# buctcurry/ICKA

Hardware: AMD Instinct MI355X
Metric: MNER samples/sec (fwd+bwd) at seq=128, 36 regions, bs=32 per GPU (higher is better)
Workload: dtype bf16; 1 GPU; c2: bert(H768,L12,h12,I3072)+36x2048 regions, seq_len 128, per-GPU batch 32, 1 cross layer(s), gated head, 13 labels, train mode p=0.1, token-CE loss; global_batch=32, seq_len=128, regions=36, parallelism=dp1, launch=hipgraph, precision=bf16, accumulate=1

## Files before the change

### icka_amd/_lib.py

```python
from __future__ import annotations

import ctypes as C
import os
from typing import Optional

_HERE = os.path.dirname(os.path.abspath(__file__))
LIB_PATH = os.path.join(_HERE, "libicka_hip.so")

c_vp, c_i32, c_i64, c_u64, c_f32 = C.c_void_p, C.c_int32, C.c_int64, C.c_uint64, C.c_float

ABI_VERSION = 6
GEMM_NT, GEMM_NN, GEMM_TN, GEMM_TT = 0, 1, 2, 3
ATTN_FP8, ATTN_TILED = 1, 2
LSTM_PER_STEP, LSTM_TICKETS, LSTM_NO_BATCH_SPLIT = 1, 2, 4
EPI_NONE, EPI_GELU, EPI_DGELU, EPI_ADD, EPI_GATE, EPI_TANH, EPI_RELU, EPI_ADD_RELU = 0, 1, 2, 3, 4, 5, 6, 7


class GemmDesc(C.Structure):
    _fields_ = [
        ("op", c_i32), ("M", c_i32), ("N", c_i32), ("K", c_i32), ("K1", c_i32),
        ("A", c_vp), ("lda", c_i64), ("B", c_vp), ("ldb", c_i64),
        ("A2", c_vp), ("lda2", c_i64), ("B2", c_vp), ("ldb2", c_i64),
        ("C", c_vp), ("ldc", c_i64), ("c_is_f32", c_i32),
        ("C2", c_vp), ("ldc2", c_i64),
        ("aux", c_vp), ("ldaux", c_i64),
        ("bias", c_vp), ("bias2", c_vp),
        ("alpha", c_f32), ("beta", c_f32),
        ("epilogue", c_i32),
        ("colsum_out", c_vp), ("colsum_accumulate", c_i32),
        ("ab_f16", c_i32), ("C3", c_vp), ("ldc3", c_i64), ("aux_f16", c_i32), ("c3_only", c_i32),
        ("tune", c_u64),
    ]


class SlabReduction(C.Structure):
    _fields_ = [("partials", c_vp), ("slab_stride", c_i64), ("nslab", c_i32), ("H", c_i32), ("nslots", c_i32),
                ("accumulate", c_i32), ("out", c_vp * 4)]


class XGemmDesc(C.Structure):
    _fields_ = [
        ("op", c_i32), ("M", c_i32), ("N", c_i32), ("K", c_i32),
        ("A", c_vp), ("lda", c_i64), ("a_bs0", c_i64), ("a_bs1", c_i64),
        ("B", c_vp), ("ldb", c_i64), ("b_bs0", c_i64), ("b_bs1", c_i64),
        ("C", c_vp), ("ldc", c_i64), ("c_bs0", c_i64), ("c_bs1", c_i64),
        ("nb0", c_i32), ("nb1", c_i32),
        ("bias", c_vp),
        ("alpha", c_f32), ("beta", c_f32),
    ]


PROTOTYPES = {
    "icka_abi_version": (c_i32, []),
    "icka_copy_many": (c_i32, [c_vp, c_vp, c_vp, c_i32, c_vp]),
    "icka_build_arch": (C.c_char_p, []),
    "icka_gemm": (c_i32, [C.POINTER(GemmDesc), c_vp]),
    "icka_gemm_grouped": (c_i32, [C.POINTER(GemmDesc), c_i32, c_vp]),
    "icka_gemm_grouped_ex": (c_i32, [C.POINTER(GemmDesc), c_i32, C.POINTER(SlabReduction), c_i32, c_vp]),
    "icka_gemm_ln": (c_i32, [C.POINTER(GemmDesc), c_vp, c_vp, c_i64, c_i32, c_vp, c_vp, c_vp, c_i64, c_vp, c_i32, c_vp, c_vp, c_f32,
                             c_f32, c_u64, c_vp, c_vp, c_vp]),
    "icka_gemm_qkv_attn": (c_i32, [C.POINTER(GemmDesc), c_vp, c_vp, c_vp, c_i64, c_vp, c_i32, c_i32, c_i32, c_f32, c_f32, c_u64, c_vp, c_vp]),
    "icka_gemm_ln_sync_words": (c_i64, []),
    "icka_gemm_ln_test_hooks": (c_i32, [c_i32, c_i32]),
    "icka_ln_fwd": (c_i32, [c_vp, c_i64, c_i32, c_vp, c_vp, c_i64, c_i32, c_vp, c_vp, c_vp, c_i64, c_vp, c_i64,
                            c_vp, c_vp, c_vp, c_i32, c_i32, c_f32, c_f32, c_u64, c_vp]),
    "icka_ln_fwd_h": (c_i32, [c_vp, c_i64, c_i32, c_vp, c_vp, c_i64, c_i32, c_vp, c_vp, c_vp, c_i64, c_vp, c_i64,
                            c_vp, c_vp, c_vp, c_i32, c_i32, c_f32, c_f32, c_u64, c_vp]),
    "icka_ln_bwd_workspace_floats": (c_i64, [c_i32]),
    "icka_ln_bwd": (c_i32, [c_vp, c_i64, c_vp, c_i64, c_vp, c_vp, c_vp, c_vp, c_i64, c_vp, c_i64, c_vp, c_vp, c_vp,
                            c_vp, c_i32, c_i32, c_f32, c_u64, c_i32, c_vp]),
    "icka_ln_bwd_slabs": (c_i32, [c_vp, c_i64, c_vp, c_i64, c_vp, c_vp, c_vp, c_vp, c_i64, c_vp, c_i64, c_vp, c_i32,
                                  c_i32, c_f32, c_u64, c_vp]),
    "icka_ln_bwd_nslab": (c_i32, [c_i32]),
    "icka_ln_slab_slots": (c_i32, []),
    "icka_embed_fwd": (c_i32, [c_vp, c_vp, c_vp, c_vp, c_vp, c_vp, c_vp, c_vp, c_vp, c_vp, c_vp, c_i32, c_i32,
                               c_i32, c_i32, c_i32, c_f32, c_f32, c_u64, c_vp]),
    "icka_embed_fwd_h": (c_i32, [c_vp, c_vp, c_vp, c_vp, c_vp, c_vp, c_vp, c_vp, c_vp, c_vp, c_vp, c_i32, c_i32,
                               c_i32, c_i32, c_i32, c_f32, c_f32, c_u64, c_vp]),
    "icka_embed_bwd": (c_i32, [c_vp, c_vp, c_vp, c_vp, c_vp, c_vp, c_vp, c_vp, c_vp, c_vp, c_vp, c_vp, c_i32, c_i32,
                               c_i32, c_i32, c_i32, c_i32, c_f32, c_u64, c_i32, c_vp]),
    "icka_embed_bwd_rows": (c_i32, [c_vp, c_vp, c_vp, c_vp, c_vp, c_vp, c_vp, c_vp, c_vp, c_vp, c_vp, c_vp, c_i32, c_i32,
                                    c_i32, c_i32, c_i32, c_i32, c_f32, c_u64, c_i32, c_vp]),
    "icka_embed_scatter_rows": (c_i32, [c_vp, c_i32, c_vp, c_vp, c_i64, c_i32, c_i32, c_i32, c_f32, c_vp]),
    "icka_attn_fwd": (c_i32, [c_vp, c_i64, c_vp, c_i64, c_vp, c_i64, c_vp, c_vp, c_i64, c_vp, c_i32, c_i32, c_i32,
                              c_i32, c_f32, c_f32, c_u64, c_vp]),
    "icka_attn_fwd_ex": (c_i32, [c_vp, c_i64, c_vp, c_i64, c_vp, c_i64, c_vp, c_vp, c_vp, c_i64, c_vp, c_i32, c_i32, c_i32,
                                 c_i32, c_f32, c_f32, c_u64, c_i32, c_vp, c_vp]),
    "icka_attn_keepbits_words": (c_i64, [c_i32, c_i32, c_i32, c_i32]),
    "icka_attn_fwd_fp8": (c_i32, [c_vp, c_i64, c_vp, c_i64, c_vp, c_i64, c_vp, c_vp, c_i64, c_vp, c_i32, c_i32, c_i32,
                              c_i32, c_f32, c_f32, c_u64, c_vp]),
    "icka_cls_head_fwd": (c_i32, [c_vp, c_vp, c_vp, c_vp, c_vp, c_i32, c_i32, c_i32, c_vp]),
    "icka_cls_head_fwd_h": (c_i32, [c_vp, c_vp, c_vp, c_vp, c_vp, c_i32, c_i32, c_i32, c_vp]),
    "icka_cls_head_bwd": (c_i32, [c_vp, c_i64, c_vp, c_vp, c_vp, c_vp, c_vp, c_vp, c_vp, c_vp, c_vp, c_i32, c_i32, c_i32,
                                  c_vp]),
    "icka_cls_head_bwd_slabs": (c_i32, [c_i32]),
    "icka_cls_head_slab_floats": (c_i64, [c_i32, c_i32]),
    "icka_conv_stem_patches": (c_i32, [c_vp, c_vp, c_i32, c_i32, c_i32, c_i64, c_vp]),
    "icka_conv_im2col3x3": (c_i32, [c_vp, c_vp, c_i32, c_i32, c_i32, c_i32, c_i32, c_i64, c_vp]),
    "icka_conv3x3_gemm": (c_i32, [c_vp, c_vp, c_vp, c_vp, c_i64, c_vp, c_i32, c_i32, c_i32, c_i32, c_i32, c_i32, c_i64, c_i32,
                                   c_vp, c_vp]),
    "icka_conv_subsample": (c_i32, [c_vp, c_vp, c_i32, c_i32, c_i32, c_i32, c_i32, c_i64, c_vp]),
    "icka_conv_maxpool3x3s2": (c_i32, [c_vp, c_vp, c_i32, c_i32, c_i32, c_i32, c_i64, c_vp]),
    "icka_conv_features_out": (c_i32, [c_vp, c_vp, c_vp, c_vp, c_i32, c_i32, c_i32, c_vp]),
    "icka_gemm_bn_stats": (c_i32, [c_vp, c_i64, c_vp, c_i64, c_vp, c_i64, c_i32, c_i32, c_i32, c_i64, c_vp, c_vp]),
    "icka_conv3x3_gemm_stats": (c_i32, [c_vp, c_vp, c_vp, c_i32, c_i32, c_i32, c_i32, c_i32, c_i32, c_i64, c_vp, c_vp, c_vp]),
    "icka_bn_finalize": (c_i32, [c_vp, c_i32, c_i32, c_vp, c_vp, c_vp, c_vp, c_vp, c_f32, c_f32, c_vp, c_vp, c_vp]),
    "icka_bn_apply": (c_i32, [c_vp, c_vp, c_vp, c_vp, c_vp, c_vp, c_vp, c_i32, c_i64, c_i64, c_i32, c_vp, c_vp, c_vp]),
    "icka_lstm_fwd": (c_i32, [c_vp, c_i64, c_vp, c_vp, c_vp, c_vp, c_vp, c_i32, c_i32, c_i32, c_i32, c_vp]),
    "icka_lstm_bwd": (c_i32, [c_vp, c_vp, c_vp, c_vp, c_vp, c_i64, c_vp, c_i32, c_i32, c_i32, c_i32, c_vp]),
    "icka_lstm_barrier_error": (c_i32, []),
    "icka_lstm_clear_error": (c_i32, []),
    "icka_lstm_set_reserved_cus": (c_i32, [c_i32]),
    "icka_lstm_test_hooks": (c_i32, [c_i32, c_i32]),
    "icka_linear_small_m": (c_i32, [c_vp, c_i64, c_vp, c_vp, c_vp, c_i64, c_i32, c_i32, c_i32, c_i32, c_vp]),
    "icka_transpose_bf16": (c_i32, [c_vp, c_vp, c_i32, c_i32, c_i32, c_vp]),
    "icka_crf_llh": (c_i32, [c_vp, c_i64, c_vp, c_vp, c_vp, c_vp, c_vp, c_vp, c_i32, c_i32, c_i32, c_vp]),
    "icka_crf_grad": (c_i32, [c_vp, c_i64, c_vp, c_vp, c_vp, c_vp, c_vp, c_vp, c_vp, c_i64, c_vp, c_vp, c_vp, c_i32,
                              c_i32, c_i32, c_vp]),
    "icka_crf_decode": (c_i32, [c_vp, c_i64, c_vp, c_vp, c_vp, c_vp, c_vp, c_vp, c_i32, c_i32, c_i32, c_vp]),
    "icka_crf_score_decode": (c_i32, [c_vp, c_i64, c_vp, c_vp, c_vp, c_vp, c_vp, c_vp, c_vp, c_vp, c_i64, c_i32, c_i32, c_i32,
                                      c_vp]),
    "icka_chunk_eval": (c_i32, [c_vp, c_vp, c_i64, c_vp, c_i64, c_vp, c_vp, c_vp, c_vp, c_i32, c_i32, c_i32, c_i32, c_vp]),
    "icka_loss_accumulate": (c_i32, [c_vp, c_vp, c_vp]),
    "icka_attn_bwd":(c_i32, [c_vp, c_i64, c_vp, c_i64, c_vp, c_i64, c_vp, c_vp, c_i64, c_vp, c_i64, c_vp, c_vp,
                              c_vp, c_i64, c_vp, c_i64, c_vp, c_i64, c_i32, c_i32, c_i32, c_i32, c_f32, c_f32, c_u64,
                              c_vp, c_i32, c_vp]),
    "icka_cast_f32_to_bf16": (c_i32, [c_vp, c_vp, c_i64, c_vp]),
    "icka_cast_to_f16": (c_i32, [c_vp, c_i32, c_vp, c_i64, c_vp]),
    "icka_cast_f32_to_bf16_f16": (c_i32, [c_vp, c_vp, c_vp, c_i64, c_vp]),
    "icka_cast_bf16_to_f32": (c_i32, [c_vp, c_vp, c_i64, c_vp]),
    "icka_cast_pad_f32_to_bf16": (c_i32, [c_vp, c_i64, c_vp, c_i64, c_i32, c_i32, c_vp]),
    "icka_additive_mask": (c_i32, [c_vp, c_i64, c_vp, c_i32, c_i32, c_vp]),
    "icka_dropout": (c_i32, [c_vp, c_i64, c_vp, c_i64, c_vp, c_i64, c_i32, c_i32, c_f32, c_u64, c_vp]),
    "icka_regions_to_tokens": (c_i32, [c_vp, c_vp, c_i32, c_i32, c_i32, c_i32, c_vp]),
    "icka_regions_to_tokens_h": (c_i32, [c_vp, c_vp, c_vp, c_i32, c_i32, c_i32, c_i32, c_vp]),
    "icka_sample_gate_fwd_h": (c_i32, [c_vp, c_i64, c_vp, c_i32, c_vp, c_vp, c_i64, c_i32, c_i32, c_i32, c_vp]),
    "icka_colsum": (c_i32, [c_vp, c_i64, c_vp, c_vp, c_i32, c_i32, c_i32, c_vp]),
    "icka_colsum_workspace_floats": (c_i64, [c_i32]),
    "icka_gate_bwd": (c_i32, [c_vp, c_i64, c_vp, c_vp, c_i64, c_vp, c_i64, c_vp, c_vp, c_i64, c_i32, c_i32, c_vp]),
    "icka_sample_gate_fwd": (c_i32, [c_vp, c_i64, c_vp, c_i64, c_vp, c_i32, c_vp, c_i64, c_i32, c_i32, c_i32, c_vp]),
    "icka_sample_gate_bwd": (c_i32, [c_vp, c_i64, c_vp, c_i64, c_vp, c_i64, c_vp, c_i32, c_vp, c_i64, c_vp, c_i64, c_vp,
                                     c_i32, c_i32, c_i32, c_vp]),
    "icka_crs_fwd": (c_i32, [c_vp, c_i64, c_vp, c_i64, c_vp, c_vp, c_vp, c_i32, c_i32, c_i32, c_vp]),
    "icka_crs_bwd": (c_i32, [c_vp, c_vp, c_i64, c_vp, c_i64, c_vp, c_vp, c_vp, c_vp, c_vp, c_i32, c_i32, c_i32, c_i32,
                             c_vp]),
    "icka_add_bf16": (c_i32, [c_vp, c_vp, c_vp, c_i64, c_vp]),
    "icka_tanh_bwd": (c_i32, [c_vp, c_vp, c_vp, c_i64, c_vp]),
    "icka_contrastive_workspace_floats": (c_i64, [c_i32]),
    "icka_contrastive_fwd": (c_i32, [c_vp, c_i64, c_vp, c_i64, c_i32, c_i32, c_i32, c_f32, c_f32, c_vp, c_i32, c_vp, c_vp, c_vp]),
    "icka_contrastive_bwd": (c_i32, [c_vp, c_i64, c_vp, c_i64, c_i32, c_i32, c_i32, c_f32, c_f32, c_vp, c_vp, c_vp, c_vp, c_vp,
                                     c_vp, c_i32, c_vp, c_vp]),
    "icka_relu_bwd": (c_i32, [c_vp, c_vp, c_vp, c_i64, c_i32, c_vp]),
    "icka_sample_swap": (c_i32, [c_vp, c_vp, c_i32, c_i64, c_i32, c_vp]),
    "icka_dgelu_bf16": (c_i32, [c_vp, c_vp, c_vp, c_i64, c_vp]),
    "icka_embed_prompt_fwd": (c_i32, [c_vp, c_vp, c_vp, c_vp, c_vp, c_vp, c_vp, c_vp, c_vp, c_vp, c_vp, c_vp, c_i32, c_i32,
# ... 101 lines not shown
```

### icka_amd/csrc/gemm.hip

```cpp
#include "common.h"
#include "ln_row.h"
#include "attn_core.h"
#include <cstdio>
#include <cstdlib>

namespace {

constexpr int BM = 128, BN = 128, BK = 64;
constexpr int TILE_BYTES = 128 * 64 * 2;

struct GemmArgs {
    int M, N, K, K1;
    const bf16_t* A;  int64_t lda;
    const bf16_t* B;  int64_t ldb;
    const bf16_t* A2; int64_t lda2;
    const bf16_t* B2; int64_t ldb2;
    void* C;  int64_t ldc;
    bf16_t* C2; int64_t ldc2;
    const bf16_t* aux; int64_t ldaux;
    const float* bias; const float* bias2;
    float alpha, beta;
    int epi, c_f32;
    int a_vec, b_vec;
    int abl;
// ... 274 lines not shown
__device__ __forceinline__ void wait_vmcnt() { asm volatile("s_waitcnt vmcnt(%0)" ::"n"(N) : "memory"); }

template <bool KM, int NCOL = 128>
__device__ __forceinline__ void dma_init(const bf16_t* (&ptr)[4], const bf16_t* __restrict__ P, int64_t ld, int row0,
                                         int wave, int lane) {
#pragma unroll
    for (int j = 0; j < 4; ++j) {
        const int p = wave + 4 * j;
        if (!KM) {
            const int row = (8 * p + (lane >> 3)) % NCOL;
            const int lc = (lane & 7) ^ ((row >> 1) & 7);
            ptr[j] = P + (int64_t)(row0 + row) * ld + 8 * lc;
        } else {
            const int kr = 4 * p + (lane >> 4);
            int lc = (lane & 15) ^ (((kr & 3) << 2) | ((kr >> 2) & 3));
            if (lc >= NCOL / 8) lc &= 7;
            ptr[j] = P + (int64_t)kr * ld + row0 + 8 * lc;
        }
    }
}
#ifndef ICKA_DMA_POL
#define ICKA_DMA_POL ""
#endif
template <int NJ = 4>
__device__ __forceinline__ void dma_issue(const bf16_t* (&ptr)[4], int64_t stride, uint32_t lds_base) {
    uint32_t keep;
    if constexpr (NJ == 2) {
        asm volatile(
            "s_mov_b32 %0, m0\n\t"
            "s_mov_b32 m0, %3\n\t"
            "s_nop 0\n\t"
            "global_load_lds_dwordx4 %1, off" ICKA_DMA_POL "\n\t"
            "s_add_u32 m0, m0, 0x1000\n\t"
            "s_nop 0\n\t"
            "global_load_lds_dwordx4 %2, off" ICKA_DMA_POL "\n\t"
            "s_mov_b32 m0, %0"
            : "=&s"(keep)
            : "v"(ptr[0]), "v"(ptr[1]), "s"(lds_base)
            : "memory", "scc");
#pragma unroll
        for (int j = 0; j < 2; ++j) ptr[j] += stride;
        return;
    }
    if constexpr (NJ == 3) {
        asm volatile(
            "s_mov_b32 %0, m0\n\t"
            "s_mov_b32 m0, %4\n\t"
            "s_nop 0\n\t"
            "global_load_lds_dwordx4 %1, off" ICKA_DMA_POL "\n\t"
            "s_add_u32 m0, m0, 0x1000\n\t"
            "s_nop 0\n\t"
            "global_load_lds_dwordx4 %2, off" ICKA_DMA_POL "\n\t"
            "s_add_u32 m0, m0, 0x1000\n\t"
            "s_nop 0\n\t"
            "global_load_lds_dwordx4 %3, off" ICKA_DMA_POL "\n\t"
            "s_mov_b32 m0, %0"
            : "=&s"(keep)
            : "v"(ptr[0]), "v"(ptr[1]), "v"(ptr[2]), "s"(lds_base)
            : "memory", "scc");
#pragma unroll
        for (int j = 0; j < 3; ++j) ptr[j] += stride;
        return;
    }
    asm volatile(
        "s_mov_b32 %0, m0\n\t"
        "s_mov_b32 m0, %5\n\t"
        "s_nop 0\n\t"
        "global_load_lds_dwordx4 %1, off" ICKA_DMA_POL "\n\t"
        "s_add_u32 m0, m0, 0x1000\n\t"
        "s_nop 0\n\t"
        "global_load_lds_dwordx4 %2, off" ICKA_DMA_POL "\n\t"
        "s_add_u32 m0, m0, 0x1000\n\t"
        "s_nop 0\n\t"
        "global_load_lds_dwordx4 %3, off" ICKA_DMA_POL "\n\t"
        "s_add_u32 m0, m0, 0x1000\n\t"
        "s_nop 0\n\t"
        "global_load_lds_dwordx4 %4, off" ICKA_DMA_POL "\n\t"
        "s_mov_b32 m0, %0"
        : "=&s"(keep)
        : "v"(ptr[0]), "v"(ptr[1]), "v"(ptr[2]), "v"(ptr[3]), "s"(lds_base)
        : "memory", "scc");
#pragma unroll
    for (int j = 0; j < 4; ++j) ptr[j] += stride;
}

__device__ __forceinline__ uint32_t off_c(int row, int ch) { return row * 512 + ((ch ^ (row & 31)) << 4); }
__device__ __forceinline__ uint32_t off_cw(int row, int ch) { return row * 768 + ((ch ^ (row & 15)) << 4); }

template <typename T>
__device__ __forceinline__ void st_out(T* p, const T v) {
#ifdef ICKA_ST_TEMPORAL
    *p = v;
#else
    __builtin_nontemporal_store(v, p);
#endif
}
template <typename T>
__device__ __forceinline__ T ld_once(const T* p) {
#ifdef ICKA_NT_AUX
    return __builtin_nontemporal_load(p);
#else
    return *p;
#endif
}
__device__ __forceinline__ void load8_bf16(const bf16_t* p, float (&o)[8]) {
    const bf16x8 v = as_bf16x8(ld_once(reinterpret_cast<const u32x4*>(p)));
#pragma unroll
    for (int e = 0; e < 8; ++e) o[e] = bf2f(v[e]);
}
__device__ __forceinline__ void load8_aux(const bf16_t* p, int f16, float (&o)[8]) {
    if (f16) {
        const f16x8 v = __builtin_bit_cast(f16x8, ld_once(reinterpret_cast<const u32x4*>(p)));
#pragma unroll
        for (int e = 0; e < 8; ++e) o[e] = (float)v[e];
    } else {
        load8_bf16(p, o);
    }
}
__device__ __forceinline__ void cvt8_aux(const u32x4 raw, int f16, float (&o)[8]) {
    if (f16) {
        const f16x8 v = __builtin_bit_cast(f16x8, raw);
#pragma unroll
        for (int e = 0; e < 8; ++e) o[e] = (float)v[e];
    } else {
        const bf16x8 v = as_bf16x8(raw);
#pragma unroll
        for (int e = 0; e < 8; ++e) o[e] = bf2f(v[e]);
    }
}
__device__ __forceinline__ void store8_bf16(bf16_t* p, const float (&v)[8]) {
    bf16x8 o;
#pragma unroll
    for (int e = 0; e < 8; ++e) o[e] = f2bf(v[e]);
    st_out(reinterpret_cast<u32x4*>(p), as_u32x4(o));
}
template <typename T>
__device__ __forceinline__ void st_main(T* p, const T v, int plain) {
    if (plain) *p = v;
    else st_out(p, v);
}
__device__ __forceinline__ void store8_bf16_main(bf16_t* p, const float (&v)[8], int plain) {
    bf16x8 o;
#pragma unroll
    for (int e = 0; e < 8; ++e) o[e] = f2bf(v[e]);
    st_main(reinterpret_cast<u32x4*>(p), as_u32x4(o), plain);
}

__device__ __forceinline__ _Float16 f2h(float v) { return (_Float16)fminf(fmaxf(v, -65504.f), 65504.f); }
__device__ __forceinline__ void store8_f16(void* p, const float (&v)[8], int plain = 0) {
    f16x8 o;
#pragma unroll
    for (int e = 0; e < 8; ++e) o[e] = f2h(v[e]);
    st_main(reinterpret_cast<u32x4*>(p), __builtin_bit_cast(u32x4, o), plain);
}

__device__ __forceinline__ void tile_origin(int bid, int nb, int nbm, int nbn, int& m0, int& n0, int bn = BN) {
    const int xcd = bid & 7, li = bid >> 3;
    if (nbn >= 12 && (nb & 7) == 0 && (nbm & 3) == 0 && (nbn & 1) == 0) {
        const int sm = nbm >> 2, sn = nbn >> 1;
        const int xi = xcd >> 1, xj = xcd & 1;
        m0 = (xi * sm + li / sn) * BM;
        n0 = (xj * sn + li % sn) * bn;
        return;
    }
    const int qn = nb >> 3, rn = nb & 7;
    const int sw = (xcd < rn ? xcd * (qn + 1) : rn * (qn + 1) + (xcd - rn) * qn) + li;
// ... 1071 lines not shown
    return best;
}

template <bool A_KM, bool B_KM, bool F16 = false>
int launch(GemmArgs g, bool aligned, hipStream_t st, const Tune& t) {
    const int nb = ((g.M + BM - 1) / BM) * ((g.N + BN - 1) / BN);
    if constexpr (!A_KM && !B_KM) {
        if (!aligned && g.n64ok && t.ws) {
            hipLaunchKernelGGL((gemm_ws_kernel<false, false, 3, 0, 64, F16>), dim3((g.M / BM) * (g.N / 64)), dim3(512), 0, st, g);
            ICKA_CHECK_LAUNCH();
            return 0;
        }
    }
    if (aligned) {
#ifdef ICKA_GEMM_ABLATE
        if (t.abl == 1 && !t.ws) hipLaunchKernelGGL((gemm_dma_kernel<A_KM, B_KM, 3, 1>), dim3(nb), dim3(256), 0, st, g);
        else if (t.abl == 2 && !t.ws) hipLaunchKernelGGL((gemm_dma_kernel<A_KM, B_KM, 3, 2>), dim3(nb), dim3(256), 0, st, g);
        else
#endif
        {
            if (t.ws || F16) {
#ifdef ICKA_GEMM_ABLATE
                if (t.bn == 96 && g.n96ok) {
                    const int nb96 = (g.M / BM) * (g.N / 96);
                    if (t.abl == 1) { hipLaunchKernelGGL((gemm_ws_kernel<A_KM, B_KM, 3, 1, 96>), dim3(nb96), dim3(512), 0, st, g); ICKA_CHECK_LAUNCH(); return 0; }
                    if (t.abl == 2) { hipLaunchKernelGGL((gemm_ws_kernel<A_KM, B_KM, 3, 2, 96>), dim3(nb96), dim3(512), 0, st, g); ICKA_CHECK_LAUNCH(); return 0; }
                    if (t.abl == 3) { hipLaunchKernelGGL((gemm_ws_kernel<A_KM, B_KM, 3, 3, 96>), dim3(nb96), dim3(512), 0, st, g); ICKA_CHECK_LAUNCH(); return 0; }
                }
                if (t.abl == 1) { hipLaunchKernelGGL((gemm_ws_kernel<A_KM, B_KM, 3, 1>), dim3(nb), dim3(512), 0, st, g); ICKA_CHECK_LAUNCH(); return 0; }
                if (t.abl == 2) { hipLaunchKernelGGL((gemm_ws_kernel<A_KM, B_KM, 3, 2>), dim3(nb), dim3(512), 0, st, g); ICKA_CHECK_LAUNCH(); return 0; }
#endif
                if constexpr (!A_KM) {
                    const int nb3 = (g.M / 256) * (g.N / 192);
                    const int rounds3 = (nb3 + 255) / 256;
                    if (t.w3 && g.M % 256 == 0 && g.N % 192 == 0 && g.K <= 1024 && g.K1 == 0 && nb3 % 8 == 0 &&
                        nb3 >= 128 && 4 * nb3 >= 3 * 256 * rounds3 && g.ksplit == 1) {
                        { const int pm = gemm_w3_grid(g.M, g.N, 192, t.w3grid), pn = 8 / pm;
                          g.w3_sn = (g.N / 192) / pn; g.w3_pnlog = pn == 1 ? 0 : (pn == 2 ? 1 : (pn == 4 ? 2 : 3)); }
                        hipLaunchKernelGGL((gemm_w3_kernel<B_KM, F16>), dim3(nb3), dim3(768), 0, st, g);
                        ICKA_CHECK_LAUNCH();
                        return 0;
                    }
                    const int nb2 = (g.M / 256) * (g.N / 128);
                    if (t.w3 && g.M % 256 == 0 && g.K1 == 0 && g.ksplit == 1 && nb2 % 8 == 0 && nb2 >= 192 && nb2 <= 256 &&
                        !(g.n96ok && t.bn == 96) && !(g.K <= 1024 && g.direct && g.c_f32 && g.epi == ICKA_EPI_NONE && g.beta == 0.f)) {
                        { const int pm = gemm_w3_grid(g.M, g.N, 128, t.w3grid), pn = 8 / pm;
                          g.w3_sn = (g.N / 128) / pn; g.w3_pnlog = pn == 1 ? 0 : (pn == 2 ? 1 : (pn == 4 ? 2 : 3)); }
                        hipLaunchKernelGGL((gemm_w3_kernel<B_KM, F16, 128>), dim3(nb2), dim3(768), 0, st, g);
                        ICKA_CHECK_LAUNCH();
                        return 0;
                    }
                }
                if (g.n96ok && t.bn != 128) {
                    const int nb96 = (g.M / BM) * (g.N / 96);
                    if (t.bn == 96 || (nb < 256 && nb96 <= 256 && nb96 > nb)) {
                        if ((t.ws == 2 || (t.ws == 1 && nb96 >= 448 && g.K <= 1024)) && !A_KM)
                            hipLaunchKernelGGL((gemm_ws2_kernel<A_KM, B_KM, 96, F16>), dim3(nb96), dim3(512), 0, st, g);
                        else if (t.nbuf == 4 && !F16)
                            hipLaunchKernelGGL((gemm_ws_kernel<A_KM, B_KM, 4, 0, 96>), dim3(nb96), dim3(512), 0, st, g);
                        else if (t.nbuf == 5 && !F16)
                            hipLaunchKernelGGL((gemm_ws_kernel<A_KM, B_KM, 5, 0, 96>), dim3(nb96), dim3(512), 0, st, g);
                        else
                            hipLaunchKernelGGL((gemm_ws_kernel<A_KM, B_KM, 3, 0, 96, F16>), dim3(nb96), dim3(512), 0, st, g);
                        ICKA_CHECK_LAUNCH();
                        return 0;
                    }
                }
                if ((t.ws == 2 || (t.ws == 1 && nb >= 448 && g.K <= 1024)) && !A_KM)
                    hipLaunchKernelGGL((gemm_ws2_kernel<A_KM, B_KM, 128, F16>), dim3(nb), dim3(512), 0, st, g);
                else if (t.nbuf == 4 && !F16) hipLaunchKernelGGL((gemm_ws_kernel<A_KM, B_KM, 4>), dim3(nb), dim3(512), 0, st, g);
                else if (t.nbuf == 5 && !F16) hipLaunchKernelGGL((gemm_ws_kernel<A_KM, B_KM, 5>), dim3(nb), dim3(512), 0, st, g);
                else hipLaunchKernelGGL((gemm_ws_kernel<A_KM, B_KM, 3, 0, 128, F16>), dim3(nb), dim3(512), 0, st, g);
                ICKA_CHECK_LAUNCH();
                return 0;
            }
            const int nbuf = t.nbuf > 0 ? t.nbuf : (nb >= 448 ? 2 : 4);
            if (nbuf == 2) hipLaunchKernelGGL((gemm_dma_kernel<A_KM, B_KM, 2, 0>), dim3(nb), dim3(256), 0, st, g);
            else if (nbuf == 3) hipLaunchKernelGGL((gemm_dma_kernel<A_KM, B_KM, 3, 0>), dim3(nb), dim3(256), 0, st, g);
            else hipLaunchKernelGGL((gemm_dma_kernel<A_KM, B_KM, 4, 0>), dim3(nb), dim3(256), 0, st, g);
        }
    } else {
        const int nk = (g.K + BK - 1) / BK;
        int ks = 1;
        if (g.c_f32 && g.epi == ICKA_EPI_NONE && nb < 64 && nk >= 16 && g.M <= 256 && !g.C3) {
            ks = 256 / nb;
            if (ks > nk / 4) ks = nk / 4;
            if (ks < 1) ks = 1;
        }
        if (ks > 1) {
            const int64_t n = (int64_t)g.M * g.N;
            hipLaunchKernelGGL(scale_c_kernel, dim3((unsigned)((n + 255) / 256)), dim3(256), 0, st,
                               reinterpret_cast<float*>(g.C), g.ldc, g.M, g.N, g.beta);
            ICKA_CHECK_LAUNCH();
            g.beta = 0.f;
            g.ksplit = ks;
        }
        hipLaunchKernelGGL((gemm_kernel<A_KM, B_KM, false, F16>), dim3(nb, ks), dim3(256), 0, st, g);
    }
    ICKA_CHECK_LAUNCH();
    return 0;
}

inline bool vec_ok(const void* p, int64_t ld) { return (ld % 8 == 0) && ((reinterpret_cast<uintptr_t>(p) & 15) == 0); }

}

#ifdef ICKA_GEMM_STAMP
extern "C" int icka_diag_gemm_stamp_buffer(void* p) {
    g_stamp = (unsigned long long*)p;
    return 0;
}
#endif

static int site_bit(const icka_gemm_desc* d) {
    const int64_t N = d->N, K = d->K;
    if (d->c_is_f32 == 1 || d->M < 1024) return -1;
    if (d->op == ICKA_GEMM_NT) {
        if (N == 3 * K) return 0;
        if (N == K) return 1;
        if (N == 4 * K) return 2;
        if (K == 4 * N) return 3;
    } else if (d->op == ICKA_GEMM_NN) {
        if (N == 4 * K) return 4;
        if (K == 4 * N) return 5;
        if (N == K) return 6;
        if (K == 3 * N) return 7;
    }
    return -1;
}
static int plain_mask() {
    static int m = -1;
    if (m < 0) {
        const char* e = getenv("ICKA_GEMM_PLAIN_MASK");
        m = e ? (int)strtol(e, nullptr, 0) : 0;
    }
    return m;
}

static int convert(const icka_gemm_desc* d, GemmArgs& g, bool& aligned, Tune& t) {
    if (!d || !d->A || !d->B || !d->C) return ICKA_E_ARG;
    if (!tune_of(d->tune, t)) return ICKA_E_ARG;
    if (d->M <= 0 || d->N <= 0 || d->K <= 0) return ICKA_E_SHAPE;
    if (d->op < ICKA_GEMM_NT || d->op > ICKA_GEMM_TN) return ICKA_E_ARG;
    if (d->K1 != 0 && (d->K1 < 0 || d->K1 >= d->K || d->K1 % BK != 0 || !d->A2 || !d->B2)) return ICKA_E_ARG;
    if ((d->epilogue == ICKA_EPI_GELU) && !d->C2) return ICKA_E_ARG;
    if ((d->epilogue == ICKA_EPI_DGELU || d->epilogue == ICKA_EPI_ADD || d->epilogue == ICKA_EPI_GATE ||
         d->epilogue == ICKA_EPI_ADD_RELU) && !d->aux)
        return ICKA_E_ARG;
    g.M = d->M; g.N = d->N; g.K = d->K; g.K1 = d->K1;
    g.A = (const bf16_t*)d->A; g.lda = d->lda; g.B = (const bf16_t*)d->B; g.ldb = d->ldb;
    g.A2 = (const bf16_t*)d->A2; g.lda2 = d->lda2; g.B2 = (const bf16_t*)d->B2; g.ldb2 = d->ldb2;
    g.C = d->C; g.ldc = d->ldc; g.C2 = (bf16_t*)d->C2; g.ldc2 = d->ldc2;
    g.aux = (const bf16_t*)d->aux; g.ldaux = d->ldaux; g.bias = d->bias; g.bias2 = d->bias2;
    g.alpha = d->alpha; g.beta = d->beta; g.epi = d->epilogue;
    if (d->c_is_f32 < 0 || d->c_is_f32 > 2) return ICKA_E_ARG;
    g.c_f32 = d->c_is_f32 == 1; g.c_f16 = d->c_is_f32 == 2;
    g.f16 = d->ab_f16 != 0; g.C3 = (bf16_t*)d->C3; g.ldc3 = d->ldc3; g.aux_f16 = d->aux_f16 != 0;
    if (g.f16 && d->op != ICKA_GEMM_NT) return ICKA_E_ARG;
    if (g.c_f16 && d->beta != 0.f) return ICKA_E_ARG;
    if (g.C3 && !g.c_f16 && !g.c_f32) return ICKA_E_ARG;
    if (g.C3 && g.c_f32 && d->op != ICKA_GEMM_TN) return ICKA_E_ARG;
    g.c3_only = d->c3_only != 0;
    {
        const int sb = site_bit(d);
        g.plain = (sb >= 0 && ((plain_mask() >> sb) & 1)) ? 1 : 0;
    }
    if (g.c3_only && !(g.C3 && g.c_f32 && d->beta == 0.f && d->epilogue == ICKA_EPI_NONE)) return ICKA_E_ARG;
// ... 180 lines not shown
        hipLaunchKernelGGL((gemm_ws_kernel<false, false, 3, 0, 64, false, true>), dim3((g.M / BM) * (Cout / 64)), dim3(512), 0, st, g);
    ICKA_CHECK_LAUNCH();
    return 0;
}

static int launch_bn_stats(BnStatsArgs& p, hipStream_t st) {
    GemmArgs& g = p.g;
    g.K1 = 0; g.alpha = 1.f; g.beta = 0.f; g.epi = ICKA_EPI_NONE; g.c_f32 = 0; g.a_vec = g.b_vec = 1; g.ksplit = 1; g.direct = 0;
    if (g.N % 128 == 0)
        hipLaunchKernelGGL((gemm_ws_bn_stats_kernel<128, false>), dim3((g.M / BM) * (g.N / 128)), dim3(512), 0, st, p);
    else
        hipLaunchKernelGGL((gemm_ws_bn_stats_kernel<64, false>), dim3((g.M / BM) * (g.N / 64)), dim3(512), 0, st, p);
    ICKA_CHECK_LAUNCH();
    return 0;
}

extern "C" int icka_gemm_bn_stats(const void* a, int64_t lda, const void* w, int64_t ldw, void* y, int64_t ldy, int32_t M, int32_t N,
                                  int32_t K, int64_t rows_valid, float* partials, void* stream) {
    if (!a || !w || !y || !partials) return ICKA_E_ARG;
    if (M <= 0 || M % BM || N <= 0 || N % 64 || K <= 0 || K % BK || rows_valid < 1 || rows_valid > M) return ICKA_E_SHAPE;
    auto al = [](const void* p) { return (reinterpret_cast<uintptr_t>(p) & 15) == 0; };
    if (!al(a) || !al(w) || !al(y) || !al(partials) || lda % 8 || ldw % 8 || ldy % 8 || lda < K || ldw < K || ldy < N)
        return ICKA_E_ALIGN;
    BnStatsArgs p{};
    p.g.M = M; p.g.N = N; p.g.K = K;
    p.g.A = (const bf16_t*)a; p.g.lda = lda; p.g.B = (const bf16_t*)w; p.g.ldb = ldw; p.g.C = y; p.g.ldc = ldy;
    p.part = partials; p.rows_valid = (int)rows_valid;
    return launch_bn_stats(p, (hipStream_t)stream);
}

extern "C" int icka_conv3x3_gemm_stats(const void* x, const void* w, void* y, int32_t B, int32_t H, int32_t W, int32_t C, int32_t Cout,
                                       int32_t stride, int64_t rows_padded, const void* zeros, float* partials, void* stream) {
    if (!x || !w || !y || !zeros || !partials) return ICKA_E_ARG;
    if (B <= 0 || H <= 0 || W <= 0 || C <= 0 || C % 64 || Cout <= 0 || Cout % 64 || (stride != 1 && stride != 2))
        return ICKA_E_SHAPE;
    const int Ho = (H + 2 - 3) / stride + 1, Wo = (W + 2 - 3) / stride + 1;
    const int64_t rows = (int64_t)B * Ho * Wo;
    if (rows_padded < rows || rows_padded % BM || rows_padded > 0x7fffffff) return ICKA_E_SHAPE;
    auto al = [](const void* p) { return (reinterpret_cast<uintptr_t>(p) & 15) == 0; };
    if (!al(x) || !al(w) || !al(y) || !al(zeros) || !al(partials)) return ICKA_E_ALIGN;
    BnStatsArgs p{};
    p.g.M = (int)rows_padded; p.g.N = Cout; p.g.K = 9 * C;
    p.g.A = (const bf16_t*)x; p.g.lda = C; p.g.B = (const bf16_t*)w; p.g.ldb = 9 * (int64_t)C; p.g.C = y; p.g.ldc = Cout;
    p.g.cvH = H; p.g.cvW = W; p.g.cvC = C; p.g.cvS = stride; p.g.cvHo = Ho; p.g.cvWo = Wo; p.g.cvRows = (int)rows;
    p.g.cvZero = (const bf16_t*)zeros;
    p.part = partials; p.rows_valid = (int)rows;
    GemmArgs& g = p.g;
    g.K1 = 0; g.alpha = 1.f; g.beta = 0.f; g.epi = ICKA_EPI_NONE; g.c_f32 = 0; g.a_vec = g.b_vec = 1; g.ksplit = 1; g.direct = 0;
    hipStream_t st = (hipStream_t)stream;
    if (Cout % 128 == 0)
        hipLaunchKernelGGL((gemm_ws_bn_stats_kernel<128, true>), dim3((g.M / BM) * (Cout / 128)), dim3(512), 0, st, p);
    else
        hipLaunchKernelGGL((gemm_ws_bn_stats_kernel<64, true>), dim3((g.M / BM) * (Cout / 64)), dim3(512), 0, st, p);
    ICKA_CHECK_LAUNCH();
    return 0;
}

template <bool A_KM, bool B_KM, int NBUF>
__global__ __launch_bounds__(512) void gemm_ws_group_kernel(const GroupArgs ga) {
    __shared__ __attribute__((aligned(16))) char smem[NBUF * 2 * TILE_BYTES];
    const int bid = blockIdx.x;
    int pi = 0;
#pragma unroll
    for (int i = 1; i < MAX_GROUP; ++i) pi += bid >= ga.start[i] ? 1 : 0;
    const GemmArgs g = ga.p[pi];
    gemm_ws_body<A_KM, B_KM, NBUF>(g, smem, bid - ga.start[pi], ga.start[pi + 1] - ga.start[pi]);
}

constexpr int BIG_STAGE = 3 * TILE_BYTES;
constexpr int BIG_NBUF = 3;
constexpr int CS_COLS = 64;

constexpr int MAX_RED = 4;
struct SlabRed {
    const float* partials; float* out[4];
    int nslab, H, nslots, slab_stride, accumulate, blocks;
};
struct BigGroupArgs {
    GemmArgs p[MAX_GROUP];
    int start[MAX_GROUP + 1];
    int cs_start[MAX_GROUP + 1];
    SlabRed red[MAX_RED];
    int red_start[MAX_RED + 1];
};

__device__ __forceinline__ void slab_reduce_block(const SlabRed& r, char* smem, int rb) {
    float* red = reinterpret_cast<float*>(smem);
    const int tid = threadIdx.x, cx = tid & 63, sy = tid >> 6;
    const int idx = rb * 64 + cx;
    const bool ok = idx < r.nslots * r.H;
    float s = 0.f;
    if (ok) {
        const int slot = idx / r.H, c = idx - slot * r.H;
        const float* p = r.partials + (int64_t)slot * r.H + c;
        for (int b = sy; b < r.nslab; b += 8) s += p[(int64_t)b * r.slab_stride];
    }
    red[sy * 64 + cx] = s;
    __syncthreads();
    if (sy == 0 && ok) {
        const int slot = idx / r.H, c = idx - slot * r.H;
        float* out = r.out[slot];
        if (out) {
            float t = 0.f;
#pragma unroll
            for (int k = 0; k < 8; ++k) t += red[k * 64 + cx];
            out[c] = r.accumulate ? out[c] + t : t;
        }
    }
}
__global__ __launch_bounds__(512) void slab_reduce_kernel(const SlabRed r) {
    __shared__ __attribute__((aligned(16))) char smem[8 * 64 * 4];
    slab_reduce_block(r, smem, blockIdx.x);
}
struct GroupArgsRed { GroupArgs ga; SlabRed red[MAX_RED]; int red_start[MAX_RED + 1]; };
template <bool A_KM, bool B_KM, int NBUF>
__global__ __launch_bounds__(512) void gemm_ws_group_red_kernel(const GroupArgsRed gr) {
    __shared__ __attribute__((aligned(16))) char smem[NBUF * 2 * TILE_BYTES];
    const int bid = blockIdx.x;
    const int tiles = gr.ga.start[MAX_GROUP];
    if (bid >= tiles) {
        const int rb = bid - tiles;
        int ri = 0;
#pragma unroll
        for (int i = 1; i < MAX_RED; ++i) ri += rb >= gr.red_start[i] ? 1 : 0;
        slab_reduce_block(gr.red[ri], smem, rb - gr.red_start[ri]);
        return;
    }
    int pi = 0;
#pragma unroll
    for (int i = 1; i < MAX_GROUP; ++i) pi += bid >= gr.ga.start[i] ? 1 : 0;
    const GemmArgs g = gr.ga.p[pi];
    gemm_ws_body<A_KM, B_KM, NBUF>(g, smem, bid - gr.ga.start[pi], gr.ga.start[pi + 1] - gr.ga.start[pi]);
}
struct SlabRedMulti { SlabRed red[MAX_RED]; int red_start[MAX_RED + 1]; };
__global__ __launch_bounds__(512) void slab_reduce_multi_kernel(const SlabRedMulti m) {
    __shared__ __attribute__((aligned(16))) char smem[8 * 64 * 4];
    const int rb = blockIdx.x;
    int ri = 0;
#pragma unroll
    for (int i = 1; i < MAX_RED; ++i) ri += rb >= m.red_start[i] ? 1 : 0;
    slab_reduce_block(m.red[ri], smem, rb - m.red_start[ri]);
}

template <bool WIRE>
__device__ __forceinline__ void gemm_big_tn_body(const GemmArgs& g, char* smem, const int m0, const int n0) {
    const int tid = threadIdx.x, lane = tid & 63;
    const int wave = __builtin_amdgcn_readfirstlane(tid >> 6);
    const uint32_t lds0 = __builtin_amdgcn_readfirstlane((uint32_t)reinterpret_cast<uintptr_t>(LDS_PTR(char, smem)));
    const int nk = g.K / BK;

    if (wave >= 4) {
        const int lw = wave - 4;
        const bf16_t* pa0[4];
        const bf16_t* pa1[4];
        const bf16_t* pb[4];
        dma_init<true>(pa0, g.A, g.lda, m0, lw, lane);
        dma_init<true>(pa1, g.A, g.lda, m0 + 128, lw, lane);
        dma_init<true>(pb, g.B, g.ldb, n0, lw, lane);
        const int64_t sa = (int64_t)BK * g.lda, sb = (int64_t)BK * g.ldb;
#define ICKA_BIG_STAGE(BUF)                                              \
    do {                                                                 \
        dma_issue(pa0, sa, lds0 + (BUF) + lw * 1024);                    \
        dma_issue(pa1, sa, lds0 + (BUF) + TILE_BYTES + lw * 1024);       \
        dma_issue(pb, sb, lds0 + (BUF) + 2 * TILE_BYTES + lw * 1024);    \
    } while (0)
#pragma unroll
// ... 54 lines not shown
    __builtin_amdgcn_sched_barrier(0);
    int cur = 0;
    for (int kt = 0; kt + 1 < nk; ++kt) {
        ICKA_BIG_READ(fa1, fb1, cur, 1);
        ICKA_BIG_MMA(fa0, fb0);
        ICKA_BIG_INTERLEAVE();
        const int nxt = cur + 1 == BIG_NBUF ? 0 : cur + 1;
        asm volatile("s_waitcnt lgkmcnt(0)" ::: "memory");
        __builtin_amdgcn_s_barrier();
        asm volatile("" ::: "memory");
        ICKA_BIG_READ(fa0, fb0, nxt, 0);
        ICKA_BIG_MMA(fa1, fb1);
        ICKA_BIG_INTERLEAVE();
        cur = nxt;
    }
    ICKA_BIG_READ(fa1, fb1, cur, 1);
    ICKA_BIG_MMA(fa0, fb0);
    ICKA_BIG_INTERLEAVE();
    ICKA_BIG_MMA(fa1, fb1);
    __builtin_amdgcn_sched_barrier(0);
#undef ICKA_BIG_INTERLEAVE
#undef ICKA_BIG_READ
#undef ICKA_BIG_MMA
    asm volatile("s_nop 7\n\ts_nop 7" ::: "memory");
#pragma unroll
    for (int ni = 0; ni < 4; ++ni) {
        const int n = n0 + wc + 16 * ni + 4 * (lane >> 4);
#pragma unroll
        for (int mi = 0; mi < 8; ++mi) {
            const int m = m0 + wsub * 128 + 16 * mi + (lane & 15);
            f32x4* dst = reinterpret_cast<f32x4*>(reinterpret_cast<float*>(g.C) + (int64_t)m * g.ldc + n);
            f32x4 v = acc[mi][ni] * g.alpha;
            if (g.beta != 0.f) v += g.beta * ld_once(dst);
            if (!WIRE || !g.c3_only) st_out(dst, v);
            if constexpr (WIRE) {
                if (g.C3) st_out(reinterpret_cast<u32x2*>(g.C3 + (int64_t)m * g.ldc3 + n), pack4(v[0], v[1], v[2], v[3]));
            }
        }
    }
}

__device__ __forceinline__ void big_colsum_block(const GemmArgs& g, char* smem, int cb) {
    float* red = reinterpret_cast<float*>(smem);
    const int tid = threadIdx.x, cx = tid & 7, ry = tid >> 3;
    const int col = cb * CS_COLS + cx * 8;
    float s[8];
#pragma unroll
    for (int e = 0; e < 8; ++e) s[e] = 0.f;
    if (col < g.M) {
        const bf16_t* base = g.A + col;
        int k = ry;
        for (; k + 7 * 64 < g.K; k += 8 * 64) {
            u32x4 v[8];
#pragma unroll
            for (int u = 0; u < 8; ++u) v[u] = *reinterpret_cast<const u32x4*>(base + (int64_t)(k + 64 * u) * g.lda);
#pragma unroll
            for (int u = 0; u < 8; ++u) {
                const bf16x8 h = as_bf16x8(v[u]);
#pragma unroll
                for (int e = 0; e < 8; ++e) s[e] += bf2f(h[e]);
            }
        }
        for (; k < g.K; k += 64) {
            const bf16x8 h = as_bf16x8(*reinterpret_cast<const u32x4*>(base + (int64_t)k * g.lda));
#pragma unroll
            for (int e = 0; e < 8; ++e) s[e] += bf2f(h[e]);
        }
    }
#pragma unroll
    for (int e = 0; e < 8; ++e) red[ry * CS_COLS + cx * 8 + e] = s[e];
    __syncthreads();
    if (tid < CS_COLS) {
        const int c = cb * CS_COLS + tid;
        if (c < g.M) {
            float t = 0.f;
#pragma unroll 8
            for (int r = 0; r < 64; ++r) t += red[r * CS_COLS + tid];
            g.colsum[c] = g.colsum_acc ? g.colsum[c] + t : t;
        }
    }
}


template <bool WIRE>
__device__ __forceinline__ void gemm_big12_tn_body(const GemmArgs& g, char* smem, const int m0, const int n0) {
    const int tid = threadIdx.x, lane = tid & 63;
    const int wave = __builtin_amdgcn_readfirstlane(tid >> 6);
    const uint32_t lds0 = __builtin_amdgcn_readfirstlane((uint32_t)reinterpret_cast<uintptr_t>(LDS_PTR(char, smem)));
    const int nk = g.K / BK;
    if (wave >= 8) {
        const int lw = wave - 8;
        const bf16_t* pa0[4];
        const bf16_t* pa1[4];
        const bf16_t* pb[4];
        dma_init<true>(pa0, g.A, g.lda, m0, lw, lane);
        dma_init<true>(pa1, g.A, g.lda, m0 + 128, lw, lane);
        dma_init<true>(pb, g.B, g.ldb, n0, lw, lane);
        const int64_t sa = (int64_t)BK * g.lda, sb = (int64_t)BK * g.ldb;
#define ICKA_BIG_STAGE(BUF)                                              \
    do {                                                                 \
        dma_issue(pa0, sa, lds0 + (BUF) + lw * 1024);                    \
        dma_issue(pa1, sa, lds0 + (BUF) + TILE_BYTES + lw * 1024);       \
        dma_issue(pb, sb, lds0 + (BUF) + 2 * TILE_BYTES + lw * 1024);    \
    } while (0)
#pragma unroll
        for (int t = 0; t < BIG_NBUF - 1; ++t)
            if (t < nk) ICKA_BIG_STAGE(t * BIG_STAGE);
        int cur = 0;
        for (int kt = 0; kt < nk; ++kt) {
            int ahead = nk - 1 - kt;
            ahead = ahead > BIG_NBUF - 2 ? BIG_NBUF - 2 : ahead;
            if (ahead >= 1) wait_vmcnt<12>();
            else wait_vmcnt<0>();
            __builtin_amdgcn_s_barrier();
            if (kt + BIG_NBUF - 1 < nk) {
                int nx = cur + BIG_NBUF - 1;
                nx = nx >= BIG_NBUF ? nx - BIG_NBUF : nx;
                ICKA_BIG_STAGE(nx * BIG_STAGE);
            }
            cur = cur + 1 == BIG_NBUF ? 0 : cur + 1;
        }
#undef ICKA_BIG_STAGE
        return;
    }
    const int wr = (wave >> 1) * 64, wc = (wave & 1) * 64;
    f32x4 acc[4][4];
#pragma unroll
    for (int i = 0; i < 4; ++i)
#pragma unroll
        for (int j = 0; j < 4; ++j) acc[i][j] = f32x4{0.f, 0.f, 0.f, 0.f};
    int cur = 0;
    for (int kt = 0; kt < nk; ++kt) {
        __builtin_amdgcn_s_barrier();
        asm volatile("" ::: "memory");
        const char* st = smem + cur * BIG_STAGE;
        const char* sA = st + (wr >> 7) * TILE_BYTES;
        const char* sB = st + 2 * TILE_BYTES;
#pragma unroll
        for (int ks = 0; ks < 2; ++ks) {
            bf16x8 fa[4], fb[4];
#pragma unroll
            for (int t = 0; t < 4; ++t) fa[t] = read_frag<true>(sA, (wr & 127) + 16 * t, ks, lane);
#pragma unroll
            for (int t = 0; t < 4; ++t) fb[t] = read_frag<true>(sB, wc + 16 * t, ks, lane);
#pragma unroll
            for (int mi = 0; mi < 4; ++mi)
#pragma unroll
                for (int ni = 0; ni < 4; ++ni) acc[mi][ni] = mfma16(fb[ni], fa[mi], acc[mi][ni]);
        }
        cur = cur + 1 == BIG_NBUF ? 0 : cur + 1;
    }
    asm volatile("s_nop 7\n\ts_nop 7" ::: "memory");
#pragma unroll
    for (int ni = 0; ni < 4; ++ni) {
        const int n = n0 + wc + 16 * ni + 4 * (lane >> 4);
#pragma unroll
        for (int mi = 0; mi < 4; ++mi) {
            const int m = m0 + wr + 16 * mi + (lane & 15);
            f32x4* dst = reinterpret_cast<f32x4*>(reinterpret_cast<float*>(g.C) + (int64_t)m * g.ldc + n);
            f32x4 v = acc[mi][ni] * g.alpha;
            if (g.beta != 0.f) v += g.beta * ld_once(dst);
            if (!WIRE || !g.c3_only) st_out(dst, v);
            if constexpr (WIRE) {
                if (g.C3) st_out(reinterpret_cast<u32x2*>(g.C3 + (int64_t)m * g.ldc3 + n), pack4(v[0], v[1], v[2], v[3]));
            }
        }
    }
}

template <bool W12, bool WIRE = false>
__global__ __launch_bounds__(W12 ? 768 : 512) void gemm_big_group_kernel(const BigGroupArgs ga) {
    __shared__ __attribute__((aligned(16))) char smem[BIG_NBUF * BIG_STAGE];
    const int bid = blockIdx.x;
    const int tiles = ga.start[MAX_GROUP];
    if (bid >= tiles + ga.cs_start[MAX_GROUP]) {
        const int rb = bid - tiles - ga.cs_start[MAX_GROUP];
        int ri = 0;
#pragma unroll
        for (int i = 1; i < MAX_RED; ++i) ri += rb >= ga.red_start[i] ? 1 : 0;
        if (W12 && threadIdx.x >= 512) return;
        slab_reduce_block(ga.red[ri], smem, rb - ga.red_start[ri]);
        return;
    }
    if (bid >= tiles) {
        const int cb = bid - tiles;
        int pi = 0;
#pragma unroll
        for (int i = 1; i < MAX_GROUP; ++i) pi += cb >= ga.cs_start[i] ? 1 : 0;
        const GemmArgs g = ga.p[pi];
        if (W12 && threadIdx.x >= 512) return;
        big_colsum_block(g, smem, cb - ga.cs_start[pi]);
        return;
    }
    const int xcd = bid & 7, slot = bid >> 3;
    const int qn = tiles >> 3, rn = tiles & 7;
    const int gt = (xcd < rn ? xcd * (qn + 1) : rn * (qn + 1) + (xcd - rn) * qn) + slot;
    int pi = 0;
#pragma unroll
    for (int i = 1; i < MAX_GROUP; ++i) pi += gt >= ga.start[i] ? 1 : 0;
    const GemmArgs g = ga.p[pi];
    const int local = gt - ga.start[pi];
    const int nbm = g.M / 256, nbn = g.N / BN;
    int tm, tn;
    if (nbn > nbm) { tm = local % nbm; tn = local / nbm; }
    else { tm = local / nbn; tn = local % nbn; }
    if constexpr (W12) gemm_big12_tn_body<WIRE>(g, smem, tm * 256, tn * BN);
    else gemm_big_tn_body<WIRE>(g, smem, tm * 256, tn * BN);
}

static bool big_ok(const GemmArgs& g, bool aligned) {
    return aligned && g.M % 256 == 0 && g.c_f32 && g.epi == ICKA_EPI_NONE && g.K1 == 0 && !g.bias && !g.bias2 && g.direct;
}

template <bool A_KM, bool B_KM>
static int launch_group(const GroupArgs& ga, int total, hipStream_t st, const Tune& t) {
    if (t.ws) {
        hipLaunchKernelGGL((gemm_ws_group_kernel<A_KM, B_KM, 3>), dim3(total), dim3(512), 0, st, ga);
        ICKA_CHECK_LAUNCH();
        return 0;
    }
    const int nbuf = t.nbuf > 0 ? t.nbuf : (total >= 448 ? 2 : 4);
    if (nbuf == 2) hipLaunchKernelGGL((gemm_dma_group_kernel<A_KM, B_KM, 2>), dim3(total), dim3(256), 0, st, ga);
    else if (nbuf == 3) hipLaunchKernelGGL((gemm_dma_group_kernel<A_KM, B_KM, 3>), dim3(total), dim3(256), 0, st, ga);
    else hipLaunchKernelGGL((gemm_dma_group_kernel<A_KM, B_KM, 4>), dim3(total), dim3(256), 0, st, ga);
    ICKA_CHECK_LAUNCH();
    return 0;
}

static int grouped_impl(const icka_gemm_desc* descs, int32_t n, const icka_slab_reduction* reds, int32_t n_red,
                        hipStream_t st);

extern "C" int icka_gemm_grouped(const icka_gemm_desc* descs, int32_t n, void* stream) {
    if (!descs || n <= 0) return ICKA_E_ARG;
    return grouped_impl(descs, n, nullptr, 0, (hipStream_t)stream);
}

extern "C" int icka_gemm_grouped_ex(const icka_gemm_desc* descs, int32_t n, const icka_slab_reduction* reds,
                                    int32_t n_red, void* stream) {
    if (n < 0 || n_red < 0 || (n > 0 && !descs) || (n_red > 0 && !reds) || n_red > MAX_RED) return ICKA_E_ARG;
    for (int r = 0; r < n_red; ++r)
        if (!reds[r].partials || reds[r].nslab <= 0 || reds[r].H <= 0 || reds[r].nslots <= 0 || reds[r].nslots > 4 ||
            reds[r].slab_stride < (int64_t)reds[r].nslots * reds[r].H)
            return ICKA_E_ARG;
    return grouped_impl(descs, n, reds, n_red, (hipStream_t)stream);
}

static SlabRed to_red(const icka_slab_reduction& r) {
    SlabRed o{};
    o.partials = r.partials;
    for (int k = 0; k < 4; ++k) o.out[k] = k < r.nslots ? r.out[k] : nullptr;
    o.nslab = r.nslab; o.H = r.H; o.nslots = r.nslots; o.slab_stride = (int)r.slab_stride; o.accumulate = r.accumulate;
    o.blocks = (r.nslots * r.H + 63) / 64;
    return o;
}

static int grouped_impl(const icka_gemm_desc* descs, int32_t n, const icka_slab_reduction* reds, int32_t n_red,
                        hipStream_t st) {
    bool reds_done = n_red == 0;
    int i = 0;
    Tune t = kTuneEnv;
    if (n > 0 && !tune_of(descs[0].tune, t)) return ICKA_E_ARG;
    Tune tk;
    while (i < n) {
        if (t.big && t.ws && descs[i].op == ICKA_GEMM_TN) {
            BigGroupArgs ba;
            int cnt = 0, total = 0, cs_total = 0;
            while (i + cnt < n && cnt < MAX_GROUP && descs[i + cnt].op == ICKA_GEMM_TN) {
                bool aligned = false;
                GemmArgs g;
                const int rc = convert(&descs[i + cnt], g, aligned, tk);
                if (rc) return rc;
                if (!big_ok(g, aligned)) break;
                ba.p[cnt] = g;
                ba.start[cnt] = total;
                ba.cs_start[cnt] = cs_total;
                total += (g.M / 256) * (g.N / BN);
                if (g.colsum) cs_total += (g.M + CS_COLS - 1) / CS_COLS;
                ++cnt;
            }
            if (cnt >= 1 && total >= 64) {
                for (int k = cnt; k <= MAX_GROUP; ++k) { ba.start[k] = total; ba.cs_start[k] = cs_total; }
                for (int k = cnt; k < MAX_GROUP; ++k) ba.p[k] = ba.p[0];
                int red_total = 0;
                for (int r = 0; r < MAX_RED; ++r) {
                    ba.red_start[r] = red_total;
                    if (!reds_done && r < n_red) { ba.red[r] = to_red(reds[r]); red_total += ba.red[r].blocks; }
                    else ba.red[r] = SlabRed{};
                }
                ba.red_start[MAX_RED] = red_total;
                reds_done = true;
                bool wire = false;
                for (int k = 0; k < cnt; ++k) wire = wire || ba.p[k].C3 != nullptr;
                const dim3 grid(total + cs_total + red_total);
                if (t.big == 2) {
                    if (wire) hipLaunchKernelGGL((gemm_big_group_kernel<true, true>), grid, dim3(768), 0, st, ba);
                    else hipLaunchKernelGGL((gemm_big_group_kernel<true, false>), grid, dim3(768), 0, st, ba);
                } else {
                    if (wire) hipLaunchKernelGGL((gemm_big_group_kernel<false, true>), grid, dim3(512), 0, st, ba);
                    else hipLaunchKernelGGL((gemm_big_group_kernel<false, false>), grid, dim3(512), 0, st, ba);
                }
                ICKA_CHECK_LAUNCH();
                i += cnt;
                continue;
            }
        }
        GroupArgs ga;
        int cnt = 0, total = 0;
        const int op = descs[i].op;
        while (i + cnt < n && cnt < MAX_GROUP && descs[i + cnt].op == op && !descs[i + cnt].ab_f16) {
            bool aligned = false;
            const int rc = convert(&descs[i + cnt], ga.p[cnt], aligned, tk);
            if (rc) return rc;
            if (ga.p[cnt].colsum && !(aligned && t.ws)) return ICKA_E_ARG;
            if (!aligned) break;
            ga.start[cnt] = total;
            total += (ga.p[cnt].M / BM) * (ga.p[cnt].N / BN);
            ++cnt;
        }
        if (cnt >= 2) {
            for (int k = cnt; k <= MAX_GROUP; ++k) ga.start[k] = total;
            for (int k = cnt; k < MAX_GROUP; ++k) ga.p[k] = ga.p[0];
            int rc;
            if (op == ICKA_GEMM_TN && !reds_done && t.ws) {
                GroupArgsRed gr;
                gr.ga = ga;
                int red_total = 0;
                for (int r = 0; r < MAX_RED; ++r) {
                    gr.red_start[r] = red_total;
                    if (r < n_red) { gr.red[r] = to_red(reds[r]); red_total += gr.red[r].blocks; }
                    else gr.red[r] = SlabRed{};
                }
                gr.red_start[MAX_RED] = red_total;
                hipLaunchKernelGGL((gemm_ws_group_red_kernel<true, true, 3>), dim3(total + red_total), dim3(512), 0, st, gr);
                ICKA_CHECK_LAUNCH();
                reds_done = true;
                rc = 0;
            } else if (op == ICKA_GEMM_NT) rc = launch_group<false, false>(ga, total, st, t);
            else if (op == ICKA_GEMM_NN) rc = launch_group<false, true>(ga, total, st, t);
            else rc = launch_group<true, true>(ga, total, st, t);
            if (rc) return rc;
            i += cnt;
        } else {
            const int rc = icka_gemm(&descs[i], (void*)st);
            if (rc) return rc;
            ++i;
        }
    }
    if (!reds_done) {
        if (n_red == 1) {
            const SlabRed sr = to_red(reds[0]);
            hipLaunchKernelGGL(slab_reduce_kernel, dim3(sr.blocks), dim3(512), 0, st, sr);
        } else {
            SlabRedMulti m;
            int total = 0;
            for (int r = 0; r < MAX_RED; ++r) {
                m.red_start[r] = total;
                if (r < n_red) { m.red[r] = to_red(reds[r]); total += m.red[r].blocks; }
                else m.red[r] = SlabRed{};
            }
            m.red_start[MAX_RED] = total;
            for (int r = n_red; r < MAX_RED; ++r) m.red_start[r] = total;
            hipLaunchKernelGGL(slab_reduce_multi_kernel, dim3(total), dim3(512), 0, st, m);
        }
        ICKA_CHECK_LAUNCH();
    }
    return 0;
}
```

### icka_amd/csrc/layernorm.hip

```cpp
#include "common.h"
#include "ln_row.h"
#include <cstdlib>

namespace {

constexpr int BWD_BLOCKS = 1024;
constexpr int SLOTS = 4;

template <int NCH>
__global__ __launch_bounds__(256) void ln_fwd_kernel(const LnFwdArgs a_) {
    LnFwdArgs a = a_;
    a.drop = drop_resolve(a.drop);
    const int lane = threadIdx.x & 63;
    const int wid = blockIdx.x * 4 + (threadIdx.x >> 6), nw = gridDim.x * 4;
    ln_fwd_rows<NCH>(a, wid, nw, a.M, lane);
}

struct LnBwdArgs {
    const bf16_t* dy; int64_t lddy; const bf16_t* dy2; int64_t lddy2; const bf16_t* xhat; const float* rstd;
    const float* gamma; bf16_t* dres; int64_t lddres; bf16_t* dx; int64_t lddx; float* partials;
    int M, H; DropCfg drop;
};

template <int NCH, int NS>
__device__ __forceinline__ void flush_columns(float (&acc)[NS][NCH][8], float* lds, float* partials, int H) {
    const int lane = threadIdx.x & 63, nchunk = H >> 3;
    for (int i = threadIdx.x; i < NS * H; i += 256) lds[i] = 0.f;
    __syncthreads();
#pragma unroll
    for (int s = 0; s < NS; ++s)
#pragma unroll
        for (int i = 0; i < NCH; ++i) {
            const int c = lane + 64 * i;
            if (c < nchunk) {
#pragma unroll
                for (int e = 0; e < 8; ++e) atomicAdd(&lds[s * H + c * 8 + e], acc[s][i][e]);
            }
        }
    __syncthreads();
    float* slab = partials + (int64_t)blockIdx.x * SLOTS * H;
    for (int i = threadIdx.x; i < NS * H; i += 256) slab[i] = lds[i];
}

template <int NCH>
__device__ __forceinline__ void ln_bwd_load_raw(const LnBwdArgs& a, int row, int lane, int nchunk, u32x4 (&dy)[NCH], u32x4 (&dy2)[NCH],
                                                u32x4 (&xh)[NCH]) {
#pragma unroll
    for (int i = 0; i < NCH; ++i) {
        const int c = lane + 64 * i;
        if (c < nchunk) {
            dy[i] = *reinterpret_cast<const u32x4*>(a.dy + (int64_t)row * a.lddy + c * 8);
            if (a.dy2) dy2[i] = *reinterpret_cast<const u32x4*>(a.dy2 + (int64_t)row * a.lddy2 + c * 8);
            xh[i] = *reinterpret_cast<const u32x4*>(a.xhat + (int64_t)row * a.H + c * 8);
        }
    }
}
__device__ __forceinline__ void unpack8(const u32x4 raw, float (&o)[8]) {
    const bf16x8 v = as_bf16x8(raw);
#pragma unroll
    for (int e = 0; e < 8; ++e) o[e] = bf2f(v[e]);
}

template <int NCH>
__device__ __forceinline__ void ln_rows_body(const LnBwdArgs& a_, int blk, int nblk) {
    LnBwdArgs a = a_;
    a.drop = drop_resolve(a.drop);
    const int lane = threadIdx.x & 63;
    const int wid = blk * 4 + (threadIdx.x >> 6), nw = nblk * 4;
    const int nchunk = a.H >> 3;
    const float inv_h = 1.f / (float)a.H;
    u32x4 rdy[NCH], rdy2[NCH], rxh[NCH];
    if (wid < a.M) ln_bwd_load_raw<NCH>(a, wid, lane, nchunk, rdy, rdy2, rxh);
    for (int row = wid; row < a.M; row += nw) {
        float xh[NCH][8], gd[NCH][8];
        float s1 = 0.f, s2 = 0.f;
        uint32_t kb[NCH];
#pragma unroll
        for (int i = 0; i < NCH; ++i) {
            kb[i] = 0xffu;
            const int c = lane + 64 * i;
            if (a.drop.thr && c < nchunk) {
                const uint32_t base = (uint32_t)row * (uint32_t)a.H + c * 8;
                uint32_t bits = 0u;
#pragma unroll
                for (int e = 0; e < 8; ++e) bits |= (icka_hash(a.drop.s0, a.drop.s1, base + e) >= a.drop.thr ? 1u : 0u) << e;
                kb[i] = bits;
            }
        }
#pragma unroll
        for (int i = 0; i < NCH; ++i) asm volatile("" : "+v"(kb[i]));
#pragma unroll
        for (int i = 0; i < NCH; ++i) {
            const int c = lane + 64 * i;
            if (c < nchunk) {
                float dy[8];
                unpack8(rdy[i], dy);
                if (a.dy2) {
                    float t[8];
                    unpack8(rdy2[i], t);
#pragma unroll
                    for (int e = 0; e < 8; ++e) dy[e] += t[e];
                }
                unpack8(rxh[i], xh[i]);
                float g[8];
                load8f(a.gamma + c * 8, g);
#pragma unroll
                for (int e = 0; e < 8; ++e) {
                    gd[i][e] = g[e] * dy[e];
                    s1 += gd[i][e];
                    s2 += gd[i][e] * xh[i][e];
                }
            }
        }
        const int nrow = row + nw;
        if (nrow < a.M) ln_bwd_load_raw<NCH>(a, nrow, lane, nchunk, rdy, rdy2, rxh);
        const float c1 = wave_sum(s1) * inv_h, c2 = wave_sum(s2) * inv_h;
        const float rstd = a.rstd[row];
#pragma unroll
        for (int i = 0; i < NCH; ++i) {
            const int c = lane + 64 * i;
            if (c < nchunk) {
                float ds[8];
#pragma unroll
                for (int e = 0; e < 8; ++e) ds[e] = rstd * (gd[i][e] - c1 - xh[i][e] * c2);
                if (a.dres) store8(a.dres + (int64_t)row * a.lddres + c * 8, ds);
                if (a.drop.thr) {
#pragma unroll
                    for (int e = 0; e < 8; ++e) ds[e] *= ((kb[i] >> e) & 1u) ? a.drop.scale : 0.f;
                }
                if (a.dx) store8(a.dx + (int64_t)row * a.lddx + c * 8, ds);
            }
        }
    }
}

template <int NCH>
__global__ __launch_bounds__(256) void ln_bwd_kernel(const LnBwdArgs a) {
    ln_rows_body<NCH>(a, blockIdx.x, gridDim.x);
}

constexpr int COL_GROUPS = 128;
__device__ __forceinline__ void ln_cols_body(const bf16_t* __restrict__ dy, int64_t lddy,
                                             const bf16_t* __restrict__ dy2, int64_t lddy2,
                                             const bf16_t* __restrict__ xhat, const bf16_t* __restrict__ dx,
                                             int64_t lddx, float* __restrict__ partials, int M, int H,
                                             int rows_per_group, int bx, int by) {
    __shared__ float red[3][8][32][8];
    const int cx = threadIdx.x & 31, ry = threadIdx.x >> 5;
    const int col = (bx * 32 + cx) * 8;
    const int r0 = by * rows_per_group;
    int r1 = r0 + rows_per_group; r1 = r1 > M ? M : r1;
    float ag[8], ab[8], ax[8];
#pragma unroll
    for (int e = 0; e < 8; ++e) { ag[e] = 0.f; ab[e] = 0.f; ax[e] = 0.f; }
    if (col < H) {
#pragma unroll 4
        for (int r = r0 + ry; r < r1; r += 8) {
            float d[8], x[8];
            load8(dy + (int64_t)r * lddy + col, d);
            if (dy2) {
                float t[8];
                load8(dy2 + (int64_t)r * lddy2 + col, t);
#pragma unroll
                for (int e = 0; e < 8; ++e) d[e] += t[e];
            }
            load8(xhat + (int64_t)r * H + col, x);
#pragma unroll
            for (int e = 0; e < 8; ++e) { ag[e] += d[e] * x[e]; ab[e] += d[e]; }
            if (dx) {
                load8(dx + (int64_t)r * lddx + col, x);
#pragma unroll
                for (int e = 0; e < 8; ++e) ax[e] += x[e];
            }
        }
    }
#pragma unroll
    for (int e = 0; e < 8; ++e) { red[0][ry][cx][e] = ag[e]; red[1][ry][cx][e] = ab[e]; red[2][ry][cx][e] = ax[e]; }
    __syncthreads();
    for (int i = threadIdx.x; i < 3 * 256; i += 256) {
        const int slot = i >> 8, cc = i & 255, c = bx * 256 + cc;
        if (c < H) {
            float t = 0.f;
#pragma unroll
            for (int k = 0; k < 8; ++k) t += red[slot][k][cc >> 3][cc & 7];
            partials[((int64_t)by * SLOTS + slot) * H + c] = t;
        }
    }
}
__global__ __launch_bounds__(256) void ln_cols_kernel(const bf16_t* __restrict__ dy, int64_t lddy,
                                                      const bf16_t* __restrict__ dy2, int64_t lddy2,
                                                      const bf16_t* __restrict__ xhat, const bf16_t* __restrict__ dx,
                                                      int64_t lddx, float* __restrict__ partials, int M, int H,
                                                      int rows_per_group) {
    ln_cols_body(dy, lddy, dy2, lddy2, xhat, dx, lddx, partials, M, H, rows_per_group, blockIdx.x, blockIdx.y);
}

struct LnColsArgs {
    int nx, groups, rows_per_group;
};
template <int NCH>
__global__ __launch_bounds__(256) void ln_bwd_fused_kernel(const LnBwdArgs a, const LnColsArgs c) {
    const int ncol = c.nx * c.groups;
    if ((int)blockIdx.x >= ncol) {
        ln_rows_body<NCH>(a, blockIdx.x - ncol, gridDim.x - ncol);
        return;
    }
    ln_cols_body(a.dy, a.lddy, a.dy2, a.lddy2, a.xhat, nullptr, 0, a.partials, a.M, a.H, c.rows_per_group,
                 blockIdx.x % c.nx, blockIdx.x / c.nx);
}

__global__ __launch_bounds__(1024) void finalize_kernel(const float* __restrict__ partials, int nslab, int H, float* o0,
                                                        float* o1, float* o2, float* o3, int accumulate) {
    __shared__ float red[16][64];
    const int cx = threadIdx.x & 63, sy = threadIdx.x >> 6;
    const int idx = blockIdx.x * 64 + cx;
    float s = 0.f;
    if (idx < SLOTS * H) {
        const int slot = idx / H, c = idx - slot * H;
        for (int b = sy; b < nslab; b += 16) s += partials[((int64_t)b * SLOTS + slot) * H + c];
    }
    red[sy][cx] = s;
    __syncthreads();
    if (sy == 0 && idx < SLOTS * H) {
        const int slot = idx / H, c = idx - slot * H;
        float* out = slot == 0 ? o0 : slot == 1 ? o1 : slot == 2 ? o2 : o3;
        if (out) {
            float t = 0.f;
#pragma unroll
            for (int k = 0; k < 16; ++k) t += red[k][cx];
            out[c] = accumulate ? out[c] + t : t;
        }
    }
}

struct EmbFwdArgs {
    const int64_t* ids; const int64_t* tt; const float* word; const float* pos; const float* type;
    const float* gamma; const float* beta; bf16_t* y; void* yf; bf16_t* xhat; float* rstd;
    int M, S, H, vocab, n_type; float eps; DropCfg drop;
    const int32_t* src; const bf16_t* prompt; int S_in, P, pos_offset;
    int yf_f16;
};

template <int NCH>
__global__ __launch_bounds__(256) void embed_fwd_kernel(const EmbFwdArgs a_) {
    EmbFwdArgs a = a_;
    a.drop = drop_resolve(a.drop);
    const int lane = threadIdx.x & 63;
    const int wid = blockIdx.x * 4 + (threadIdx.x >> 6), nw = gridDim.x * 4;
    const int nchunk = a.H >> 3;
    const float inv_h = 1.f / (float)a.H;
    for (int row = wid; row < a.M; row += nw) {
        const int sp = row % a.S;
        const int sidx = a.src ? a.src[sp] : sp;
        const bf16_t* prow = sidx < 0 ? a.prompt + ((int64_t)(row / a.S) * a.P + (-1 - sidx)) * a.H : nullptr;
        int64_t id = sidx < 0 ? 0 : a.ids[a.src ? (int64_t)(row / a.S) * a.S_in + sidx : row];
        id = id < 0 ? 0 : (id >= a.vocab ? a.vocab - 1 : id);
        int64_t t = a.tt ? a.tt[row] : 0;
        t = t < 0 ? 0 : (t >= a.n_type ? a.n_type - 1 : t);
        float s[NCH][8];
        float sum = 0.f;
#pragma unroll
        for (int i = 0; i < NCH; ++i) {
            const int c = lane + 64 * i;
            if (c < nchunk) {
                float w[8], p[8], ty[8];
                if (prow) load8(prow + c * 8, w);
                else load8f(a.word + id * a.H + c * 8, w);
                load8f(a.pos + (int64_t)(sp + a.pos_offset) * a.H + c * 8, p);
                load8f(a.type + t * a.H + c * 8, ty);
#pragma unroll
                for (int e = 0; e < 8; ++e) { s[i][e] = (w[e] + p[e]) + ty[e]; sum += s[i][e]; }
            } else {
#pragma unroll
                for (int e = 0; e < 8; ++e) s[i][e] = 0.f;
            }
        }
        const float mean = wave_sum(sum) * inv_h;
        float sq = 0.f;
#pragma unroll
        for (int i = 0; i < NCH; ++i)
            if (lane + 64 * i < nchunk) {
#pragma unroll
                for (int e = 0; e < 8; ++e) { const float d = s[i][e] - mean; sq += d * d; }
            }
        const float rstd = 1.f / sqrtf(wave_sum(sq) * inv_h + a.eps);
        if (lane == 0 && a.rstd) a.rstd[row] = rstd;
#pragma unroll
// ... 244 lines not shown
                           int64_t ldy, void* y2, int64_t ldy2, void* y_twin, void* xhat, float* rstd, int32_t M,
                           int32_t H, float eps, float p_drop, uint64_t seed, void* stream) {
    if (!x || !gamma || !beta || !y) return ICKA_E_ARG;
    if (x_is_f32 < 0 || x_is_f32 > 2 || res_is_f32 < 0 || res_is_f32 > 2) return ICKA_E_ARG;
    if (M <= 0 || H <= 0 || H % 8 != 0 || H > 8 * 64 * MAX_CH) return ICKA_E_SHAPE;
    if (ldx % 8 || ldy % 8 || (residual && ldr % 8) || (y2 && ldy2 % 8)) return ICKA_E_ALIGN;
    if (!al16(x) || !al16(y) || (residual && !al16(residual)) || (y2 && !al16(y2)) || (xhat && !al16(xhat)) ||
        (bias && !al16(bias)) || !al16(gamma) || !al16(beta) || (y_twin && !al16(y_twin)))
        return ICKA_E_ALIGN;
    LnFwdArgs a{x, ldx, x_is_f32, bias, residual, ldr, res_is_f32, gamma, beta, (bf16_t*)y, ldy,
                (bf16_t*)y2, ldy2, y_twin, (bf16_t*)xhat, rstd, M, H, eps, make_drop(p_drop, seed), twin_f16};
    hipStream_t st = (hipStream_t)stream;
    DISPATCH_NCH(pick_nch(H), ln_fwd_kernel, fwd_grid(M), 0, st, a);
    ICKA_CHECK_LAUNCH();
    return 0;
}

extern "C" int icka_ln_fwd(const void* x, int64_t ldx, int32_t x_is_f32, const float* bias, const void* residual,
                           int64_t ldr, int32_t res_is_f32, const float* gamma, const float* beta, void* y,
                           int64_t ldy, void* y2, int64_t ldy2, float* y_f32, void* xhat, float* rstd, int32_t M,
                           int32_t H, float eps, float p_drop, uint64_t seed, void* stream) {
    return ln_fwd_impl(0, x, ldx, x_is_f32, bias, residual, ldr, res_is_f32, gamma, beta, y, ldy, y2, ldy2, y_f32, xhat, rstd,
                       M, H, eps, p_drop, seed, stream);
}
extern "C" int icka_ln_fwd_h(const void* x, int64_t ldx, int32_t x_kind, const float* bias, const void* residual,
                             int64_t ldr, int32_t res_kind, const float* gamma, const float* beta, void* y,
                             int64_t ldy, void* y2, int64_t ldy2, void* y_f16, void* xhat, float* rstd, int32_t M,
                             int32_t H, float eps, float p_drop, uint64_t seed, void* stream) {
    return ln_fwd_impl(1, x, ldx, x_kind, bias, residual, ldr, res_kind, gamma, beta, y, ldy, y2, ldy2, y_f16, xhat, rstd,
                       M, H, eps, p_drop, seed, stream);
}

extern "C" int icka_ln_bwd(const void* dy, int64_t lddy, const void* dy2, int64_t lddy2, const void* xhat,
                           const float* rstd, const float* gamma, void* dres, int64_t lddres, void* dx, int64_t lddx,
                           float* dgamma, float* dbeta, float* dbias, float* partials, int32_t M, int32_t H,
                           float p_drop, uint64_t seed, int32_t accumulate, void* stream) {
    if (!dy || !xhat || !rstd || !gamma || !partials) return ICKA_E_ARG;
    if (dbias && !dx) return ICKA_E_ARG;
    if (M <= 0 || H <= 0 || H % 8 != 0 || H > 8 * 64 * MAX_CH) return ICKA_E_SHAPE;
    if (lddy % 8 || (dy2 && lddy2 % 8) || (dres && lddres % 8) || (dx && lddx % 8)) return ICKA_E_ALIGN;
    if (!al16(dy) || (dy2 && !al16(dy2)) || !al16(xhat) || (dres && !al16(dres)) || (dx && !al16(dx)) || !al16(gamma))
        return ICKA_E_ALIGN;
    LnBwdArgs a{(const bf16_t*)dy, lddy, (const bf16_t*)dy2, lddy2, (const bf16_t*)xhat, rstd, gamma,
                (bf16_t*)dres, lddres, (bf16_t*)dx, lddx, partials, M, H, make_drop(p_drop, seed)};
    hipStream_t st = (hipStream_t)stream;
    int groups = (M + 31) / 32; groups = groups > COL_GROUPS ? COL_GROUPS : groups;
    const int rpg = (M + groups - 1) / groups;
    const int nx = (H + 255) / 256;
    if ((dgamma || dbeta) && !dbias) {
        const LnColsArgs c{nx, groups, rpg};
        const int grid = nx * groups + bwd_row_grid(M);
        switch (pick_nch(H)) {
            case 1: hipLaunchKernelGGL((ln_bwd_fused_kernel<1>), dim3(grid), dim3(256), 0, st, a, c); break;
            case 2: hipLaunchKernelGGL((ln_bwd_fused_kernel<2>), dim3(grid), dim3(256), 0, st, a, c); break;
            case 3: hipLaunchKernelGGL((ln_bwd_fused_kernel<3>), dim3(grid), dim3(256), 0, st, a, c); break;
            default: hipLaunchKernelGGL((ln_bwd_fused_kernel<4>), dim3(grid), dim3(256), 0, st, a, c); break;
        }
        ICKA_CHECK_LAUNCH();
        hipLaunchKernelGGL(finalize_kernel, dim3((2 * H + 63) / 64), dim3(1024), 0, st, partials, groups, H, dgamma,
                           dbeta, (float*)nullptr, (float*)nullptr, accumulate);
        ICKA_CHECK_LAUNCH();
        return 0;
    }
    DISPATCH_NCH(pick_nch(H), ln_bwd_kernel, bwd_row_grid(M), 0, st, a);
    ICKA_CHECK_LAUNCH();
    if (dgamma || dbeta || dbias) {
        hipLaunchKernelGGL(ln_cols_kernel, dim3((H + 255) / 256, groups), dim3(256), 0, st, (const bf16_t*)dy, lddy,
                           (const bf16_t*)dy2, lddy2, (const bf16_t*)xhat, dbias ? (const bf16_t*)dx : nullptr, lddx,
                           partials, M, H, rpg);
        ICKA_CHECK_LAUNCH();
        hipLaunchKernelGGL(finalize_kernel, dim3((SLOTS * H + 63) / 64), dim3(1024), 0, st, partials, groups, H, dgamma,
                           dbeta, dbias, (float*)nullptr, accumulate);
        ICKA_CHECK_LAUNCH();
    }
    return 0;
}

extern "C" int32_t icka_ln_bwd_nslab(int32_t M) {
    int groups = (M + 31) / 32;
    return groups > COL_GROUPS ? COL_GROUPS : groups;
}
extern "C" int32_t icka_ln_slab_slots(void) { return SLOTS; }

extern "C" int icka_ln_bwd_slabs(const void* dy, int64_t lddy, const void* dy2, int64_t lddy2, const void* xhat,
                                 const float* rstd, const float* gamma, void* dres, int64_t lddres, void* dx,
                                 int64_t lddx, float* partials, int32_t M, int32_t H, float p_drop, uint64_t seed,
                                 void* stream) {
    if (!dy || !xhat || !rstd || !gamma || !partials) return ICKA_E_ARG;
    if (M <= 0 || H <= 0 || H % 8 != 0 || H > 8 * 64 * MAX_CH) return ICKA_E_SHAPE;
    if (lddy % 8 || (dy2 && lddy2 % 8) || (dres && lddres % 8) || (dx && lddx % 8)) return ICKA_E_ALIGN;
    if (!al16(dy) || (dy2 && !al16(dy2)) || !al16(xhat) || (dres && !al16(dres)) || (dx && !al16(dx)) || !al16(gamma))
        return ICKA_E_ALIGN;
    LnBwdArgs a{(const bf16_t*)dy, lddy, (const bf16_t*)dy2, lddy2, (const bf16_t*)xhat, rstd, gamma,
                (bf16_t*)dres, lddres, (bf16_t*)dx, lddx, partials, M, H, make_drop(p_drop, seed)};
    const int groups = icka_ln_bwd_nslab(M);
    const int nx = (H + 255) / 256;
    const LnColsArgs c{nx, groups, (M + groups - 1) / groups};
    const int grid = nx * groups + bwd_row_grid(M);
    hipStream_t st = (hipStream_t)stream;
    switch (pick_nch(H)) {
        case 1: hipLaunchKernelGGL((ln_bwd_fused_kernel<1>), dim3(grid), dim3(256), 0, st, a, c); break;
        case 2: hipLaunchKernelGGL((ln_bwd_fused_kernel<2>), dim3(grid), dim3(256), 0, st, a, c); break;
        case 3: hipLaunchKernelGGL((ln_bwd_fused_kernel<3>), dim3(grid), dim3(256), 0, st, a, c); break;
        default: hipLaunchKernelGGL((ln_bwd_fused_kernel<4>), dim3(grid), dim3(256), 0, st, a, c); break;
    }
    ICKA_CHECK_LAUNCH();
    return 0;
}

static int embed_fwd_impl(int32_t twin_f16, const int64_t* ids, const int64_t* token_type, const float* word, const float* pos,
                              const float* type, const float* gamma, const float* beta, void* y, void* y_twin,
                              void* xhat, float* rstd, int32_t B, int32_t S, int32_t H, int32_t vocab,
                              int32_t n_type, float eps, float p_drop, uint64_t seed, void* stream) {
    if (!ids || !word || !pos || !type || !gamma || !beta || !y) return ICKA_E_ARG;
    if (B <= 0 || S <= 0 || H <= 0 || H % 8 != 0 || H > 8 * 64 * MAX_CH || vocab <= 0 || n_type <= 0)
        return ICKA_E_SHAPE;
    if (!al16(word) || !al16(pos) || !al16(type) || !al16(gamma) || !al16(beta) || !al16(y) || (xhat && !al16(xhat)) ||
        (y_twin && !al16(y_twin)))
        return ICKA_E_ALIGN;
    EmbFwdArgs a{ids, token_type, word, pos, type, gamma, beta, (bf16_t*)y, y_twin, (bf16_t*)xhat, rstd,
                 B * S, S, H, vocab, n_type, eps, make_drop(p_drop, seed), nullptr, nullptr, S, 0, 0, twin_f16};
    hipStream_t st = (hipStream_t)stream;
    DISPATCH_NCH(pick_nch(H), embed_fwd_kernel, row_grid(B * S), 0, st, a);
    ICKA_CHECK_LAUNCH();
    return 0;
}

extern "C" int icka_embed_fwd(const int64_t* ids, const int64_t* token_type, const float* word, const float* pos,
                              const float* type, const float* gamma, const float* beta, void* y, float* y_f32,
                              void* xhat, float* rstd, int32_t B, int32_t S, int32_t H, int32_t vocab,
                              int32_t n_type, float eps, float p_drop, uint64_t seed, void* stream) {
    return embed_fwd_impl(0, ids, token_type, word, pos, type, gamma, beta, y, y_f32, xhat, rstd, B, S, H, vocab, n_type, eps,
                          p_drop, seed, stream);
}
extern "C" int icka_embed_fwd_h(const int64_t* ids, const int64_t* token_type, const float* word, const float* pos,
                                const float* type, const float* gamma, const float* beta, void* y, void* y_f16,
                                void* xhat, float* rstd, int32_t B, int32_t S, int32_t H, int32_t vocab,
                                int32_t n_type, float eps, float p_drop, uint64_t seed, void* stream) {
    return embed_fwd_impl(1, ids, token_type, word, pos, type, gamma, beta, y, y_f16, xhat, rstd, B, S, H, vocab, n_type, eps,
                          p_drop, seed, stream);
}

extern "C" int icka_embed_prompt_fwd(const int64_t* ids, const int32_t* src, const void* prompt, const float* word,
                                     const float* pos, const float* type, const float* gamma, const float* beta, void* y,
                                     float* y_f32, void* xhat, float* rstd, int32_t B, int32_t S_in, int32_t S,
                                     int32_t P, int32_t H, int32_t vocab, int32_t pos_offset, float eps, float p_drop,
                                     uint64_t seed, void* stream) {
    if (!ids || !src || !prompt || !word || !pos || !type || !gamma || !beta || !y) return ICKA_E_ARG;
    if (B <= 0 || S <= 0 || S_in <= 0 || P <= 0 || H <= 0 || H % 8 != 0 || H > 8 * 64 * MAX_CH || vocab <= 0 || pos_offset < 0)
        return ICKA_E_SHAPE;
    if (!al16(word) || !al16(pos) || !al16(type) || !al16(gamma) || !al16(beta) || !al16(y) || (xhat && !al16(xhat)) ||
        !al16(prompt))
        return ICKA_E_ALIGN;
    EmbFwdArgs a{ids, nullptr, word, pos, type, gamma, beta, (bf16_t*)y, y_f32, (bf16_t*)xhat, rstd,
                 B * S, S, H, vocab, 1, eps, make_drop(p_drop, seed), src, (const bf16_t*)prompt, S_in, P, pos_offset, 0};
    hipStream_t st = (hipStream_t)stream;
    DISPATCH_NCH(pick_nch(H), embed_fwd_kernel, row_grid(B * S), 0, st, a);
    ICKA_CHECK_LAUNCH();
    return 0;
}

static int embed_bwd_impl(const void* dy, const int64_t* ids, const int64_t* token_type, const void* xhat,
                          const float* rstd, const float* gamma, float* dword, float* dtok, float* dpos, float* dtype,
                          float* dgamma, float* dbeta, float* partials, int32_t B, int32_t S, int32_t H,
                          int32_t vocab, int32_t n_type, int32_t padding_idx, float p_drop, uint64_t seed,
                          int32_t accumulate, void* stream) {
    if (!dy || !ids || !xhat || !rstd || !gamma || (!dword && !dtok) || !dpos || !dtype || !dgamma || !dbeta || !partials)
        return ICKA_E_ARG;
    if (B <= 0 || S <= 0 || H <= 0 || H % 8 != 0 || H > 8 * 64 * MAX_CH || vocab <= 0 || n_type <= 0)
        return ICKA_E_SHAPE;
    if (!al16(dy) || !al16(xhat) || !al16(gamma)) return ICKA_E_ALIGN;
    EmbBwdArgs a{(const bf16_t*)dy, ids, token_type, (const bf16_t*)xhat, rstd, gamma, dword, dpos, dtype, partials,
                 B * S, S, H, vocab, n_type, padding_idx, make_drop(p_drop, seed), nullptr, nullptr, S, 0, 0, dtok};
    hipStream_t st = (hipStream_t)stream;
    int grid = bwd_grid(B * S);
    if (S <= BWD_BLOCKS) {
        grid = S;
        switch (pick_nch(H)) {
            case 1: hipLaunchKernelGGL((embed_bwd_pos_kernel<1>), dim3(S), dim3(512), 8 * H * sizeof(float), st, a); break;
            case 2: hipLaunchKernelGGL((embed_bwd_pos_kernel<2>), dim3(S), dim3(512), 8 * H * sizeof(float), st, a); break;
            case 3: hipLaunchKernelGGL((embed_bwd_pos_kernel<3>), dim3(S), dim3(512), 8 * H * sizeof(float), st, a); break;
            default: hipLaunchKernelGGL((embed_bwd_pos_kernel<4>), dim3(S), dim3(512), 8 * H * sizeof(float), st, a); break;
        }
    } else {
        DISPATCH_NCH(pick_nch(H), embed_bwd_kernel, grid, 8 * H * sizeof(float), st, a);
    }
    ICKA_CHECK_LAUNCH();
    float* t0 = n_type <= 2 ? dtype : nullptr;
    float* t1 = n_type == 2 ? dtype + H : nullptr;
    hipLaunchKernelGGL(finalize_kernel, dim3((SLOTS * H + 63) / 64), dim3(1024), 0, st, partials, grid, H, dgamma,
// ... 86 lines not shown
```

### icka_amd/kernels.py

```python
from __future__ import annotations

import ctypes as C
import math
from typing import Optional

import torch

from . import _lib
from ._lib import (EPI_ADD, EPI_ADD_RELU, EPI_DGELU, EPI_GATE, EPI_GELU, EPI_NONE, EPI_RELU, EPI_TANH, GEMM_NN, GEMM_NT, GEMM_TN,
                   GemmDesc, check)

BF16 = torch.bfloat16
F32 = torch.float32
F16 = torch.float16


_RAW_STREAM = getattr(torch._C, "_cuda_getCurrentRawStream", None)
_CUR_DEVICE = getattr(torch._C, "_cuda_getDevice", None)


def _stream() -> int:
    if _RAW_STREAM is not None and _CUR_DEVICE is not None:
        return _RAW_STREAM(_CUR_DEVICE())
    return torch.cuda.current_stream().cuda_stream
# ... 180 lines not shown
        if tile_n not in (96, 128):
            raise ValueError("tile_n: 96 or 128")
        t |= (1 if tile_n == 96 else 2) << 4
    if wide_tiles is not None:
        t |= (2 if wide_tiles else 1) << 8
    if direct_epilogue is not None:
        t |= (2 if direct_epilogue else 1) << 12
    if warp_specialized is not None:
        if warp_specialized not in (0, 1, 2, 3):
            raise ValueError("warp_specialized: 0 .. 3")
        t |= (warp_specialized + 1) << 16
    if w3_grid is not None:
        if w3_grid not in (1, 2, 4, 8):
            raise ValueError("w3_grid: 1, 2, 4 or 8")
        t |= w3_grid << 20
    if big_tiles is not None:
        if big_tiles not in (0, 1, 2):
            raise ValueError("big_tiles: 0 .. 2")
        t |= (big_tiles + 1) << 24
    if ablation is not None:
        if ablation not in (1, 2, 3):
            raise ValueError("ablation: 1 .. 3 (diagnostic builds)")
        t |= ablation << 28
    return t


def gemm(op: int, A: torch.Tensor, B: torch.Tensor, out: torch.Tensor, **kw) -> torch.Tensor:
    lib = _lib.load()
    d = gemm_desc(op, A, B, out, **kw)
    if _PROF is not None:
        _PROF.append((0, d, 1, [d]))
    check(lib.icka_gemm(C.byref(d), _stream()), "icka_gemm")
    return out


def slab_reduction(partials: torch.Tensor, nslab: int, H: int, outs, accumulate: bool, slab_stride: int = 0,
                   offset: int = 0):
    r = _lib.SlabReduction()
    if slab_stride == 0:
        slab_stride = _lib.load().icka_ln_slab_slots() * H
    r.partials, r.slab_stride, r.nslab, r.H = partials.data_ptr() + 4 * offset, slab_stride, nslab, H
    r.nslots, r.accumulate = len(outs), int(bool(accumulate))
    for i, o in enumerate(outs):
        _dev(o, "reduction output")
        if o.dtype != F32 or o.numel() != H or not o.is_contiguous():
            raise ValueError("reduction outputs must be contiguous f32 with %d elements" % H)
        r.out[i] = o.data_ptr()
    r._keep = (partials,) + tuple(outs)
    return r


def cls_head_fwd(seq, gated, W, bias, logits):
    dt = seq.dtype if seq.dtype == F16 else BF16
    _mat(seq, "seq", dt); _mat(gated, "gated", dt)
    M, H = seq.shape
    Cn = W.shape[0]
    if not (seq.is_contiguous() and gated.is_contiguous() and W.is_contiguous() and logits.is_contiguous()):
        raise ValueError("cls_head_fwd: contiguous operands")
    if W.dtype != dt or tuple(W.shape) != (Cn, 2 * H) or logits.dtype != F32 or tuple(logits.shape) != (M, Cn):
        raise ValueError("cls_head_fwd: W %s [C,2H], logits f32 [M,C]" % dt)
    lib = _lib.load()
    fn = lib.icka_cls_head_fwd_h if dt == F16 else lib.icka_cls_head_fwd
    check(fn(seq.data_ptr(), gated.data_ptr(), W.data_ptr(), _ptr(bias), logits.data_ptr(), M, H, Cn, _stream()),
          "icka_cls_head_fwd")
    return logits


def cls_head_bwd(dl, seq, gated, gate, cross, W, dseq, du, dcross, partials):
    M, H = seq.shape
    Cn = W.shape[0]
    for n, t in (("seq", seq), ("gated", gated), ("gate", gate), ("cross", cross), ("dseq", dseq), ("du", du),
                 ("dcross", dcross)):
        _mat(t, n)
        if not t.is_contiguous() or tuple(t.shape) != (M, H):
            raise ValueError("%s must be contiguous bf16 [M,H]" % n)
    _mat(dl, "dl")
    lib = _lib.load()
    check(lib.icka_cls_head_bwd(dl.data_ptr(), dl.stride(0), seq.data_ptr(), gated.data_ptr(), gate.data_ptr(),
                                cross.data_ptr(), W.data_ptr(), dseq.data_ptr(), du.data_ptr(), dcross.data_ptr(),
                                partials.data_ptr(), M, H, Cn, _stream()), "icka_cls_head_bwd")
    return lib.icka_cls_head_bwd_slabs(M)


def gemm_grouped(descs, reductions=None) -> None:
    reductions = reductions or []
    if not descs and not reductions:
        return
    lib = _lib.load()
    arr = (GemmDesc * max(len(descs), 1))(*descs)
    if _PROF is not None and descs:
        _PROF.append((1, arr, len(descs), list(descs)))
    if not reductions:
        check(lib.icka_gemm_grouped(arr, len(descs), _stream()), "icka_gemm_grouped")
        return
    for i in range(0, len(reductions), 4):
        chunk = reductions[i:i + 4]
        rarr = (_lib.SlabReduction * len(chunk))(*chunk)
        check(lib.icka_gemm_grouped_ex(arr if i == 0 else None, len(descs) if i == 0 else 0, rarr, len(chunk),
                                       _stream()), "icka_gemm_grouped_ex")


def _kind(t: torch.Tensor) -> int:
    return {BF16: 0, F32: 1, F16: 2}[t.dtype]


def ln_fwd(x, bias, residual, gamma, beta, y, *, y2=None, y_f32=None, y_f16=None, xhat=None, rstd=None, eps=1e-12,
           p_drop=0.0, seed=0):
    lib = _lib.load()
    _mat(x, "x", x.dtype if x.dtype in (BF16, F32, F16) else BF16); _mat(y, "y")
    if residual is not None:
        _mat(residual, "residual", residual.dtype if residual.dtype in (BF16, F32, F16) else BF16)
    if y_f32 is not None and y_f16 is not None:
        raise ValueError("one twin copy: y_f32 or y_f16")
    M, H = x.shape
    twin = y_f16 if y_f16 is not None else y_f32
    if twin is not None and (twin.dtype != (F16 if y_f16 is not None else F32) or not twin.is_contiguous()
                             or tuple(twin.shape) != (M, H)):
        raise ValueError("twin output must be contiguous [M,H] f32 (y_f32) / fp16 (y_f16)")
    fn = lib.icka_ln_fwd_h if y_f16 is not None else lib.icka_ln_fwd
    check(fn(x.data_ptr(), x.stride(0), _kind(x), _ptr(bias), _ptr(residual), _ld(residual),
             0 if residual is None else _kind(residual), gamma.data_ptr(), beta.data_ptr(),
             y.data_ptr(), y.stride(0), _ptr(y2), _ld(y2), _ptr(twin), _ptr(xhat), _ptr(rstd),
             M, H, eps, p_drop, seed, _stream()), "icka_ln_fwd")
    return y


class GemmLnHandoffError(RuntimeError):
    """A stripe wait of a fused dense + LayerNorm launch gave up: the rows it finished are NaN."""


_GEMM_LN_ERR = None
_GEMM_LN_ERR_NP = None
_GEMM_LN_ERR_PTR = 0


def _gemm_ln_err_word() -> int:
    global _GEMM_LN_ERR, _GEMM_LN_ERR_NP, _GEMM_LN_ERR_PTR
    if _GEMM_LN_ERR is None:
        _GEMM_LN_ERR = torch.zeros(16, dtype=torch.int32).pin_memory()
        _GEMM_LN_ERR_NP = _GEMM_LN_ERR.numpy()
        _GEMM_LN_ERR_PTR = _GEMM_LN_ERR.data_ptr()
    return _GEMM_LN_ERR_PTR


def gemm_ln_sync(device) -> torch.Tensor:
    return torch.zeros(_lib.load().icka_gemm_ln_sync_words(), dtype=torch.int32, device=device)


def gemm_ln(h, w, o, bias, residual, gamma, beta, y, sync, *, y_f32=None, y_f16=None, xhat=None, rstd=None, eps=1e-12,
            p_drop=0.0, seed=0) -> bool:
    gemm_ln_check_error("detected before the next fused launch")
    lib = _lib.load()
    d = gemm_desc(GEMM_NT, h, w, o)
    _mat(y, "y")
    if residual is not None:
        _mat(residual, "residual", residual.dtype if residual.dtype in (BF16, F32, F16) else BF16)
    twin = y_f16 if y_f16 is not None else y_f32
    M, N = o.shape
    if twin is not None and (twin.dtype != (F16 if y_f16 is not None else F32) or not twin.is_contiguous() or tuple(twin.shape) != (M, N)):
        raise ValueError("twin output must be contiguous [M,N] f32 (y_f32) / fp16 (y_f16)")
    args = (d, _ptr(bias), _ptr(residual), _ld(residual), 0 if residual is None else _kind(residual), gamma.data_ptr(),
            beta.data_ptr(), y.data_ptr(), y.stride(0), _ptr(twin), int(y_f16 is not None), _ptr(xhat), _ptr(rstd), eps,
            p_drop, seed, sync.data_ptr(), _gemm_ln_err_word(), _stream())
    rc = lib.icka_gemm_ln(*args)
    if rc == -1:
        return False
    check(rc, "icka_gemm_ln")
    if _PROF is not None:
        d._keep = (h, w, o, bias, residual, gamma, beta, y, twin, xhat, rstd, sync)
        _PROF.append((2, args, 1, [d]))
    return True


def gemm_qkv_attn(x, w, bias, qkv, add_mask, ctx, lse, B, heads, S, *, p_drop=0.0, seed=0, scale=None, out16=None,
                  keepbits=None) -> bool:
    lib = _lib.load()
    d = gemm_desc(GEMM_NT, x, w, qkv, bias=bias)
    _mat(ctx, "ctx")
    H = heads * 64
    if tuple(qkv.shape) != (B * S, 3 * H) or tuple(ctx.shape) != (B * S, H):
        return False
    if add_mask.dtype != F32 or not add_mask.is_contiguous() or add_mask.numel() != B * S:
        raise ValueError("add_mask must be contiguous f32 [B, S]")
    if lse is not None and (lse.dtype != F32 or not lse.is_contiguous() or lse.numel() != B * heads * S):
        raise ValueError("lse must be contiguous f32 [B, heads, S]")
    if out16 is not None:
        _mat(out16, "out16", F16)
        if tuple(out16.shape) != tuple(ctx.shape) or out16.stride(0) != ctx.stride(0):
            raise ValueError("out16 must have the shape and row stride of ctx")
    if keepbits is not None and (not keepbits.is_cuda or keepbits.element_size() != 4 or not keepbits.is_contiguous()
                                 or keepbits.numel() < lib.icka_attn_keepbits_words(B, heads, S, S)):
        raise ValueError("keepbits: contiguous 32-bit device buffer of icka_attn_keepbits_words words (attn_keepbits)")
    args = (d, add_mask.data_ptr(), ctx.data_ptr(), _ptr(out16), ctx.stride(0), _ptr(lse), B, heads, S,
            (1.0 / 8.0) if scale is None else scale, p_drop, seed, _ptr(keepbits), _stream())
    rc = lib.icka_gemm_qkv_attn(*args)
    if rc == -1:
        return False
    check(rc, "icka_gemm_qkv_attn")
    if _PROF is not None:
        d._keep = (x, w, bias, qkv, add_mask, ctx, lse, out16, keepbits)
        _PROF.append((3, args, 1, [d]))
    return True


def gemm_ln_check_error(where: str = "") -> None:
    if _GEMM_LN_ERR_NP is not None and _GEMM_LN_ERR_NP[0] != 0:
        _GEMM_LN_ERR_NP[0] = 0
        raise GemmLnHandoffError(
            "icka_amd fused dense + LayerNorm%s: a block gave up waiting for the other blocks of its 128-row stripe -- the grid "
            "was not co-resident (another kernel held CUs: a collective on another stream, a second model, a partitioned GPU).  "
            "The rows it finished are NaN.  Reserve CUs (icka_lstm_set_reserved_cus) or set ICKA_FUSE_DENSE_LN=0."
            % ((" (" + where + ")") if where else ""))


def ln_bwd_slabs(dy, xhat, rstd, gamma, partials, *, dy2=None, dres=None, dx=None, p_drop=0.0, seed=0) -> int:
    lib = _lib.load()
    _mat(dy, "dy"); _mat(xhat, "xhat")
    M, H = dy.shape
    check(lib.icka_ln_bwd_slabs(dy.data_ptr(), dy.stride(0), _ptr(dy2), _ld(dy2), xhat.data_ptr(), rstd.data_ptr(),
                                gamma.data_ptr(), _ptr(dres), _ld(dres), _ptr(dx), _ld(dx), partials.data_ptr(), M, H,
                                p_drop, seed, _stream()), "icka_ln_bwd_slabs")
    return lib.icka_ln_bwd_nslab(M)


def ln_bwd_workspace(H: int, device) -> torch.Tensor:
    return torch.empty(_lib.load().icka_ln_bwd_workspace_floats(H), dtype=F32, device=device)


def ln_bwd(dy, xhat, rstd, gamma, *, dy2=None, dres=None, dx=None, dgamma=None, dbeta=None, dbias=None,
           partials=None, p_drop=0.0, seed=0, accumulate=True):
    lib = _lib.load()
    _mat(dy, "dy"); _mat(xhat, "xhat")
    M, H = dy.shape
    check(lib.icka_ln_bwd(dy.data_ptr(), dy.stride(0), _ptr(dy2), _ld(dy2), xhat.data_ptr(), rstd.data_ptr(),
                          gamma.data_ptr(), _ptr(dres), _ld(dres), _ptr(dx), _ld(dx), _ptr(dgamma), _ptr(dbeta),
                          _ptr(dbias), partials.data_ptr(), M, H, p_drop, seed, int(accumulate), _stream()),
          "icka_ln_bwd")


def embed_fwd(ids, token_type, word, pos, typ, gamma, beta, y, *, y_f32=None, y_f16=None, xhat=None, rstd=None, eps=1e-12,
              p_drop=0.0, seed=0):
    lib = _lib.load()
    _dev(ids, "ids")
    B, S = ids.shape
    H = word.shape[1]
    if y_f32 is not None and y_f16 is not None:
        raise ValueError("one twin copy: y_f32 or y_f16")
    twin = y_f16 if y_f16 is not None else y_f32
    if twin is not None and (twin.dtype != (F16 if y_f16 is not None else F32) or not twin.is_contiguous()):
        raise ValueError("twin output must be contiguous f32 (y_f32) / fp16 (y_f16)")
    fn = lib.icka_embed_fwd_h if y_f16 is not None else lib.icka_embed_fwd
    check(fn(ids.data_ptr(), _ptr(token_type), word.data_ptr(), pos.data_ptr(), typ.data_ptr(),
             gamma.data_ptr(), beta.data_ptr(), y.data_ptr(), _ptr(twin), _ptr(xhat), _ptr(rstd),
             B, S, H, word.shape[0], typ.shape[0], eps, p_drop, seed, _stream()), "icka_embed_fwd")
    return y


def embed_bwd(dy, ids, token_type, xhat, rstd, gamma, dword, dpos, dtype_, dgamma, dbeta, partials, *,
              padding_idx=0, p_drop=0.0, seed=0, accumulate=True):
    lib = _lib.load()
    B, S = ids.shape
    H = dword.shape[1]
    check(lib.icka_embed_bwd(dy.data_ptr(), ids.data_ptr(), _ptr(token_type), xhat.data_ptr(), rstd.data_ptr(),
                             gamma.data_ptr(), dword.data_ptr(), dpos.data_ptr(), dtype_.data_ptr(),
                             dgamma.data_ptr(), dbeta.data_ptr(), partials.data_ptr(), B, S, H, dword.shape[0],
                             dtype_.shape[0], padding_idx, p_drop, seed, int(accumulate), _stream()),
          "icka_embed_bwd")


def embed_bwd_rows(dy, ids, token_type, xhat, rstd, gamma, dtok, dpos, dtype_, dgamma, dbeta, partials, *, vocab,
                   padding_idx=0, p_drop=0.0, seed=0, accumulate=True):
    lib = _lib.load()
    B, S = ids.shape
    H = dtok.shape[1]
    if dtok.dtype != F32 or tuple(dtok.shape) != (B * S, H) or not dtok.is_contiguous():
        raise ValueError("dtok must be contiguous f32 [B*S, H]")
    check(lib.icka_embed_bwd_rows(dy.data_ptr(), ids.data_ptr(), _ptr(token_type), xhat.data_ptr(), rstd.data_ptr(),
                                  gamma.data_ptr(), dtok.data_ptr(), dpos.data_ptr(), dtype_.data_ptr(), dgamma.data_ptr(),
                                  dbeta.data_ptr(), partials.data_ptr(), B, S, H, int(vocab), dtype_.shape[0], padding_idx, p_drop,
                                  seed, int(accumulate), _stream()), "icka_embed_bwd_rows")


def embed_scatter_rows(rows, ids, dword, *, padding_idx=0, scale=1.0):
    _dev(rows, "rows"); _dev(ids, "ids"); _dev(dword, "dword")
    if rows.dtype not in (F32, BF16) or rows.dim() != 2 or not rows.is_contiguous():
        raise ValueError("rows must be contiguous f32 / bf16 [T, H]")
    if ids.dtype != torch.int64 or ids.numel() != rows.shape[0] or not ids.is_contiguous():
        raise ValueError("ids must be contiguous int64 with one entry per row")
    if dword.dtype != F32 or dword.dim() != 2 or dword.shape[1] != rows.shape[1] or not dword.is_contiguous():
        raise ValueError("dword must be contiguous f32 [vocab, H]")
    check(_lib.load().icka_embed_scatter_rows(rows.data_ptr(), int(rows.dtype == BF16), ids.data_ptr(), dword.data_ptr(),
                                              rows.shape[0], rows.shape[1], dword.shape[0], padding_idx, float(scale), _stream()),
          "icka_embed_scatter_rows")


def embed_prompt_fwd(ids, src, prompt, word, pos, typ, gamma, beta, y, *, y_f32=None, xhat=None, rstd=None,
                     pos_offset=0, eps=1e-5, p_drop=0.0, seed=0):
    lib = _lib.load()
    _dev(ids, "ids"); _dev(src, "src"); _dev(prompt, "prompt")
    if ids.dtype != torch.int64 or not ids.is_contiguous() or ids.dim() != 2:
        raise ValueError("ids must be contiguous int64 [B,S_in]")
    if src.dtype != torch.int32 or src.dim() != 1 or not src.is_contiguous():
        raise ValueError("src must be contiguous int32 [S]")
    B, S_in = ids.shape
# ... 806 lines not shown
```

### icka_amd/ops.py

```python
from __future__ import annotations

from typing import Optional

import torch

from . import kernels as K
from .arena import ParamArena

BF16, F32, F16 = torch.bfloat16, torch.float32, torch.float16
import os as _os
ATTN_KEEPBITS = _os.environ.get("ICKA_ATTN_KEEPBITS", "auto")
FUSE_DENSE_LN = _os.environ.get("ICKA_FUSE_DENSE_LN", "1") != "0"
FUSE_DENSE_LN_MIN_ROWS = 3072
FUSE_QKV_ATTN = _os.environ.get("ICKA_FUSE_QKV_ATTN", "1") != "0"
FUSE_QKV_ATTN_MIN_ROWS = 3072


def _keepbits_on(Sq: int, Skv: int) -> bool:
    if ATTN_KEEPBITS == "auto":
        return Sq > 128 and Skv > 128 and Sq <= 256 and Skv <= 256
    return ATTN_KEEPBITS == "1"


def _empty(ref: torch.Tensor, *shape, dtype=BF16) -> torch.Tensor:
    return torch.empty(*shape, dtype=dtype, device=ref.device)


def _c(t: torch.Tensor) -> torch.Tensor:
    if t.dtype != BF16:
        raise TypeError("expected a bf16 gradient, got %s" % t.dtype)
    return t if t.is_contiguous() else t.contiguous()


class Dims(object):
    __slots__ = ("B", "S", "R", "H", "I", "heads", "eps", "p_hidden", "p_attn", "train", "h16", "pack")

    def __init__(self, B, S, R, H, I, heads, eps, p_hidden, p_attn, train, h16=False, pack=None):
        self.B, self.S, self.R, self.H, self.I, self.heads, self.eps = B, S, R, H, I, heads, eps
        self.p_hidden = p_hidden if train else 0.0
        self.p_attn = p_attn if train else 0.0
        self.train = train
        self.h16 = bool(h16)
        self.pack = pack


def _fwd_twin(A: ParamArena, x, xf, d: Dims):
    if not d.h16:
        return xf
    if A.shadow16 is None:
        A.enable_fp16_shadow()
        A.sync(force=True)
    if xf is not None and xf.dtype == F16:
        return xf
    return K.cast_to_f16(x if xf is None else xf, _empty(x, x.shape[0], x.shape[1], dtype=F16))


def _wgrad(A: ParamArena, dy, x, gout, beta: float, bias=None) -> None:
    bout, bacc = None, False
    if bias is not None:
        bacc = A.grad_beta(bias) > 0
        bout = A.g_cat(bias) if isinstance(bias, tuple) else A.g(bias)
        M, N, Kt = dy.shape[1], x.shape[1], dy.shape[0]
        if M % 128 or N % 128 or Kt % 64:
            csw = A.workspace("colsum", K._lib.load().icka_colsum_workspace_floats(M))
            K.colsum(dy, bout, csw, accumulate=bacc)
            bout = None
    wire = A.wire_of(gout, beta)
    A.pending_wgrad.append((K.gemm_desc(K.GEMM_TN, dy, x, gout, beta=beta, colsum_out=bout, colsum_accumulate=bacc,
                                        **wire), dy, x, gout, bout, wire))


def _flush_wgrad(A: ParamArena) -> None:
    if A.pending_wgrad or A.pending_reductions:
        K.gemm_grouped([t[0] for t in A.pending_wgrad], reductions=A.pending_reductions)
        A.pending_wgrad = []
        A.pending_reductions = []


def _ln_bwd_deferred(A: ParamArena, tag: str, norm, dy, xhat, rstd, *, dy2, dres, dx, p_drop, seed) -> None:
    H = dy.shape[1]
    ws = A.workspace(tag, K._lib.load().icka_ln_bwd_workspace_floats(H))
    acc = A.grad_beta((norm.weight, norm.bias)) > 0
    nslab = K.ln_bwd_slabs(dy, xhat, rstd, norm.weight, ws, dy2=dy2, dres=dres, dx=dx, p_drop=p_drop, seed=seed)
    A.pending_reductions.append(K.slab_reduction(ws, nslab, H, (A.g(norm.weight), A.g(norm.bias)), acc))


def _attn_generic_fwd(qkv, kvbuf, self_attn: bool, add_mask, d: Dims, Skv: int, seed_a: int, ctx, ctx16, save: bool):
    import math
    from . import exact as X
    B, h, S, H = d.B, d.heads, d.S, d.H
    dh = H // h
    q32b = K.cast_bf16_to_f32(qkv, torch.empty(qkv.shape, dtype=F32, device=qkv.device))
    if self_attn:
        q, k, v = q32b[:, :H], q32b[:, H:2 * H], q32b[:, 2 * H:]
        kv32b = None
    else:
        kv32b = K.cast_bf16_to_f32(kvbuf, torch.empty(kvbuf.shape, dtype=F32, device=kvbuf.device))
        q, k, v = q32b, kv32b[:, :H], kv32b[:, H:]
    P = torch.empty(B, h, S, Skv, dtype=F32, device=qkv.device)
    X.gemm_raw(X.GEMM_NT, S, Skv, dh, q, q.stride(0), (S * q.stride(0), dh), k, k.stride(0), (Skv * k.stride(0), dh),
               P, Skv, (h * S * Skv, S * Skv), B, h)
    Pd = torch.empty_like(P) if d.p_attn > 0 else None
    X.softmax_fwd(P, Pd, add_mask, B, h, S, Skv, 1.0 / math.sqrt(dh), d.p_attn, seed_a)
    Pu = P if Pd is None else Pd
    ctx32 = torch.empty(B * S, H, dtype=F32, device=qkv.device)
    X.gemm_raw(X.GEMM_NN, S, dh, Skv, Pu, Skv, (h * S * Skv, S * Skv), v, v.stride(0), (Skv * v.stride(0), dh),
               ctx32, H, (S * H, dh), B, h)
    K.cast_f32_to_bf16(ctx32, ctx)
    if ctx16 is not None:
        K.cast_to_f16(ctx32, ctx16)
    return ("generic", q32b, kv32b, P, Pd) if save else None


def _attn_generic_bwd(gen, self_attn: bool, dctx, d: Dims, Skv: int, seed_a: int, dq_out, dkv_out) -> None:
    import math
    from . import exact as X
    _tag, q32b, kv32b, P, Pd = gen
    B, h, S, H = d.B, d.heads, d.S, d.H
    dh = H // h
    scale = 1.0 / math.sqrt(dh)
    dev = q32b.device
    d32 = K.cast_bf16_to_f32(dctx if dctx.is_contiguous() else dctx.contiguous(), torch.empty(B * S, H, dtype=F32, device=dev))
    if self_attn:
        q, k, v = q32b[:, :H], q32b[:, H:2 * H], q32b[:, 2 * H:]
        g32 = torch.empty(B * S, 3 * H, dtype=F32, device=dev)
        dq, dk, dv = g32[:, :H], g32[:, H:2 * H], g32[:, 2 * H:]
        gkv = None
    else:
        q, k, v = q32b, kv32b[:, :H], kv32b[:, H:]
        g32 = torch.empty(B * S, H, dtype=F32, device=dev)
        gkv = torch.empty(kv32b.shape, dtype=F32, device=dev)
        K.zero_(gkv.view(-1))
        dq, dk, dv = g32, gkv[:, :H], gkv[:, H:]
    pb = (h * S * Skv, S * Skv)
    Pu = P if Pd is None else Pd
    dS = torch.empty_like(P)
    X.gemm_raw(X.GEMM_NT, S, Skv, dh, d32, H, (S * H, dh), v, v.stride(0), (Skv * v.stride(0), dh), dS, Skv, pb, B, h)
    X.gemm_raw(X.GEMM_TN, Skv, dh, S, Pu, Skv, pb, d32, H, (S * H, dh), dv, dv.stride(0), (Skv * dv.stride(0), dh), B, h)
    X.softmax_bwd(P, dS, B, h, S, Skv, scale, d.p_attn, seed_a)
    X.gemm_raw(X.GEMM_NN, S, dh, Skv, dS, Skv, pb, k, k.stride(0), (Skv * k.stride(0), dh), dq, dq.stride(0),
               (S * dq.stride(0), dh), B, h)
    X.gemm_raw(X.GEMM_TN, Skv, dh, S, dS, Skv, pb, q, q.stride(0), (S * q.stride(0), dh), dk, dk.stride(0),
               (Skv * dk.stride(0), dh), B, h)
    K.cast_f32_to_bf16(g32, dq_out)
    if gkv is not None:
        K.cast_f32_to_bf16(gkv, dkv_out)


def _attn_core_fwd(A: ParamArena, sa, x, kv_src, add_mask, d: Dims, Skv: int, save: bool, x16=None, kv16=None):
    M, H = x.shape
    h16 = x16 is not None
    xa = x16 if h16 else x
    if kv_src is None:
        qkv = _empty(x, M, 3 * H)
        wq = (sa.query.weight, sa.key.weight, sa.value.weight)
        bq = A.f_cat((sa.query.bias, sa.key.bias, sa.value.bias))
        pre = None
        want_kb = save and d.p_attn > 0 and _keepbits_on(d.S, Skv)
        if (FUSE_QKV_ATTN and d.pack is None and d.S in (128, 256) and Skv == d.S and H == 64 * d.heads and M >= FUSE_QKV_ATTN_MIN_ROWS
                and not (want_kb and d.S != 256)):
            ctx = _empty(x, M, H)
            ctx16 = _empty(x, M, H, dtype=F16) if h16 else None
            seed_a = A.next_seed() if d.p_attn > 0 else 0
            lse = _empty(x, d.B, d.heads, d.S, dtype=F32) if save else None
            kb = K.attn_keepbits(d.B, d.heads, d.S, Skv, x.device) if want_kb else None
            if K.gemm_qkv_attn(xa, A.w16_cat(wq) if h16 else A.w_cat(wq), bq, qkv, add_mask, ctx, lse, d.B, d.heads, d.S,
                               p_drop=d.p_attn, seed=seed_a, out16=ctx16, keepbits=kb):
                return ctx, ctx16, ((qkv, None, lse, seed_a, kb) if save else None)
            pre = (ctx, seed_a, lse, ctx16, kb)
        K.gemm(K.GEMM_NT, xa, A.w16_cat(wq) if h16 else A.w_cat(wq), qkv, bias=bq)
        q, k, v = qkv[:, :H], qkv[:, H:2 * H], qkv[:, 2 * H:]
        kvbuf = None
    else:
        pre = None
        qkv = _empty(x, M, H)
        K.gemm(K.GEMM_NT, xa, A.w16(sa.query.weight) if h16 else A.w(sa.query.weight), qkv, bias=sa.query.bias)
        kvbuf = _empty(x, kv_src.shape[0], 2 * H)
        wkv = (sa.key.weight, sa.value.weight)
        if h16 and kv16 is not None:
            K.gemm(K.GEMM_NT, kv16, A.w16_cat(wkv), kvbuf, bias=A.f_cat((sa.key.bias, sa.value.bias)))
        else:
            K.gemm(K.GEMM_NT, kv_src, A.w_cat(wkv), kvbuf, bias=A.f_cat((sa.key.bias, sa.value.bias)))
        q, k, v = qkv, kvbuf[:, :H], kvbuf[:, H:]
    ctx = pre[0] if pre else _empty(x, M, H)
    ctx16 = pre[3] if pre else (_empty(x, M, H, dtype=F16) if h16 else None)
    seed_a = pre[1] if pre else (A.next_seed() if d.p_attn > 0 else 0)
    if H // d.heads != 64:
        if (kv_src is not None) and bool(getattr(sa, "fp8_scores", False)):
            raise ValueError("the fp8 cross-attention kernels are built for head size 64, got %d" % (H // d.heads))
        gen = _attn_generic_fwd(qkv, kvbuf, kv_src is None, add_mask, d, Skv, seed_a, ctx, ctx16, save)
        return ctx, ctx16, ((qkv, kvbuf, gen, seed_a, None) if save else None)
    lse = pre[2] if pre else (_empty(x, d.B, d.heads, d.S, dtype=F32) if save else None)
    fp8 = (kv_src is not None) and bool(getattr(sa, "fp8_scores", False))
    kb = pre[4] if pre else (K.attn_keepbits(d.B, d.heads, d.S, Skv, x.device) if (save and d.p_attn > 0 and _keepbits_on(d.S, Skv)) else None)
    if d.pack is not None:
        K.attn_fwd_packed(q, k, v, add_mask, ctx, lse, d.pack.cu, kv_src is None, d.B, d.heads, d.S, Skv, p_drop=d.p_attn,
                          seed=seed_a, keepbits=kb)
        return ctx, ctx16, ((qkv, kvbuf, lse, seed_a, kb) if save else None)
    K.attn_fwd(q, k, v, add_mask, ctx, lse, d.B, d.heads, d.S, Skv, p_drop=d.p_attn, seed=seed_a, fp8=fp8, out16=ctx16,
               keepbits=kb)
    return ctx, ctx16, ((qkv, kvbuf, lse, seed_a, kb) if save else None)


def _attn_core_bwd(A: ParamArena, sa, x, kv_src, add_mask, d: Dims, Skv: int, saved, ctx, dctx, dres, need_dkv_src: bool):
    qkv, kvbuf, lse, seed_a, kb = saved
    M, H = x.shape
    generic = isinstance(lse, tuple)
    delta = None if generic else _empty(x, d.B, d.heads, d.S, dtype=F32)
    epi = dict(epilogue=K.EPI_ADD, aux=dres) if dres is not None else {}
    if kv_src is None:
        dqkv = _empty(x, M, 3 * H)
        q, k, v = qkv[:, :H], qkv[:, H:2 * H], qkv[:, 2 * H:]
        if generic:
            _attn_generic_bwd(lse, True, dctx, d, Skv, seed_a, dqkv, None)
        elif d.pack is not None:
            K.attn_bwd_packed(q, k, v, add_mask, dctx, lse, delta, dqkv[:, :H], dqkv[:, H:2 * H], dqkv[:, 2 * H:], d.pack.cu,
                              True, d.B, d.heads, d.S, Skv, p_drop=d.p_attn, seed=seed_a, keepbits=kb)
        else:
            K.attn_bwd(q, k, v, add_mask, ctx, dctx, lse, delta, dqkv[:, :H], dqkv[:, H:2 * H], dqkv[:, 2 * H:], d.B,
                       d.heads, d.S, Skv, p_drop=d.p_attn, seed=seed_a, keepbits=kb)
        wg = (sa.query.weight, sa.key.weight, sa.value.weight)
        bg = (sa.query.bias, sa.key.bias, sa.value.bias)
        _wgrad(A, dqkv, x, A.g_cat(wg), A.grad_beta(wg), bias=bg)
        dx = _empty(x, M, H)
        K.gemm(K.GEMM_NN, dqkv, A.w_cat(wg), dx, **epi)
        return dx, None
    dq = _empty(x, M, H)
    dkv = _empty(x, kv_src.shape[0], 2 * H)
    if kv_src.shape[0] > d.B * Skv:
        K.zero_rows_(dkv, d.B * Skv)
    if generic:
        _attn_generic_bwd(lse, False, dctx, d, Skv, seed_a, dq, dkv)
    elif d.pack is not None:
        K.attn_bwd_packed(qkv, kvbuf[:, :H], kvbuf[:, H:], add_mask, dctx, lse, delta, dq, dkv[:, :H], dkv[:, H:], d.pack.cu,
                          False, d.B, d.heads, d.S, Skv, p_drop=d.p_attn, seed=seed_a, keepbits=kb)
    else:
        K.attn_bwd(qkv, kvbuf[:, :H], kvbuf[:, H:], add_mask, ctx, dctx, lse, delta, dq, dkv[:, :H], dkv[:, H:], d.B,
                   d.heads, d.S, Skv, p_drop=d.p_attn, seed=seed_a, keepbits=kb)
    _wgrad(A, dq, x, A.g(sa.query.weight), A.grad_beta(sa.query.weight), bias=sa.query.bias)
    wg = (sa.key.weight, sa.value.weight)
    bg = (sa.key.bias, sa.value.bias)
    _wgrad(A, dkv, kv_src, A.g_cat(wg), A.grad_beta(wg), bias=bg)
    dx = _empty(x, M, H)
    K.gemm(K.GEMM_NN, dq, A.w(sa.query.weight), dx, **epi)
    dsrc = None
    if need_dkv_src:
        dsrc = _empty(x, kv_src.shape[0], H)
        K.gemm(K.GEMM_NN, dkv, A.w_cat(wg), dsrc)
    return dx, dsrc


def _dense_norm_fwd(A: ParamArena, mod, h, res, d: Dims, save: bool, h16=None):
    M = h.shape[0]
    H = mod.dense.weight.shape[0]
    o = _empty(h, M, H, dtype=F32)
    y = _empty(h, M, H)
    yf = _empty(h, M, H, dtype=F16 if d.h16 else F32)
    xhat = _empty(h, M, H) if save else None
    rstd = _empty(h, M, dtype=F32) if save else None
    seed_h = A.next_seed() if d.p_hidden > 0 else 0
    twin = {"y_f16": yf} if d.h16 else {"y_f32": yf}
    if FUSE_DENSE_LN and h16 is None and M >= FUSE_DENSE_LN_MIN_ROWS:
        sync = A._ws.get("gemm_ln_sync")
        if sync is None:
            sync = A._ws["gemm_ln_sync"] = K.gemm_ln_sync(h.device)
        if K.gemm_ln(h, A.w(mod.dense.weight), o, mod.dense.bias, res, mod.LayerNorm.weight, mod.LayerNorm.bias, y, sync,
                     xhat=xhat, rstd=rstd, eps=d.eps, p_drop=d.p_hidden, seed=seed_h, **twin):
            return y, yf, ((xhat, rstd, seed_h) if save else None)
    if h16 is not None:
        K.gemm(K.GEMM_NT, h16, A.w16(mod.dense.weight), o)
    else:
        K.gemm(K.GEMM_NT, h, A.w(mod.dense.weight), o)
    K.ln_fwd(o, mod.dense.bias, res, mod.LayerNorm.weight, mod.LayerNorm.bias, y, xhat=xhat, rstd=rstd,
             eps=d.eps, p_drop=d.p_hidden, seed=seed_h, **twin)
    return y, yf, ((xhat, rstd, seed_h) if save else None)


def _dense_norm_bwd(A: ParamArena, tag: str, mod, h, d: Dims, saved, dy, dy2):
    xhat, rstd, seed_h = saved
    M, H = xhat.shape
    dres = _empty(h, M, H)
    do = _empty(h, M, H)
    _ln_bwd_deferred(A, tag, mod.LayerNorm, dy, xhat, rstd, dy2=dy2, dres=dres, dx=do, p_drop=d.p_hidden, seed=seed_h)
    _wgrad(A, do, h, A.g(mod.dense.weight), A.grad_beta(mod.dense.weight), bias=mod.dense.bias)
    return do, dres


def _inter_fwd(A: ParamArena, inter, x, x16=None):
    M = x.shape[0]
    I = inter.dense.weight.shape[0]
    z = _empty(x, M, I)
    g = _empty(x, M, I)
    if x16 is not None:
        g16 = _empty(x, M, I, dtype=F16)
        K.gemm(K.GEMM_NT, x16, A.w16(inter.dense.weight), g16, bias=inter.dense.bias, epilogue=K.EPI_GELU, out2=z, out3=g)
        return g, z, g16
    K.gemm(K.GEMM_NT, x, A.w(inter.dense.weight), g, bias=inter.dense.bias, epilogue=K.EPI_GELU, out2=z)
    return g, z, None


def _inter_bwd(A: ParamArena, inter, x, dz, dres):
    _wgrad(A, dz, x, A.g(inter.dense.weight), A.grad_beta(inter.dense.weight), bias=inter.dense.bias)
    dx = _empty(x, x.shape[0], x.shape[1])
    if dres is not None:
        K.gemm(K.GEMM_NN, dz, A.w(inter.dense.weight), dx, epilogue=K.EPI_ADD, aux=dres)
    else:
        K.gemm(K.GEMM_NN, dz, A.w(inter.dense.weight), dx)
    return dx


def _attn_block_fwd(A: ParamArena, att, x, xres, kv_src, add_mask, d: Dims, Skv: int, save: bool, kv16=None):
    xres = _fwd_twin(A, x, xres, d)
    ctx, ctx16, s_core = _attn_core_fwd(A, att.self, x, kv_src, add_mask, d, Skv, save, x16=xres if d.h16 else None,
                                        kv16=kv16 if d.h16 else None)
    y, yf, s_out = _dense_norm_fwd(A, att.output, ctx, x if xres is None else xres, d, save, h16=ctx16)
    return y, yf, ((ctx, s_core, s_out) if save else None)


def _attn_block_bwd(A: ParamArena, att, x, kv_src, add_mask, d: Dims, Skv: int, saved, dy, dy2, need_dkv_src: bool):
    ctx, s_core, s_out = saved
    dao, dres = _dense_norm_bwd(A, "ln_attn", att.output, ctx, d, s_out, dy, dy2)
    dctx = _empty(x, x.shape[0], x.shape[1])
    K.gemm(K.GEMM_NN, dao, A.w(att.output.dense.weight), dctx)
    return _attn_core_bwd(A, att.self, x, kv_src, add_mask, d, Skv, s_core, ctx, dctx, dres, need_dkv_src)


def _ffn_block_fwd(A: ParamArena, layer, x, xres, d: Dims, save: bool):
    xres = _fwd_twin(A, x, xres, d)
    g, z, g16 = _inter_fwd(A, layer.intermediate, x, xres if d.h16 else None)
    y, yf, s_out = _dense_norm_fwd(A, layer.output, g, x if xres is None else xres, d, save, h16=g16)
    return y, yf, ((z, g, s_out) if save else None)


def _ffn_block_bwd(A: ParamArena, layer, x, d: Dims, saved, dy, dy2=None):
    z, g, s_out = saved
    dfo, dres = _dense_norm_bwd(A, "ln_ffn", layer.output, g, d, s_out, dy, dy2)
    dz = _empty(x, z.shape[0], z.shape[1])
    K.gemm(K.GEMM_NN, dfo, A.w(layer.output.dense.weight), dz, epilogue=K.EPI_DGELU, aux=z)
    return _inter_bwd(A, layer.intermediate, x, dz, dres)


class EmbeddingsFn(torch.autograd.Function):

    @staticmethod
    def forward(ctx, anchor, mod, A: ParamArena, ids, tt, d: Dims):
        B, S = ids.shape
        H = d.H
        save = any(ctx.needs_input_grad)
        y = torch.empty(B * S, H, dtype=BF16, device=ids.device)
        yf = torch.empty(B * S, H, dtype=F16 if d.h16 else F32, device=ids.device)
        xhat = torch.empty_like(y) if save else None
        rstd = torch.empty(B * S, dtype=F32, device=ids.device) if save else None
        seed = A.next_seed() if d.p_hidden > 0 else 0
        K.embed_fwd(ids, tt, mod.word_embeddings.weight, mod.position_embeddings.weight,
                    mod.token_type_embeddings.weight, mod.LayerNorm.weight, mod.LayerNorm.bias, y,
                    xhat=xhat, rstd=rstd, eps=d.eps, p_drop=d.p_hidden, seed=seed,
                    **({"y_f16": yf} if d.h16 else {"y_f32": yf}))
        ctx.mod, ctx.A, ctx.d, ctx.seed = mod, A, d, seed
        ctx.save_for_backward(ids, tt, xhat, rstd)
        ctx.mark_non_differentiable(yf)
        ctx.set_materialize_grads(False)
        return y, yf

    @staticmethod
    def backward(ctx, dy, _dyf=None):
        mod, A, d = ctx.mod, ctx.A, ctx.d
        ids, tt, xhat, rstd = ctx.saved_tensors
        dy = _c(dy)
        ws = A.workspace("ln", K._lib.load().icka_ln_bwd_workspace_floats(d.H))
        tables = (mod.word_embeddings.weight, mod.position_embeddings.weight)
        small = (mod.token_type_embeddings.weight, mod.LayerNorm.weight, mod.LayerNorm.bias)
        red = A.reducer
        if red is not None and getattr(red, "sparse_word", None) is A.slot(tables[0]):
            beta_w = A.grad_beta(tables[0])
            if A.grad_beta(tables[1]) == 0.0:
                K.zero_(A.g(tables[1]).view(-1))
            acc = A.grad_beta(small) > 0
            dtok = A.workspace("dtok", ids.numel() * d.H).view(ids.numel(), d.H)
            K.embed_bwd_rows(dy, ids, tt, xhat, rstd, mod.LayerNorm.weight, dtok, A.g(tables[1]), A.g(small[0]), A.g(small[1]),
                             A.g(small[2]), ws, vocab=tables[0].shape[0], padding_idx=0, p_drop=d.p_hidden, seed=ctx.seed,
                             accumulate=acc)
            red.set_sparse_rows(dtok, ids.reshape(-1), accumulate=beta_w > 0)
            A.flush_final()
            return None, None, None, None, None, None
        if A.grad_beta(tables) == 0.0:
            K.zero_(A.g_cat(tables).view(-1))
        acc = A.grad_beta(small) > 0
        K.embed_bwd(dy, ids, tt, xhat, rstd, mod.LayerNorm.weight, A.g(tables[0]), A.g(tables[1]), A.g(small[0]),
                    A.g(small[1]), A.g(small[2]), ws, padding_idx=0, p_drop=d.p_hidden, seed=ctx.seed, accumulate=acc)
        A.flush_final()
        return None, None, None, None, None, None


class BertLayerFn(torch.autograd.Function):

    @staticmethod
    def forward(ctx, anchor, x, xf, layer, A: ParamArena, add_mask, d: Dims):
        save = any(ctx.needs_input_grad)
        x1, x1f, s_att = _attn_block_fwd(A, layer.attention, x, xf, None, add_mask, d, d.S, save)
        x2, x2f, s_ffn = _ffn_block_fwd(A, layer, x1, x1f, d, save)
        ctx.layer, ctx.A, ctx.d, ctx.s_att, ctx.s_ffn = layer, A, d, s_att, s_ffn
        ctx.save_for_backward(x, x1, add_mask)
        ctx.mark_non_differentiable(x2f)
        ctx.set_materialize_grads(False)
        return x2, x2f

    @staticmethod
    def backward(ctx, dy, _dyf=None):
        x, x1, add_mask = ctx.saved_tensors
        layer, A, d = ctx.layer, ctx.A, ctx.d
        dx1 = _ffn_block_bwd(A, layer, x1, d, ctx.s_ffn, _c(dy))
        dx, _ = _attn_block_bwd(A, layer.attention, x, None, add_mask, d, d.S, ctx.s_att, dx1, None, False)
        if not A.keep_saved:
            ctx.s_att = ctx.s_ffn = None
        _flush_wgrad(A)
        A.flush_final()
        return None, dx, None, None, None, None, None


class CrossLayerFn(torch.autograd.Function):

    @staticmethod
    def forward(ctx, anchor, s1, s1f, s2, layer, A: ParamArena, add_mask, d: Dims, s2_16=None):
        save = any(ctx.needs_input_grad)
        x1, x1f, s_att = _attn_block_fwd(A, layer.attention, s1, s1f, s2, add_mask, d, d.R, save, kv16=s2_16)
        x2, x2f, s_ffn = _ffn_block_fwd(A, layer, x1, x1f, d, save)
        ctx.layer, ctx.A, ctx.d, ctx.s_att, ctx.s_ffn = layer, A, d, s_att, s_ffn
        ctx.need_s2 = s2.requires_grad
        ctx.save_for_backward(s1, s2, x1, add_mask)
        ctx.mark_non_differentiable(x2f)
        ctx.set_materialize_grads(False)
        return x2, x2f

    @staticmethod
    def backward(ctx, dy, _dyf=None):
        s1, s2, x1, add_mask = ctx.saved_tensors
        layer, A, d = ctx.layer, ctx.A, ctx.d
        dx1 = _ffn_block_bwd(A, layer, x1, d, ctx.s_ffn, _c(dy))
        ds1, ds2 = _attn_block_bwd(A, layer.attention, s1, s2, add_mask, d, d.R, ctx.s_att, dx1, None, ctx.need_s2)
        if not A.keep_saved:
            ctx.s_att = ctx.s_ffn = None
        _flush_wgrad(A)
        A.flush_final()
        return None, ds1, None, ds2, None, None, None, None, None


class AttnCoreFn(torch.autograd.Function):

    @staticmethod
    def forward(ctx, anchor, x, kv_src, sa, A: ParamArena, add_mask, d: Dims, Skv: int):
        save = any(ctx.needs_input_grad)
        c, _c16, saved = _attn_core_fwd(A, sa, x, kv_src, add_mask, d, Skv, save)
        ctx.sa, ctx.A, ctx.d, ctx.Skv, ctx.saved = sa, A, d, Skv, saved
        ctx.need_kv = kv_src is not None and kv_src.requires_grad
        ctx.save_for_backward(x, kv_src, add_mask, c)
        return c

    @staticmethod
    def backward(ctx, dc):
        x, kv_src, add_mask, c = ctx.saved_tensors
        A = ctx.A
        dx, dsrc = _attn_core_bwd(A, ctx.sa, x, kv_src, add_mask, ctx.d, ctx.Skv, ctx.saved, c, _c(dc), None, ctx.need_kv)
        if not A.keep_saved:
            ctx.saved = None
        _flush_wgrad(A)
        A.flush_final()
        return None, dx, dsrc, None, None, None, None, None


class DenseResidualNormFn(torch.autograd.Function):

    @staticmethod
    def forward(ctx, anchor, h, res, resf, mod, A: ParamArena, d: Dims):
        save = any(ctx.needs_input_grad)
        y, yf, saved = _dense_norm_fwd(A, mod, h, res if resf is None else resf, d, save)
        ctx.mod, ctx.A, ctx.d, ctx.saved = mod, A, d, saved
        ctx.save_for_backward(h)
        ctx.mark_non_differentiable(yf)
        ctx.set_materialize_grads(False)
        return y, yf

    @staticmethod
    def backward(ctx, dy, _dyf=None):
        (h,) = ctx.saved_tensors
        mod, A = ctx.mod, ctx.A
        do, dres = _dense_norm_bwd(A, "ln_sub", mod, h, ctx.d, ctx.saved, _c(dy), None)
        dh = torch.empty_like(h)
        K.gemm(K.GEMM_NN, do, A.w(mod.dense.weight), dh)
        if not A.keep_saved:
            ctx.saved = None
        _flush_wgrad(A)
        A.flush_final()
        return None, dh, dres, None, None, None, None


class IntermediateFn(torch.autograd.Function):

    @staticmethod
    def forward(ctx, anchor, x, inter, A: ParamArena):
        g, z, _g16 = _inter_fwd(A, inter, x)
        ctx.inter, ctx.A = inter, A
        ctx.save_for_backward(x, z)
        return g

    @staticmethod
    def backward(ctx, dg):
        x, z = ctx.saved_tensors
        A = ctx.A
        dz = K.dgelu(_c(dg), z, torch.empty_like(z))
        dx = _inter_bwd(A, ctx.inter, x, dz, None)
        _flush_wgrad(A)
        A.flush_final()
        return None, dx, None, None


class LinearFn(torch.autograd.Function):

    @staticmethod
    def forward(ctx, anchor, x, lin, A: ParamArena, out_f32: bool, epilogue: int, x16=None):
        M = x.shape[0]
        N = lin.weight.shape[0]
        if x16 is not None:
            if out_f32 or epilogue != K.EPI_NONE:
                raise ValueError("LinearFn: the fp16-operand form is a plain bf16-output projection")
            if A.shadow16 is None:
                A.enable_fp16_shadow()
                A.sync(force=True)
            y = torch.empty(M, N, dtype=BF16, device=x.device)
            y16 = torch.empty(M, N, dtype=F16, device=x.device)
            K.gemm(K.GEMM_NT, x16, A.w16(lin.weight), y16, bias=lin.bias, out3=y)
            ctx.lin, ctx.A, ctx.epi = lin, A, epilogue
            ctx.need_dx = x.requires_grad
            ctx.save_for_backward(x, None)
            ctx.mark_non_differentiable(y16)
            ctx.set_materialize_grads(False)
            return y, y16
        y = torch.empty(M, N, dtype=F32 if out_f32 else BF16, device=x.device)
        if M <= 64 and not out_f32 and x.shape[1] % 128 == 0 and x.stride(0) % 8 == 0 and \
                epilogue in (K.EPI_NONE, K.EPI_TANH):
            K.linear_small_m(x, A.w(lin.weight), lin.bias, y, act=1 if epilogue == K.EPI_TANH else 0)
        else:
            K.gemm(K.GEMM_NT, x, A.w(lin.weight), y, bias=lin.bias, epilogue=epilogue)
        ctx.lin, ctx.A, ctx.epi = lin, A, epilogue
        ctx.need_dx = x.requires_grad
        ctx.save_for_backward(x, y if epilogue == K.EPI_TANH else None)
        return y

    @staticmethod
    def backward(ctx, dy, _dy16=None):
        x, y = ctx.saved_tensors
        lin, A = ctx.lin, ctx.A
        M, N = dy.shape
        if dy.dtype == F32:
            ldd = (N + 7) // 8 * 8
            dyb = torch.empty(M, ldd, dtype=BF16, device=dy.device)
            K.cast_pad_f32_to_bf16(dy if dy.stride(1) == 1 else dy.contiguous(), dyb)
            dyv = dyb[:, :N]
        else:
            dyv = _c(dy)
        if ctx.epi == K.EPI_TANH:
            dyv = K.tanh_bwd(dyv if dyv.is_contiguous() else dyv.contiguous(), y, torch.empty_like(y))
        fused = lin.bias is not None and N % 128 == 0 and x.shape[1] % 128 == 0 and M % 64 == 0
        gw = A.g(lin.weight)
        beta_w = A.grad_beta(lin.weight)
        wire = A.wire_of(gw, beta_w) if (N % 128 == 0 and x.shape[1] % 128 == 0) else {}
        K.gemm(K.GEMM_TN, dyv, x, gw, beta=beta_w,
               colsum_out=A.g(lin.bias) if fused else None,
               colsum_accumulate=fused and A.grad_beta(lin.bias) > 0,
               **wire)
# ... 424 lines not shown
```

### include/icka_hip.h

```cpp
#ifndef ICKA_HIP_H
#define ICKA_HIP_H

#include <stdint.h>

#ifdef __cplusplus
extern "C" {
#endif

#define ICKA_E_SHAPE (-1)
#define ICKA_E_ALIGN (-2)
#define ICKA_E_ARG (-3)

#define ICKA_ABI_VERSION 6
int icka_abi_version(void);
const char* icka_build_arch(void);

int icka_copy_many(const void* const* src, void* const* dst, const int64_t* bytes, int32_t n, void* stream);

enum { ICKA_GEMM_NT = 0, ICKA_GEMM_NN = 1, ICKA_GEMM_TN = 2 };
enum {
    ICKA_EPI_NONE = 0,
    ICKA_EPI_GELU = 1,
    ICKA_EPI_DGELU = 2,
    ICKA_EPI_ADD = 3,
    ICKA_EPI_GATE = 4,
    ICKA_EPI_TANH = 5,
    ICKA_EPI_RELU = 6,
    ICKA_EPI_ADD_RELU = 7
};
typedef struct icka_gemm_desc {
    int32_t op;
    int32_t M, N, K;
    int32_t K1;
    const void* A;  int64_t lda;
    const void* B;  int64_t ldb;
    const void* A2; int64_t lda2;
    const void* B2; int64_t ldb2;
    void* C;  int64_t ldc;  int32_t c_is_f32;
    void* C2; int64_t ldc2;
    const void* aux; int64_t ldaux;
    const float* bias;
    const float* bias2;
    float alpha, beta;
    int32_t epilogue;
    float* colsum_out;
    int32_t colsum_accumulate;
    int32_t ab_f16;
    void* C3; int64_t ldc3;
    int32_t aux_f16;
    int32_t c3_only;
    uint64_t tune;
} icka_gemm_desc;
#define ICKA_TUNE_RING(n) ((uint64_t)(n) << 0)
#define ICKA_TUNE_TILE_N(n) ((uint64_t)((n) == 96 ? 1 : ((n) == 128 ? 2 : 15)) << 4)
#define ICKA_TUNE_WIDE_TILES(b) ((uint64_t)((b) ? 2 : 1) << 8)
#define ICKA_TUNE_DIRECT_EPILOGUE(b) ((uint64_t)((b) ? 2 : 1) << 12)
#define ICKA_TUNE_WARP_SPECIALIZED(v) ((uint64_t)((v) + 1) << 16)
#define ICKA_TUNE_W3_GRID(pm) ((uint64_t)(pm) << 20)
#define ICKA_TUNE_BIG_TILES(v) ((uint64_t)((v) + 1) << 24)
#define ICKA_TUNE_ABLATION(m) ((uint64_t)(m) << 28)
int icka_gemm(const icka_gemm_desc* d, void* stream);
int icka_gemm_grouped(const icka_gemm_desc* descs, int32_t n, void* stream);
typedef struct icka_slab_reduction {
    const float* partials; int64_t slab_stride; int32_t nslab, H, nslots, accumulate;
    float* out[4];
} icka_slab_reduction;
int icka_gemm_grouped_ex(const icka_gemm_desc* descs, int32_t n, const icka_slab_reduction* reds, int32_t n_red,
                         void* stream);
int icka_ln_fwd(const void* x, int64_t ldx, int32_t x_is_f32, const float* bias, const void* residual, int64_t ldr,
                int32_t res_is_f32, const float* gamma, const float* beta, void* y, int64_t ldy, void* y2,
                int64_t ldy2, float* y_f32, void* xhat, float* rstd, int32_t M, int32_t H, float eps, float p_drop,
                uint64_t seed, void* stream);
int icka_gemm_ln(const icka_gemm_desc* d, const float* bias, const void* residual, int64_t ldr, int32_t res_kind,
                 const float* gamma, const float* beta, void* y, int64_t ldy, void* y_twin, int32_t twin_f16, void* xhat,
                 float* rstd, float eps, float p_drop, uint64_t seed, uint32_t* sync_words, uint32_t* error_word, void* stream);
int64_t icka_gemm_ln_sync_words(void);
int icka_gemm_ln_test_hooks(int32_t polls, int32_t drop_block);
int icka_gemm_qkv_attn(const icka_gemm_desc* d, const float* add_mask, void* ctx, void* ctx_f16, int64_t ldo, float* lse,
                       int32_t B, int32_t heads, int32_t S, float scale, float p_drop, uint64_t seed, void* keep_bits, void* stream);
int icka_ln_fwd_h(const void* x, int64_t ldx, int32_t x_kind, const float* bias, const void* residual, int64_t ldr,
                  int32_t res_kind, const float* gamma, const float* beta, void* y, int64_t ldy, void* y2,
                  int64_t ldy2, void* y_f16, void* xhat, float* rstd, int32_t M, int32_t H, float eps, float p_drop,
                  uint64_t seed, void* stream);
int64_t icka_ln_bwd_workspace_floats(int32_t H);
int icka_ln_bwd(const void* dy, int64_t lddy, const void* dy2, int64_t lddy2, const void* xhat, const float* rstd,
                const float* gamma, void* dres, int64_t lddres, void* dx, int64_t lddx, float* dgamma, float* dbeta,
                float* dbias, float* partials, int32_t M, int32_t H, float p_drop, uint64_t seed, int32_t accumulate,
                void* stream);
int icka_ln_bwd_slabs(const void* dy, int64_t lddy, const void* dy2, int64_t lddy2, const void* xhat, const float* rstd,
                      const float* gamma, void* dres, int64_t lddres, void* dx, int64_t lddx, float* partials, int32_t M,
                      int32_t H, float p_drop, uint64_t seed, void* stream);
int32_t icka_ln_bwd_nslab(int32_t M);
int32_t icka_ln_slab_slots(void);

int icka_embed_fwd(const int64_t* ids, const int64_t* token_type, const float* word, const float* pos,
                   const float* type, const float* gamma, const float* beta, void* y, float* y_f32, void* xhat,
                   float* rstd, int32_t B, int32_t S, int32_t H, int32_t vocab, int32_t n_type, float eps,
                   float p_drop, uint64_t seed, void* stream);
int icka_embed_fwd_h(const int64_t* ids, const int64_t* token_type, const float* word, const float* pos,
                     const float* type, const float* gamma, const float* beta, void* y, void* y_f16, void* xhat,
                     float* rstd, int32_t B, int32_t S, int32_t H, int32_t vocab, int32_t n_type, float eps,
                     float p_drop, uint64_t seed, void* stream);
int icka_embed_bwd(const void* dy, const int64_t* ids, const int64_t* token_type, const void* xhat,
                   const float* rstd, const float* gamma, float* dword, float* dpos, float* dtype, float* dgamma,
                   float* dbeta, float* partials, int32_t B, int32_t S, int32_t H, int32_t vocab, int32_t n_type,
                   int32_t padding_idx, float p_drop, uint64_t seed, int32_t accumulate, void* stream);
int icka_embed_bwd_rows(const void* dy, const int64_t* ids, const int64_t* token_type, const void* xhat, const float* rstd,
                        const float* gamma, float* dtok, float* dpos, float* dtype, float* dgamma, float* dbeta, float* partials,
                        int32_t B, int32_t S, int32_t H, int32_t vocab, int32_t n_type, int32_t padding_idx, float p_drop,
                        uint64_t seed, int32_t accumulate, void* stream);
int icka_embed_scatter_rows(const void* rows, int32_t rows_are_bf16, const int64_t* ids, float* dword, int64_t T, int32_t H,
                            int32_t vocab, int32_t padding_idx, float scale, void* stream);
int icka_embed_prompt_fwd(const int64_t* ids, const int32_t* src, const void* prompt, const float* word,
                          const float* pos, const float* type, const float* gamma, const float* beta, void* y,
                          float* y_f32, void* xhat, float* rstd, int32_t B, int32_t S_in, int32_t S, int32_t P,
                          int32_t H, int32_t vocab, int32_t pos_offset, float eps, float p_drop, uint64_t seed,
                          void* stream);
int icka_embed_prompt_bwd(const void* dy, const int64_t* ids, const int32_t* src, const void* xhat, const float* rstd,
                          const float* gamma, float* dword, float* dpos, float* dtype, float* dgamma, float* dbeta,
                          void* dprompt, float* partials, int32_t B, int32_t S_in, int32_t S, int32_t P, int32_t H,
                          int32_t vocab, int32_t pos_offset, int32_t padding_idx, float p_drop, uint64_t seed,
                          int32_t accumulate, void* stream);

int icka_attn_fwd(const void* Q, int64_t ldq, const void* K, int64_t ldk, const void* V, int64_t ldv,
                  const float* add_mask, void* O, int64_t ldo, float* lse, int32_t B, int32_t heads, int32_t Sq,
                  int32_t Skv, float scale, float p_drop, uint64_t seed, void* stream);
int icka_attn_fwd_fp8(const void* Q, int64_t ldq, const void* K, int64_t ldk, const void* V, int64_t ldv,
                      const float* add_mask, void* O, int64_t ldo, float* lse, int32_t B, int32_t heads, int32_t Sq,
                      int32_t Skv, float scale, float p_drop, uint64_t seed, void* stream);
int icka_attn_fwd_ex(const void* Q, int64_t ldq, const void* K, int64_t ldk, const void* V, int64_t ldv,
                     const float* add_mask, void* O, void* O_f16, int64_t ldo, float* lse, int32_t B, int32_t heads,
                     int32_t Sq, int32_t Skv, float scale, float p_drop, uint64_t seed, int32_t flags, void* keep_bits,
                     void* stream);
#define ICKA_ATTN_FP8 1
#define ICKA_ATTN_TILED 2
int64_t icka_attn_keepbits_words(int32_t B, int32_t heads, int32_t Sq, int32_t Skv);
int icka_attn_bwd(const void* Q, int64_t ldq, const void* K, int64_t ldk, const void* V, int64_t ldv,
                  const float* add_mask, const void* O, int64_t ldo, const void* dO, int64_t lddo, const float* lse,
                  float* delta, void* dQ, int64_t lddq, void* dK, int64_t lddk, void* dV, int64_t lddv, int32_t B,
                  int32_t heads, int32_t Sq, int32_t Skv, float scale, float p_drop, uint64_t seed, const void* keep_bits,
                  int32_t flags, void* stream);

int icka_pack_plan(const int64_t* mask, int32_t B, int32_t S, int32_t max_tokens, int32_t* lens, int32_t* cu_seqlens,
                   int32_t* packed_to_padded, int32_t* padded_to_packed, int32_t* cls_of, int32_t* status, void* err_word,
                   void* stream);
int icka_rows_gather(const void* src, int64_t ld_src, int64_t src_rows, void* dst, int64_t ld_dst, int64_t dst_rows,
                     int32_t row_words, const int32_t* map, int64_t map_stride, uint32_t fill, void* stream);
int icka_attn_fwd_packed(const void* Q, int64_t ldq, const void* K, int64_t ldk, const void* V, int64_t ldv,
                         const float* add_mask, void* O, int64_t ldo, float* lse, const int32_t* cu_seqlens, int32_t kv_packed,
                         int64_t Mrows, int32_t B, int32_t heads, int32_t Sq, int32_t Skv, float scale, float p_drop,
                         uint64_t seed, void* keep_bits, void* stream);
int icka_attn_bwd_packed(const void* Q, int64_t ldq, const void* K, int64_t ldk, const void* V, int64_t ldv,
                         const float* add_mask, const void* dO, int64_t lddo, const float* lse, float* delta, void* dQ,
                         int64_t lddq, void* dK, int64_t lddk, void* dV, int64_t lddv, const int32_t* cu_seqlens,
                         int32_t kv_packed, int64_t Mrows, int32_t B, int32_t heads, int32_t Sq, int32_t Skv, float scale,
                         float p_drop, uint64_t seed, const void* keep_bits, void* stream);

int icka_cast_f32_to_bf16(const float* src, void* dst, int64_t n, void* stream);
int icka_cast_bf16_to_f32(const void* src, float* dst, int64_t n, void* stream);
int icka_cast_to_f16(const void* src, int32_t src_is_f32, void* dst, int64_t n, void* stream);
int icka_cast_f32_to_bf16_f16(const float* src, void* dst_bf16, void* dst_f16, int64_t n, void* stream);
int icka_cast_pad_f32_to_bf16(const float* src, int64_t lds, void* dst, int64_t ldd, int32_t M, int32_t N,
                              void* stream);
int icka_additive_mask(const int64_t* mask, int64_t ld, float* out, int32_t B, int32_t T, void* stream);
int icka_dropout(const void* x, int64_t ldx, void* y, int64_t ldy, void* y2, int64_t ldy2, int32_t M, int32_t H,
                 float p_drop, uint64_t seed, void* stream);
int icka_regions_to_tokens(const float* src, void* dst, int32_t B, int32_t R, int32_t C, int32_t layout,
                           void* stream);
int icka_regions_to_tokens_h(const float* src, void* dst_bf16, void* dst_f16, int32_t B, int32_t R, int32_t C, int32_t layout,
                             void* stream);
int icka_colsum(const void* x, int64_t ldx, float* out, float* partials, int32_t M, int32_t N, int32_t accumulate,
                void* stream);
int64_t icka_colsum_workspace_floats(int32_t N);
int icka_gate_bwd(const void* dout, int64_t lddout, const void* g, const void* cross, int64_t ldcross,
// ... 182 lines not shown
```

Measured before the change: 6994 samples/s.

## Skip all-zero token tiles in weight-gradient GEMMs using LayerNorm-backward liveness flags

The LayerNorm backward kernel gains a variant that records per-row flags saying whether each token row's output gradient is non-zero. A second flag per row marks whether its key is masked by the attention mask. The grouped big-GEMM weight-gradient kernel gets a LIVE mode that reads these flags per 64-row K tile, ballots them into a bitmask and loads and multiplies only the live tiles. This cuts DMA and MFMA work for padded tokens, at the cost of extra flag writes, mask reads and a tile-counting pass. Separately, split-K for small fp32-output GEMMs is limited to the layout where both operands are K-major.

```diff
diff --git a/icka_amd/_lib.py b/icka_amd/_lib.py
--- a/icka_amd/_lib.py
+++ b/icka_amd/_lib.py
@@ -57,6 +57,7 @@
     "icka_gemm": (c_i32, [C.POINTER(GemmDesc), c_vp]),
     "icka_gemm_grouped": (c_i32, [C.POINTER(GemmDesc), c_i32, c_vp]),
     "icka_gemm_grouped_ex": (c_i32, [C.POINTER(GemmDesc), c_i32, C.POINTER(SlabReduction), c_i32, c_vp]),
+    "icka_gemm_grouped_live": (c_i32, [C.POINTER(GemmDesc), c_i32, C.POINTER(SlabReduction), c_i32, C.POINTER(c_vp), c_vp]),
     "icka_gemm_ln": (c_i32, [C.POINTER(GemmDesc), c_vp, c_vp, c_i64, c_i32, c_vp, c_vp, c_vp, c_i64, c_vp, c_i32, c_vp, c_vp, c_f32,
                              c_f32, c_u64, c_vp, c_vp, c_vp]),
     "icka_gemm_qkv_attn": (c_i32, [C.POINTER(GemmDesc), c_vp, c_vp, c_vp, c_i64, c_vp, c_i32, c_i32, c_i32, c_f32, c_f32, c_u64, c_vp, c_vp]),
@@ -71,6 +72,8 @@
                             c_vp, c_i32, c_i32, c_f32, c_u64, c_i32, c_vp]),
     "icka_ln_bwd_slabs": (c_i32, [c_vp, c_i64, c_vp, c_i64, c_vp, c_vp, c_vp, c_vp, c_i64, c_vp, c_i64, c_vp, c_i32,
                                   c_i32, c_f32, c_u64, c_vp]),
+    "icka_ln_bwd_slabs_live": (c_i32, [c_vp, c_i64, c_vp, c_i64, c_vp, c_vp, c_vp, c_vp, c_i64, c_vp, c_i64, c_vp, c_vp, c_vp,
+                                       c_vp, c_i32, c_i32, c_i32, c_f32, c_u64, c_vp]),
     "icka_ln_bwd_nslab": (c_i32, [c_i32]),
     "icka_ln_slab_slots": (c_i32, []),
     "icka_embed_fwd": (c_i32, [c_vp, c_vp, c_vp, c_vp, c_vp, c_vp, c_vp, c_vp, c_vp, c_vp, c_vp, c_i32, c_i32,
diff --git a/icka_amd/csrc/gemm.hip b/icka_amd/csrc/gemm.hip
--- a/icka_amd/csrc/gemm.hip
+++ b/icka_amd/csrc/gemm.hip
@@ -380,6 +380,13 @@
         : "memory", "scc");
 #pragma unroll
     for (int j = 0; j < 4; ++j) ptr[j] += stride;
+}
+
+__device__ __forceinline__ void dma_issue_at(const bf16_t* const (&ptr)[4], int64_t off, uint32_t lds_base) {
+    const bf16_t* q[4];
+#pragma unroll
+    for (int j = 0; j < 4; ++j) q[j] = ptr[j] + off;
+    dma_issue(q, 0, lds_base);
 }
 
 __device__ __forceinline__ uint32_t off_c(int row, int ch) { return row * 512 + ((ch ^ (row & 31)) << 4); }
@@ -1617,7 +1624,7 @@
     } else {
         const int nk = (g.K + BK - 1) / BK;
         int ks = 1;
-        if (g.c_f32 && g.epi == ICKA_EPI_NONE && nb < 64 && nk >= 16 && g.M <= 256 && !g.C3) {
+        if (A_KM && B_KM && g.c_f32 && g.epi == ICKA_EPI_NONE && nb < 64 && nk >= 16 && g.M <= 256 && !g.C3) {
             ks = 256 / nb;
             if (ks > nk / 4) ks = nk / 4;
             if (ks < 1) ks = 1;
@@ -1964,6 +1971,45 @@
     int cs_start[MAX_GROUP + 1];
     SlabRed red[MAX_RED];
     int red_start[MAX_RED + 1];
+    const uint8_t* k_live[MAX_GROUP];
+};
+
+struct LiveTiles {
+    const uint8_t* flags;
+    int nk, base, lane;
+    uint64_t word;
+    __device__ __forceinline__ uint64_t load_word() const {
+        uint32_t any = 0u;
+        const int t = base + lane;
+        if (t < nk) {
+            any = 1u;
+            if (flags) {
+                const u32x4* q = reinterpret_cast<const u32x4*>(flags + (int64_t)t * BK);
+                const u32x4 v = (q[0] | q[1]) | (q[2] | q[3]);
+                any = (v[0] | v[1]) | (v[2] | v[3]);
+            }
+        }
+        return __ballot(any != 0u);
+    }
+    __device__ __forceinline__ LiveTiles(const uint8_t* f, int nk_, int lane_) : flags(f), nk(nk_), base(0), lane(lane_) {
+        word = load_word();
+    }
+    static __device__ __forceinline__ int count(const uint8_t* f, int nk, int lane) {
+        LiveTiles lt(f, nk, lane);
+        int n = __builtin_popcountll(lt.word);
+        for (lt.base = 64; lt.base < nk; lt.base += 64) n += __builtin_popcountll(lt.load_word());
+        return n;
+    }
+    __device__ __forceinline__ int next() {
+        while (word == 0) {
+            if (base + 64 >= nk) return -1;
+            base += 64;
+            word = load_word();
+        }
+        const int kt = base + __builtin_ctzll(word);
+        word &= word - 1;
+        return kt;
+    }
 };
 
 __device__ __forceinline__ void slab_reduce_block(const SlabRed& r, char* smem, int rb) {
@@ -2184,8 +2230,9 @@
 }
 
 
-template <bool WIRE>
-__device__ __forceinline__ void gemm_big12_tn_body(const GemmArgs& g, char* smem, const int m0, const int n0) {
+template <bool WIRE, bool LIVE = false>
+__device__ __forceinline__ void gemm_big12_tn_body(const GemmArgs& g, char* smem, const int m0, const int n0,
+                                                   const uint8_t* k_live = nullptr) {
     const int tid = threadIdx.x, lane = tid & 63;
     const int wave = __builtin_amdgcn_readfirstlane(tid >> 6);
     const uint32_t lds0 = __builtin_amdgcn_readfirstlane((uint32_t)reinterpret_cast<uintptr_t>(LDS_PTR(char, smem)));
@@ -2205,6 +2252,38 @@
         dma_issue(pa1, sa, lds0 + (BUF) + TILE_BYTES + lw * 1024);       \
         dma_issue(pb, sb, lds0 + (BUF) + 2 * TILE_BYTES + lw * 1024);    \
     } while (0)
+        if constexpr (LIVE) {
+            static_assert(BIG_NBUF == 3, "the live-tile loader keeps two tiles in flight");
+#define ICKA_BIG_STAGE_AT(BUF, KT)                                                       \
+    do {                                                                                 \
+        const int64_t oa = (KT) * sa, ob = (KT) * sb;                                    \
+        dma_issue_at(pa0, oa, lds0 + (BUF) + lw * 1024);                                 \
+        dma_issue_at(pa1, oa, lds0 + (BUF) + TILE_BYTES + lw * 1024);                    \
+        dma_issue_at(pb, ob, lds0 + (BUF) + 2 * TILE_BYTES + lw * 1024);                 \
+    } while (0)
+            LiveTiles lt(k_live, nk, lane);
+            int t0 = lt.next();
+            int t1 = t0 >= 0 ? lt.next() : -1;
+            if (t0 >= 0) ICKA_BIG_STAGE_AT(0, t0);
+            if (t1 >= 0) ICKA_BIG_STAGE_AT(BIG_STAGE, t1);
+            int cur = 0;
+            while (t0 >= 0) {
+                const int t2 = t1 >= 0 ? lt.next() : -1;
+                if (t1 >= 0) wait_vmcnt<12>();
+                else wait_vmcnt<0>();
+                __builtin_amdgcn_s_barrier();
+                if (t2 >= 0) {
+                    int nx = cur + BIG_NBUF - 1;
+                    nx = nx >= BIG_NBUF ? nx - BIG_NBUF : nx;
+                    ICKA_BIG_STAGE_AT(nx * BIG_STAGE, t2);
+                }
+                cur = cur + 1 == BIG_NBUF ? 0 : cur + 1;
+                t0 = t1;
+                t1 = t2;
+            }
+#undef ICKA_BIG_STAGE_AT
+            return;
+        }
 #pragma unroll
         for (int t = 0; t < BIG_NBUF - 1; ++t)
             if (t < nk) ICKA_BIG_STAGE(t * BIG_STAGE);
@@ -2232,26 +2311,25 @@
 #pragma unroll
         for (int j = 0; j < 4; ++j) acc[i][j] = f32x4{0.f, 0.f, 0.f, 0.f};
     int cur = 0;
-    for (int kt = 0; kt < nk; ++kt) {
-        __builtin_amdgcn_s_barrier();
-        asm volatile("" ::: "memory");
-        const char* st = smem + cur * BIG_STAGE;
-        const char* sA = st + (wr >> 7) * TILE_BYTES;
-        const char* sB = st + 2 * TILE_BYTES;
-#pragma unroll
-        for (int ks = 0; ks < 2; ++ks) {
-            bf16x8 fa[4], fb[4];
-#pragma unroll
-            for (int t = 0; t < 4; ++t) fa[t] = read_frag<true>(sA, (wr & 127) + 16 * t, ks, lane);
-#pragma unroll
-            for (int t = 0; t < 4; ++t) fb[t] = read_frag<true>(sB, wc + 16 * t, ks, lane);
-#pragma unroll
-            for (int mi = 0; mi < 4; ++mi)
-#pragma unroll
-                for (int ni = 0; ni < 4; ++ni) acc[mi][ni] = mfma16(fb[ni], fa[mi], acc[mi][ni]);
-        }
-        cur = cur + 1 == BIG_NBUF ? 0 : cur + 1;
-    }
+#define ICKA_BIG12_TILE()                                                                                    \
+    do {                                                                                                     \
+        __builtin_amdgcn_s_barrier();        \
+        asm volatile("" ::: "memory");                                                                       \
+        const char* st = smem + cur * BIG_STAGE;                                                             \
+        const char* sA = st + (wr >> 7) * TILE_BYTES;                                                        \
+        const char* sB = st + 2 * TILE_BYTES;                                                                \
+        _Pragma("unroll") for (int ks = 0; ks < 2; ++ks) {                                                   \
+            bf16x8 fa[4], fb[4];                                                                             \
+            _Pragma("unroll") for (int t = 0; t < 4; ++t) fa[t] = read_frag<true>(sA, (wr & 127) + 16 * t, ks, lane); \
+            _Pragma("unroll") for (int t = 0; t < 4; ++t) fb[t] = read_frag<true>(sB, wc + 16 * t, ks, lane); \
+            _Pragma("unroll") for (int mi = 0; mi < 4; ++mi)                                                 \
+                _Pragma("unroll") for (int ni = 0; ni < 4; ++ni) acc[mi][ni] = mfma16(fb[ni], fa[mi], acc[mi][ni]); \
+        }                                                                                                    \
+        cur = cur + 1 == BIG_NBUF ? 0 : cur + 1;                                                             \
+    } while (0)
+    const int ntrip = LIVE ? LiveTiles::count(k_live, nk, lane) : nk;
+    for (int kt = 0; kt < ntrip; ++kt) ICKA_BIG12_TILE();
+#undef ICKA_BIG12_TILE
     asm volatile("s_nop 7\n\ts_nop 7" ::: "memory");
 #pragma unroll
     for (int ni = 0; ni < 4; ++ni) {
@@ -2270,7 +2348,7 @@
     }
 }
 
-template <bool W12, bool WIRE = false>
+template <bool W12, bool WIRE = false, bool LIVE = false>
 __global__ __launch_bounds__(W12 ? 768 : 512) void gemm_big_group_kernel(const BigGroupArgs ga) {
     __shared__ __attribute__((aligned(16))) char smem[BIG_NBUF * BIG_STAGE];
     const int bid = blockIdx.x;
@@ -2306,7 +2384,8 @@
     int tm, tn;
     if (nbn > nbm) { tm = local % nbm; tn = local / nbm; }
     else { tm = local / nbn; tn = local % nbn; }
-    if constexpr (W12) gemm_big12_tn_body<WIRE>(g, smem, tm * 256, tn * BN);
+    if constexpr (W12 && LIVE) gemm_big12_tn_body<WIRE, true>(g, smem, tm * 256, tn * BN, ga.k_live[pi]);
+    else if constexpr (W12) gemm_big12_tn_body<WIRE>(g, smem, tm * 256, tn * BN);
     else gemm_big_tn_body<WIRE>(g, smem, tm * 256, tn * BN);
 }
 
@@ -2330,21 +2409,37 @@
 }
 
 static int grouped_impl(const icka_gemm_desc* descs, int32_t n, const icka_slab_reduction* reds, int32_t n_red,
-                        hipStream_t st);
+                        hipStream_t st, const uint8_t* const* k_live = nullptr);
 
 extern "C" int icka_gemm_grouped(const icka_gemm_desc* descs, int32_t n, void* stream) {
     if (!descs || n <= 0) return ICKA_E_ARG;
     return grouped_impl(descs, n, nullptr, 0, (hipStream_t)stream);
 }
 
-extern "C" int icka_gemm_grouped_ex(const icka_gemm_desc* descs, int32_t n, const icka_slab_reduction* reds,
-                                    int32_t n_red, void* stream) {
+static int grouped_args_ok(const icka_gemm_desc* descs, int32_t n, const icka_slab_reduction* reds, int32_t n_red) {
     if (n < 0 || n_red < 0 || (n > 0 && !descs) || (n_red > 0 && !reds) || n_red > MAX_RED) return ICKA_E_ARG;
     for (int r = 0; r < n_red; ++r)
         if (!reds[r].partials || reds[r].nslab <= 0 || reds[r].H <= 0 || reds[r].nslots <= 0 || reds[r].nslots > 4 ||
             reds[r].slab_stride < (int64_t)reds[r].nslots * reds[r].H)
             return ICKA_E_ARG;
+    return 0;
+}
+
+extern "C" int icka_gemm_grouped_ex(const icka_gemm_desc* descs, int32_t n, const icka_slab_reduction* reds,
+                                    int32_t n_red, void* stream) {
+    const int rc = grouped_args_ok(descs, n, reds, n_red);
+    if (rc) return rc;
     return grouped_impl(descs, n, reds, n_red, (hipStream_t)stream);
+}
+
+extern "C" int icka_gemm_grouped_live(const icka_gemm_desc* descs, int32_t n, const icka_slab_reduction* reds,
+                                      int32_t n_red, const uint8_t* const* k_live, void* stream) {
+    if (k_live)
+        for (int i = 0; i < n; ++i)
+            if (reinterpret_cast<uintptr_t>(k_live[i]) & 15) return ICKA_E_ALIGN;
+    const int rc = grouped_args_ok(descs, n, reds, n_red);
+    if (rc) return rc;
+    return grouped_impl(descs, n, reds, n_red, (hipStream_t)stream, k_live);
 }
 
 static SlabRed to_red(const icka_slab_reduction& r) {
@@ -2357,7 +2452,7 @@
 }
 
 static int grouped_impl(const icka_gemm_desc* descs, int32_t n, const icka_slab_reduction* reds, int32_t n_red,
-                        hipStream_t st) {
+                        hipStream_t st, const uint8_t* const* k_live) {
     bool reds_done = n_red == 0;
     int i = 0;
     Tune t = kTuneEnv;
@@ -2374,6 +2469,7 @@
                 if (rc) return rc;
                 if (!big_ok(g, aligned)) break;
                 ba.p[cnt] = g;
+                ba.k_live[cnt] = k_live ? k_live[i + cnt] : nullptr;
                 ba.start[cnt] = total;
                 ba.cs_start[cnt] = cs_total;
                 total += (g.M / 256) * (g.N / BN);
@@ -2382,7 +2478,7 @@
             }
             if (cnt >= 1 && total >= 64) {
                 for (int k = cnt; k <= MAX_GROUP; ++k) { ba.start[k] = total; ba.cs_start[k] = cs_total; }
-                for (int k = cnt; k < MAX_GROUP; ++k) ba.p[k] = ba.p[0];
+                for (int k = cnt; k < MAX_GROUP; ++k) { ba.p[k] = ba.p[0]; ba.k_live[k] = nullptr; }
                 int red_total = 0;
                 for (int r = 0; r < MAX_RED; ++r) {
                     ba.red_start[r] = red_total;
@@ -2392,9 +2488,16 @@
                 ba.red_start[MAX_RED] = red_total;
                 reds_done = true;
                 bool wire = false;
-                for (int k = 0; k < cnt; ++k) wire = wire || ba.p[k].C3 != nullptr;
+                bool live = false;
+                for (int k = 0; k < cnt; ++k) {
+                    wire = wire || ba.p[k].C3 != nullptr;
+                    live = live || ba.k_live[k] != nullptr;
+                }
                 const dim3 grid(total + cs_total + red_total);
-                if (t.big == 2) {
+                if (t.big == 2 && live) {
+                    if (wire) hipLaunchKernelGGL((gemm_big_group_kernel<true, true, true>), grid, dim3(768), 0, st, ba);
+                    else hipLaunchKernelGGL((gemm_big_group_kernel<true, false, true>), grid, dim3(768), 0, st, ba);
+                } else if (t.big == 2) {
                     if (wire) hipLaunchKernelGGL((gemm_big_group_kernel<true, true>), grid, dim3(768), 0, st, ba);
                     else hipLaunchKernelGGL((gemm_big_group_kernel<true, false>), grid, dim3(768), 0, st, ba);
                 } else {
diff --git a/icka_amd/csrc/layernorm.hip b/icka_amd/csrc/layernorm.hip
--- a/icka_amd/csrc/layernorm.hip
+++ b/icka_amd/csrc/layernorm.hip
@@ -20,7 +20,10 @@
     const bf16_t* dy; int64_t lddy; const bf16_t* dy2; int64_t lddy2; const bf16_t* xhat; const float* rstd;
     const float* gamma; bf16_t* dres; int64_t lddres; bf16_t* dx; int64_t lddx; float* partials;
     int M, H; DropCfg drop;
+    uint8_t* row_live; uint8_t* row_live_kv; const float* add_mask; int mask_S;
 };
+
+constexpr float ICKA_MASKED_KEY_MAX = -5000.f;
 
 template <int NCH, int NS>
 __device__ __forceinline__ void flush_columns(float (&acc)[NS][NCH][8], float* lds, float* partials, int H) {
@@ -61,7 +64,7 @@
     for (int e = 0; e < 8; ++e) o[e] = bf2f(v[e]);
 }
 
-template <int NCH>
+template <int NCH, bool LIVE = false>
 __device__ __forceinline__ void ln_rows_body(const LnBwdArgs& a_, int blk, int nblk) {
     LnBwdArgs a = a_;
     a.drop = drop_resolve(a.drop);
@@ -74,6 +77,13 @@
     for (int row = wid; row < a.M; row += nw) {
         float xh[NCH][8], gd[NCH][8];
         float s1 = 0.f, s2 = 0.f;
+        float m_self = 0.f, m_lo = 0.f, m_hi = 0.f;
+        if (LIVE && a.row_live_kv) {
+            const float* ms = a.add_mask + (int64_t)(row / a.mask_S) * a.mask_S;
+            m_self = a.add_mask[row];
+            m_lo = lane < a.mask_S ? ms[lane] : m_self;
+            m_hi = lane + 64 < a.mask_S ? ms[lane + 64] : m_self;
+        }
         uint32_t kb[NCH];
 #pragma unroll
         for (int i = 0; i < NCH; ++i) {
@@ -112,10 +122,18 @@
                 }
             }
         }
+        bool key_open = true;
+        if (LIVE && a.row_live_kv) {
+            bool above = m_self - m_lo <= ICKA_MASKED_KEY_MAX || m_self - m_hi <= ICKA_MASKED_KEY_MAX;
+            const float* ms = a.add_mask + (int64_t)(row / a.mask_S) * a.mask_S;
+            for (int k = lane + 128; k < a.mask_S; k += 64) above = above || m_self - ms[k] <= ICKA_MASKED_KEY_MAX;
+            key_open = __ballot(above) == 0;
+        }
         const int nrow = row + nw;
         if (nrow < a.M) ln_bwd_load_raw<NCH>(a, nrow, lane, nchunk, rdy, rdy2, rxh);
         const float c1 = wave_sum(s1) * inv_h, c2 = wave_sum(s2) * inv_h;
         const float rstd = a.rstd[row];
+        bool nz = false;
 #pragma unroll
         for (int i = 0; i < NCH; ++i) {
             const int c = lane + 64 * i;
@@ -123,12 +141,23 @@
                 float ds[8];
 #pragma unroll
                 for (int e = 0; e < 8; ++e) ds[e] = rstd * (gd[i][e] - c1 - xh[i][e] * c2);
+                if constexpr (LIVE) {
+#pragma unroll
+                    for (int e = 0; e < 8; ++e) nz = nz || ds[e] != 0.f;
+                }
                 if (a.dres) store8(a.dres + (int64_t)row * a.lddres + c * 8, ds);
                 if (a.drop.thr) {
 #pragma unroll
                     for (int e = 0; e < 8; ++e) ds[e] *= ((kb[i] >> e) & 1u) ? a.drop.scale : 0.f;
                 }
                 if (a.dx) store8(a.dx + (int64_t)row * a.lddx + c * 8, ds);
+            }
+        }
+        if constexpr (LIVE) {
+            const bool live = __ballot(nz) != 0;
+            if (lane == 0) {
+                a.row_live[row] = live ? 1 : 0;
+                if (a.row_live_kv) a.row_live_kv[row] = (live || key_open) ? 1 : 0;
             }
         }
     }
@@ -198,11 +227,11 @@
 struct LnColsArgs {
     int nx, groups, rows_per_group;
 };
-template <int NCH>
+template <int NCH, bool LIVE = false>
 __global__ __launch_bounds__(256) void ln_bwd_fused_kernel(const LnBwdArgs a, const LnColsArgs c) {
     const int ncol = c.nx * c.groups;
     if ((int)blockIdx.x >= ncol) {
-        ln_rows_body<NCH>(a, blockIdx.x - ncol, gridDim.x - ncol);
+        ln_rows_body<NCH, LIVE>(a, blockIdx.x - ncol, gridDim.x - ncol);
         return;
     }
     ln_cols_body(a.dy, a.lddy, a.dy2, a.lddy2, a.xhat, nullptr, 0, a.partials, a.M, a.H, c.rows_per_group,
@@ -613,22 +642,34 @@
 }
 extern "C" int32_t icka_ln_slab_slots(void) { return SLOTS; }
 
-extern "C" int icka_ln_bwd_slabs(const void* dy, int64_t lddy, const void* dy2, int64_t lddy2, const void* xhat,
-                                 const float* rstd, const float* gamma, void* dres, int64_t lddres, void* dx,
-                                 int64_t lddx, float* partials, int32_t M, int32_t H, float p_drop, uint64_t seed,
-                                 void* stream) {
+static int ln_bwd_slabs_impl(const void* dy, int64_t lddy, const void* dy2, int64_t lddy2, const void* xhat,
+                             const float* rstd, const float* gamma, void* dres, int64_t lddres, void* dx,
+                             int64_t lddx, float* partials, int32_t M, int32_t H, float p_drop, uint64_t seed,
+                             uint8_t* row_live, uint8_t* row_live_kv, const float* add_mask, int32_t mask_S,
+                             void* stream) {
     if (!dy || !xhat || !rstd || !gamma || !partials) return ICKA_E_ARG;
     if (M <= 0 || H <= 0 || H % 8 != 0 || H > 8 * 64 * MAX_CH) return ICKA_E_SHAPE;
     if (lddy % 8 || (dy2 && lddy2 % 8) || (dres && lddres % 8) || (dx && lddx % 8)) return ICKA_E_ALIGN;
     if (!al16(dy) || (dy2 && !al16(dy2)) || !al16(xhat) || (dres && !al16(dres)) || (dx && !al16(dx)) || !al16(gamma))
         return ICKA_E_ALIGN;
     LnBwdArgs a{(const bf16_t*)dy, lddy, (const bf16_t*)dy2, lddy2, (const bf16_t*)xhat, rstd, gamma,
-                (bf16_t*)dres, lddres, (bf16_t*)dx, lddx, partials, M, H, make_drop(p_drop, seed)};
+                (bf16_t*)dres, lddres, (bf16_t*)dx, lddx, partials, M, H, make_drop(p_drop, seed),
+                row_live, row_live_kv, add_mask, mask_S};
     const int groups = icka_ln_bwd_nslab(M);
     const int nx = (H + 255) / 256;
     const LnColsArgs c{nx, groups, (M + groups - 1) / groups};
     const int grid = nx * groups + bwd_row_grid(M);
     hipStream_t st = (hipStream_t)stream;
+    if (row_live) {
+        switch (pick_nch(H)) {
+            case 1: hipLaunchKernelGGL((ln_bwd_fused_kernel<1, true>), dim3(grid), dim3(256), 0, st, a, c); break;
+            case 2: hipLaunchKernelGGL((ln_bwd_fused_kernel<2, true>), dim3(grid), dim3(256), 0, st, a, c); break;
+            case 3: hipLaunchKernelGGL((ln_bwd_fused_kernel<3, true>), dim3(grid), dim3(256), 0, st, a, c); break;
+            default: hipLaunchKernelGGL((ln_bwd_fused_kernel<4, true>), dim3(grid), dim3(256), 0, st, a, c); break;
+        }
+        ICKA_CHECK_LAUNCH();
+        return 0;
+    }
     switch (pick_nch(H)) {
         case 1: hipLaunchKernelGGL((ln_bwd_fused_kernel<1>), dim3(grid), dim3(256), 0, st, a, c); break;
         case 2: hipLaunchKernelGGL((ln_bwd_fused_kernel<2>), dim3(grid), dim3(256), 0, st, a, c); break;
@@ -637,6 +678,25 @@
     }
     ICKA_CHECK_LAUNCH();
     return 0;
+}
+
+extern "C" int icka_ln_bwd_slabs(const void* dy, int64_t lddy, const void* dy2, int64_t lddy2, const void* xhat,
+                                 const float* rstd, const float* gamma, void* dres, int64_t lddres, void* dx,
+                                 int64_t lddx, float* partials, int32_t M, int32_t H, float p_drop, uint64_t seed,
+                                 void* stream) {
+    return ln_bwd_slabs_impl(dy, lddy, dy2, lddy2, xhat, rstd, gamma, dres, lddres, dx, lddx, partials, M, H, p_drop, seed,
+                             nullptr, nullptr, nullptr, 0, stream);
+}
+
+extern "C" int icka_ln_bwd_slabs_live(const void* dy, int64_t lddy, const void* dy2, int64_t lddy2, const void* xhat,
+                                      const float* rstd, const float* gamma, void* dres, int64_t lddres, void* dx,
+                                      int64_t lddx, float* partials, uint8_t* row_live, uint8_t* row_live_kv,
+                                      const float* add_mask, int32_t mask_S, int32_t M, int32_t H, float p_drop,
+                                      uint64_t seed, void* stream) {
+    if (!row_live) return ICKA_E_ARG;
+    if (row_live_kv && (!add_mask || mask_S <= 0 || M % mask_S != 0)) return ICKA_E_ARG;
+    return ln_bwd_slabs_impl(dy, lddy, dy2, lddy2, xhat, rstd, gamma, dres, lddres, dx, lddx, partials, M, H, p_drop, seed,
+                             row_live, row_live_kv, row_live_kv ? add_mask : nullptr, mask_S, stream);
 }
 
 static int embed_fwd_impl(int32_t twin_f16, const int64_t* ids, const int64_t* token_type, const float* word, const float* pos,
diff --git a/icka_amd/kernels.py b/icka_amd/kernels.py
--- a/icka_amd/kernels.py
+++ b/icka_amd/kernels.py
@@ -286,7 +286,7 @@
     return lib.icka_cls_head_bwd_slabs(M)
 
 
-def gemm_grouped(descs, reductions=None) -> None:
+def gemm_grouped(descs, reductions=None, k_live=None) -> None:
     reductions = reductions or []
     if not descs and not reductions:
         return
@@ -294,6 +294,17 @@
     arr = (GemmDesc * max(len(descs), 1))(*descs)
     if _PROF is not None and descs:
         _PROF.append((1, arr, len(descs), list(descs)))
+    if k_live is not None and any(f is not None for f in k_live):
+        if len(k_live) != len(descs) or len(reductions) > 4:
+            raise ValueError("gemm_grouped: one k_live entry per problem, at most 4 reductions")
+        for f, dsc in zip(k_live, descs):
+            if f is not None and (f.dtype != torch.uint8 or not f.is_contiguous() or f.numel() != dsc.K):
+                raise ValueError("gemm_grouped: k_live must be a contiguous uint8 [K] tensor")
+        larr = (C.c_void_p * len(descs))(*[None if f is None else f.data_ptr() for f in k_live])
+        rarr = (_lib.SlabReduction * max(len(reductions), 1))(*reductions)
+        check(lib.icka_gemm_grouped_live(arr, len(descs), rarr if reductions else None, len(reductions), larr, _stream()),
+              "icka_gemm_grouped_live")
+        return
     if not reductions:
         check(lib.icka_gemm_grouped(arr, len(descs), _stream()), "icka_gemm_grouped")
         return
@@ -424,6 +435,26 @@
     check(lib.icka_ln_bwd_slabs(dy.data_ptr(), dy.stride(0), _ptr(dy2), _ld(dy2), xhat.data_ptr(), rstd.data_ptr(),
                                 gamma.data_ptr(), _ptr(dres), _ld(dres), _ptr(dx), _ld(dx), partials.data_ptr(), M, H,
                                 p_drop, seed, _stream()), "icka_ln_bwd_slabs")
+    return lib.icka_ln_bwd_nslab(M)
+
+
+def ln_bwd_slabs_live(dy, xhat, rstd, gamma, partials, row_live, *, row_live_kv=None, add_mask=None, dy2=None, dres=None,
+                      dx=None, p_drop=0.0, seed=0) -> int:
+    lib = _lib.load()
+    _mat(dy, "dy"); _mat(xhat, "xhat")
+    M, H = dy.shape
+    for f in (row_live, row_live_kv):
+        if f is not None and (f.dtype != torch.uint8 or not f.is_contiguous() or f.numel() != M):
+            raise ValueError("ln_bwd_slabs_live: the flags are contiguous uint8 [M] tensors")
+    S = 0
+    if row_live_kv is not None:
+        if add_mask is None or add_mask.dtype != F32 or not add_mask.is_contiguous() or add_mask.numel() != M:
+            raise ValueError("ln_bwd_slabs_live: row_live_kv needs the contiguous f32 additive mask [B,S] with B*S == M")
+        S = add_mask.shape[-1]
+    check(lib.icka_ln_bwd_slabs_live(dy.data_ptr(), dy.stride(0), _ptr(dy2), _ld(dy2), xhat.data_ptr(), rstd.data_ptr(),
+                                     gamma.data_ptr(), _ptr(dres), _ld(dres), _ptr(dx), _ld(dx), partials.data_ptr(),
+                                     row_live.data_ptr(), _ptr(row_live_kv), _ptr(add_mask) if S else None, S, M, H,
+                                     p_drop, seed, _stream()), "icka_ln_bwd_slabs_live")
     return lib.icka_ln_bwd_nslab(M)
 
 
diff --git a/icka_amd/ops.py b/icka_amd/ops.py
--- a/icka_amd/ops.py
+++ b/icka_amd/ops.py
@@ -14,6 +14,7 @@
 FUSE_DENSE_LN_MIN_ROWS = 3072
 FUSE_QKV_ATTN = _os.environ.get("ICKA_FUSE_QKV_ATTN", "1") != "0"
 FUSE_QKV_ATTN_MIN_ROWS = 3072
+WGRAD_LIVE = _os.environ.get("ICKA_WGRAD_LIVE", "1") != "0"
 
 
 def _keepbits_on(Sq: int, Skv: int) -> bool:
@@ -55,7 +56,7 @@
     return K.cast_to_f16(x if xf is None else xf, _empty(x, x.shape[0], x.shape[1], dtype=F16))
 
 
-def _wgrad(A: ParamArena, dy, x, gout, beta: float, bias=None) -> None:
+def _wgrad(A: ParamArena, dy, x, gout, beta: float, bias=None, k_live=None) -> None:
     bout, bacc = None, False
     if bias is not None:
         bacc = A.grad_beta(bias) > 0
@@ -67,22 +68,35 @@
             bout = None
     wire = A.wire_of(gout, beta)
     A.pending_wgrad.append((K.gemm_desc(K.GEMM_TN, dy, x, gout, beta=beta, colsum_out=bout, colsum_accumulate=bacc,
-                                        **wire), dy, x, gout, bout, wire))
+                                        **wire), dy, x, gout, bout, wire, k_live))
 
 
 def _flush_wgrad(A: ParamArena) -> None:
     if A.pending_wgrad or A.pending_reductions:
-        K.gemm_grouped([t[0] for t in A.pending_wgrad], reductions=A.pending_reductions)
+        flags = [t[6] for t in A.pending_wgrad]
+        if any(f is not None for f in flags):
+            K.gemm_grouped([t[0] for t in A.pending_wgrad], reductions=A.pending_reductions, k_live=flags)
+        else:
+            K.gemm_grouped([t[0] for t in A.pending_wgrad], reductions=A.pending_reductions)
         A.pending_wgrad = []
         A.pending_reductions = []
 
 
-def _ln_bwd_deferred(A: ParamArena, tag: str, norm, dy, xhat, rstd, *, dy2, dres, dx, p_drop, seed) -> None:
+def _ln_bwd_deferred(A: ParamArena, tag: str, norm, dy, xhat, rstd, *, dy2, dres, dx, p_drop, seed, live=False, add_mask=None):
     H = dy.shape[1]
     ws = A.workspace(tag, K._lib.load().icka_ln_bwd_workspace_floats(H))
     acc = A.grad_beta((norm.weight, norm.bias)) > 0
-    nslab = K.ln_bwd_slabs(dy, xhat, rstd, norm.weight, ws, dy2=dy2, dres=dres, dx=dx, p_drop=p_drop, seed=seed)
+    flags = None
+    if live:
+        row_live = _empty(dy, dy.shape[0], dtype=torch.uint8)
+        row_live_kv = _empty(dy, dy.shape[0], dtype=torch.uint8) if add_mask is not None else None
+        nslab = K.ln_bwd_slabs_live(dy, xhat, rstd, norm.weight, ws, row_live, row_live_kv=row_live_kv, add_mask=add_mask,
+                                    dy2=dy2, dres=dres, dx=dx, p_drop=p_drop, seed=seed)
+        flags = (row_live, row_live_kv)
+    else:
+        nslab = K.ln_bwd_slabs(dy, xhat, rstd, norm.weight, ws, dy2=dy2, dres=dres, dx=dx, p_drop=p_drop, seed=seed)
     A.pending_reductions.append(K.slab_reduction(ws, nslab, H, (A.g(norm.weight), A.g(norm.bias)), acc))
+    return flags
 
 
 def _attn_generic_fwd(qkv, kvbuf, self_attn: bool, add_mask, d: Dims, Skv: int, seed_a: int, ctx, ctx16, save: bool):
@@ -202,7 +216,8 @@
     return ctx, ctx16, ((qkv, kvbuf, lse, seed_a, kb) if save else None)
 
 
-def _attn_core_bwd(A: ParamArena, sa, x, kv_src, add_mask, d: Dims, Skv: int, saved, ctx, dctx, dres, need_dkv_src: bool):
+def _attn_core_bwd(A: ParamArena, sa, x, kv_src, add_mask, d: Dims, Skv: int, saved, ctx, dctx, dres, need_dkv_src: bool,
+                   k_live=None):
     qkv, kvbuf, lse, seed_a, kb = saved
     M, H = x.shape
     generic = isinstance(lse, tuple)
@@ -221,7 +236,7 @@
                        d.heads, d.S, Skv, p_drop=d.p_attn, seed=seed_a, keepbits=kb)
         wg = (sa.query.weight, sa.key.weight, sa.value.weight)
         bg = (sa.query.bias, sa.key.bias, sa.value.bias)
-        _wgrad(A, dqkv, x, A.g_cat(wg), A.grad_beta(wg), bias=bg)
+        _wgrad(A, dqkv, x, A.g_cat(wg), A.grad_beta(wg), bias=bg, k_live=k_live)
         dx = _empty(x, M, H)
         K.gemm(K.GEMM_NN, dqkv, A.w_cat(wg), dx, **epi)
         return dx, None
@@ -276,14 +291,16 @@
     return y, yf, ((xhat, rstd, seed_h) if save else None)
 
 
-def _dense_norm_bwd(A: ParamArena, tag: str, mod, h, d: Dims, saved, dy, dy2):
+def _dense_norm_bwd(A: ParamArena, tag: str, mod, h, d: Dims, saved, dy, dy2, live=False, add_mask=None):
     xhat, rstd, seed_h = saved
     M, H = xhat.shape
     dres = _empty(h, M, H)
     do = _empty(h, M, H)
-    _ln_bwd_deferred(A, tag, mod.LayerNorm, dy, xhat, rstd, dy2=dy2, dres=dres, dx=do, p_drop=d.p_hidden, seed=seed_h)
-    _wgrad(A, do, h, A.g(mod.dense.weight), A.grad_beta(mod.dense.weight), bias=mod.dense.bias)
-    return do, dres
+    flags = _ln_bwd_deferred(A, tag, mod.LayerNorm, dy, xhat, rstd, dy2=dy2, dres=dres, dx=do, p_drop=d.p_hidden, seed=seed_h,
+                             live=live, add_mask=add_mask)
+    _wgrad(A, do, h, A.g(mod.dense.weight), A.grad_beta(mod.dense.weight), bias=mod.dense.bias,
+           k_live=flags[0] if flags else None)
+    return do, dres, flags
 
 
 def _inter_fwd(A: ParamArena, inter, x, x16=None):
@@ -299,8 +316,8 @@
     return g, z, None
 
 
-def _inter_bwd(A: ParamArena, inter, x, dz, dres):
-    _wgrad(A, dz, x, A.g(inter.dense.weight), A.grad_beta(inter.dense.weight), bias=inter.dense.bias)
+def _inter_bwd(A: ParamArena, inter, x, dz, dres, k_live=None):
+    _wgrad(A, dz, x, A.g(inter.dense.weight), A.grad_beta(inter.dense.weight), bias=inter.dense.bias, k_live=k_live)
     dx = _empty(x, x.shape[0], x.shape[1])
     if dres is not None:
         K.gemm(K.GEMM_NN, dz, A.w(inter.dense.weight), dx, epilogue=K.EPI_ADD, aux=dres)
@@ -317,12 +334,16 @@
     return y, yf, ((ctx, s_core, s_out) if save else None)
 
 
-def _attn_block_bwd(A: ParamArena, att, x, kv_src, add_mask, d: Dims, Skv: int, saved, dy, dy2, need_dkv_src: bool):
+def _attn_block_bwd(A: ParamArena, att, x, kv_src, add_mask, d: Dims, Skv: int, saved, dy, dy2, need_dkv_src: bool,
+                    live=False):
     ctx, s_core, s_out = saved
-    dao, dres = _dense_norm_bwd(A, "ln_attn", att.output, ctx, d, s_out, dy, dy2)
+    live = live and kv_src is None
+    dao, dres, flags = _dense_norm_bwd(A, "ln_attn", att.output, ctx, d, s_out, dy, dy2, live=live,
+                                       add_mask=add_mask if live else None)
     dctx = _empty(x, x.shape[0], x.shape[1])
     K.gemm(K.GEMM_NN, dao, A.w(att.output.dense.weight), dctx)
-    return _attn_core_bwd(A, att.self, x, kv_src, add_mask, d, Skv, s_core, ctx, dctx, dres, need_dkv_src)
+    return _attn_core_bwd(A, att.self, x, kv_src, add_mask, d, Skv, s_core, ctx, dctx, dres, need_dkv_src,
+                          k_live=flags[1] if flags else None)
 
 
 def _ffn_block_fwd(A: ParamArena, layer, x, xres, d: Dims, save: bool):
@@ -332,12 +353,12 @@
     return y, yf, ((z, g, s_out) if save else None)
 
 
-def _ffn_block_bwd(A: ParamArena, layer, x, d: Dims, saved, dy, dy2=None):
+def _ffn_block_bwd(A: ParamArena, layer, x, d: Dims, saved, dy, dy2=None, live=False):
     z, g, s_out = saved
-    dfo, dres = _dense_norm_bwd(A, "ln_ffn", layer.output, g, d, s_out, dy, dy2)
+    dfo, dres, flags = _dense_norm_bwd(A, "ln_ffn", layer.output, g, d, s_out, dy, dy2, live=live)
     dz = _empty(x, z.shape[0], z.shape[1])
     K.gemm(K.GEMM_NN, dfo, A.w(layer.output.dense.weight), dz, epilogue=K.EPI_DGELU, aux=z)
-    return _inter_bwd(A, layer.intermediate, x, dz, dres)
+    return _inter_bwd(A, layer.intermediate, x, dz, dres, k_live=flags[0] if flags else None)
 
 
 class EmbeddingsFn(torch.autograd.Function):
@@ -409,8 +430,9 @@
     def backward(ctx, dy, _dyf=None):
         x, x1, add_mask = ctx.saved_tensors
         layer, A, d = ctx.layer, ctx.A, ctx.d
-        dx1 = _ffn_block_bwd(A, layer, x1, d, ctx.s_ffn, _c(dy))
-        dx, _ = _attn_block_bwd(A, layer.attention, x, None, add_mask, d, d.S, ctx.s_att, dx1, None, False)
+        live = WGRAD_LIVE and d.pack is None and add_mask.numel() == x.shape[0]
+        dx1 = _ffn_block_bwd(A, layer, x1, d, ctx.s_ffn, _c(dy), live=live)
+        dx, _ = _attn_block_bwd(A, layer.attention, x, None, add_mask, d, d.S, ctx.s_att, dx1, None, False, live=live)
         if not A.keep_saved:
             ctx.s_att = ctx.s_ffn = None
         _flush_wgrad(A)
@@ -484,7 +506,7 @@
     def backward(ctx, dy, _dyf=None):
         (h,) = ctx.saved_tensors
         mod, A = ctx.mod, ctx.A
-        do, dres = _dense_norm_bwd(A, "ln_sub", mod, h, ctx.d, ctx.saved, _c(dy), None)
+        do, dres, _ = _dense_norm_bwd(A, "ln_sub", mod, h, ctx.d, ctx.saved, _c(dy), None)
         dh = torch.empty_like(h)
         K.gemm(K.GEMM_NN, do, A.w(mod.dense.weight), dh)
         if not A.keep_saved:
diff --git a/include/icka_hip.h b/include/icka_hip.h
--- a/include/icka_hip.h
+++ b/include/icka_hip.h
@@ -67,6 +67,8 @@
 } icka_slab_reduction;
 int icka_gemm_grouped_ex(const icka_gemm_desc* descs, int32_t n, const icka_slab_reduction* reds, int32_t n_red,
                          void* stream);
+int icka_gemm_grouped_live(const icka_gemm_desc* descs, int32_t n, const icka_slab_reduction* reds, int32_t n_red,
+                           const uint8_t* const* k_live, void* stream);
 int icka_ln_fwd(const void* x, int64_t ldx, int32_t x_is_f32, const float* bias, const void* residual, int64_t ldr,
                 int32_t res_is_f32, const float* gamma, const float* beta, void* y, int64_t ldy, void* y2,
                 int64_t ldy2, float* y_f32, void* xhat, float* rstd, int32_t M, int32_t H, float eps, float p_drop,
@@ -90,6 +92,10 @@
 int icka_ln_bwd_slabs(const void* dy, int64_t lddy, const void* dy2, int64_t lddy2, const void* xhat, const float* rstd,
                       const float* gamma, void* dres, int64_t lddres, void* dx, int64_t lddx, float* partials, int32_t M,
                       int32_t H, float p_drop, uint64_t seed, void* stream);
+int icka_ln_bwd_slabs_live(const void* dy, int64_t lddy, const void* dy2, int64_t lddy2, const void* xhat,
+                           const float* rstd, const float* gamma, void* dres, int64_t lddres, void* dx, int64_t lddx,
+                           float* partials, uint8_t* row_live, uint8_t* row_live_kv, const float* add_mask,
+                           int32_t mask_S, int32_t M, int32_t H, float p_drop, uint64_t seed, void* stream);
 int32_t icka_ln_bwd_nslab(int32_t M);
 int32_t icka_ln_slab_slots(void);
 
```

Result: faster. 7131 samples/s, median of 6 (+1.9%).
